# briangodwinlim/SIR-GCN

Measured on AMD Instinct MI355X. Metric: edges/sec SIRConv fwd+bwd, d_hidden=256, 1/2/4/8 MI355X, higher is better.
Workload: dtype f32; 1 GPU; cfg4 S2: Chung-Lu power-law V=2000000 E=40000000 alpha=0.8; 1 SIRConv layer d_in=H=d_out=256, agg=sum, LeakyReLU(0.2), f32, feat_dropout=0.0; fwd+bwd incl. projections; graph=S2, V=2000000, E=40000000, hidden=256, agg=sum, parallelism=single GPU

## Files before the change

include/sirconv.h:

```cpp
#ifndef SIRCONV_H
#define SIRCONV_H

#include <stdint.h>

#ifdef __cplusplus
extern "C" {
#endif

#define SIR_ABI_VERSION 17

enum { SIR_AGG_SUM = 0, SIR_AGG_MEAN = 1, SIR_AGG_SYM = 2, SIR_AGG_ACCUMULATE = 16 };
enum { SIR_ACT_IDENTITY = 0, SIR_ACT_RELU = 1, SIR_ACT_LEAKY_RELU = 2, SIR_ACT_GELU = 3, SIR_ACT_GELU_TANH = 4 };
enum { SIR_DTYPE_F32 = 0, SIR_DTYPE_BF16 = 1, SIR_DTYPE_F16 = 2 };
enum { SIR_OK = 0, SIR_EINVAL = 1, SIR_EUNSUPPORTED = 2, SIR_ELAUNCH = 3 };

int sir_abi_version(void);
const char* sir_source_hash(void);
const char* sir_last_error(void);

typedef struct {
    uint64_t seed;
    double p;
    const uint64_t* seed_ptr;
} sir_dropout_t;

int sir_dropout_apply(void* X, int64_t ldx, int64_t M, int64_t N, int dtype, int64_t col0,
                      const sir_dropout_t* drop, void* stream);

int64_t sir_mask_words(int64_t H, int act);

int sir_degree_norms(const int32_t* rowptr_dst, float* in_norm,
                     const int32_t* rowptr_src, float* out_norm, int64_t n, void* stream);

#define SIR_COLSUM_BLOCKS 1024
int sir_col_sum(const float* X, int64_t ld, int64_t n_rows, int64_t n_cols, float* out,
                float* workspace, void* stream);

int sir_edge_agg_fwd(const int32_t* rowptr, const int32_t* col,
                     const int32_t* items, int64_t n_items,
                     const int32_t* splits, int64_t n_splits,
                     int64_t H, int dtype,
                     const void* Q, int64_t ldq, const void* K, int64_t ldk,
                     const float* norm_row, const float* norm_col,
                     int agg, int act, float slope,
                     void* S, int64_t lds, uint64_t* mask_out, float* partial, void* stream);

int sir_edge_agg_bwd_dst(const int32_t* rowptr, const int32_t* col,
                         const int32_t* items, int64_t n_items,
                         const int32_t* splits, int64_t n_splits,
                         int64_t H, int dtype,
                         const void* Q, int64_t ldq, const void* K, int64_t ldk,
                         const uint64_t* mask,
                         const void* G, int64_t ldg,
                         const float* norm_row, const float* norm_col,
                         int agg, int act, float slope,
                         void* dQ, int64_t lddq, void* Gm, int64_t ldgm,
                         float* partial, const sir_dropout_t* drop, void* stream);

int sir_edge_agg_bwd_src(const int32_t* rowptr_s, const int32_t* col_s, const int32_t* perm_s,
                         const int32_t* items, int64_t n_items,
                         const int32_t* splits, int64_t n_splits,
                         int64_t H, int dtype,
                         const void* K, int64_t ldk, const void* Q, int64_t ldq,
                         const uint64_t* mask,
                         const void* Gd, int64_t ldg,
                         const float* norm_row, const float* norm_col,
                         int agg, int act, float slope,
                         void* dK, int64_t lddk, float* partial, const sir_dropout_t* drop, void* stream);

int sir_edge_agg_bwd(const int32_t* rowptr, const int32_t* col, const int32_t* items, int64_t n_items,
                     const int32_t* splits, int64_t n_splits,
                     const int32_t* rowptr_s, const int32_t* col_s, const int32_t* perm_s,
                     const int32_t* items_s, int64_t n_items_s, const int32_t* splits_s, int64_t n_splits_s,
                     int64_t H, int dtype, const uint64_t* mask, const void* G, int64_t ldg,
                     const float* in_norm, const float* out_norm, int agg, int act, float slope,
                     void* dQ, int64_t lddq, void* dK, int64_t lddk, float* partial, float* partial_s,
                     const sir_dropout_t* drop, void* stream);

int sir_edge_e_agg_fwd(const int32_t* rowptr, const int32_t* col, const int32_t* items, int64_t n_items,
                       const int32_t* splits, int64_t n_splits, int64_t H, int dtype,
                       const void* Q, int64_t ldq, const void* K, int64_t ldk,
                       const void* Eh, int64_t lde, int64_t n_erows, const int32_t* eidx,
                       const float* norm_row, const float* norm_col, int agg, int act, float slope,
                       void* S, int64_t lds, uint64_t* mask_out, float* partial, void* stream);

int sir_edge_e_bwd(const int32_t* rowptr, const int32_t* col, const int32_t* items, int64_t n_items,
                   int64_t H, int dtype, const uint64_t* mask, const void* G, int64_t ldg,
                   const float* norm_row, const float* norm_col, int agg, int act, float slope,
                   const int32_t* eidx, int64_t n_erows, void* dE, int64_t ldde, void* stream);


int sir_edge_gather_add(const int32_t* rowptr, const int32_t* col, const int32_t* items, int64_t n_items,
                        int64_t F, const float* Q, int64_t ldq, const float* K, int64_t ldk,
                        float* Z, int64_t ldz, void* stream);

int sir_edge_gather_act(const int32_t* rowptr, const int32_t* col, const int32_t* items, int64_t n_items,
                        int64_t F, const float* Q, int64_t ldq, const float* K, int64_t ldk, int act, float slope,
                        float* A, int64_t lda, uint64_t* sign_mask, void* stream);

int sir_segment_sum(const int32_t* rowptr, const int32_t* col, const int32_t* perm,
                    const int32_t* items, int64_t n_items, const int32_t* splits, int64_t n_splits,
                    int64_t F, const float* X, int64_t ldx, const float* norm_row, const float* norm_col,
                    int mean, float* out, int64_t ldo, float* partial, void* stream);

int sir_edge_broadcast(const int32_t* rowptr, const int32_t* col, const int32_t* items, int64_t n_items,
                       int64_t F, const float* dS, int64_t lds, const float* norm_row, const float* norm_col,
                       int mean, float* dM, int64_t ldm, void* stream);

int sir_segment_max(const int32_t* items, int64_t n_items, const int32_t* splits, int64_t n_splits,
                    int64_t F, const float* M, int64_t ldm, float* Y, int64_t ldy, int32_t* arg, int64_t lda,
                    float* pval, int32_t* parg, void* stream);

int sir_segment_max_bwd(const int32_t* items, int64_t n_items, int64_t F, const int32_t* arg, int64_t lda,
                        const float* dY, int64_t ldy, float* dM, int64_t ldm, void* stream);

#define SIR_AGG_MAX 3
int64_t sir_edge_mlp_pack_bytes(int64_t H, int64_t F);
int sir_edge_mlp_pack(const float* W, int64_t H, int64_t F, void* packed, void* stream);
int sir_edge_mlp_fwd(const int32_t* rowptr, const int32_t* col, const int32_t* items, int64_t n_items,
                     const int32_t* splits, int64_t n_splits, int64_t H, int64_t F,
                     const float* Q, int64_t ldq, const float* K, int64_t ldk,
                     const float* norm_row, const float* norm_col, int agg, int act1, float slope, int act2,
                     const void* packed, const float* bias, float* out, int64_t ldo, int32_t* arg, int64_t lda,
                     float* pval, int32_t* parg, void* stream);

int64_t sir_edge_mlp_stream_work_bytes(int64_t F);
int sir_edge_mlp_fwd_stream(const int32_t* rowptr, const int32_t* col, const int32_t* erow, int64_t n_rows,
                            int64_t n_edges, int64_t H, int64_t F, const float* Q, int64_t ldq, const float* K,
                            int64_t ldk, const float* norm_row, const float* norm_col, int agg, int act1, float slope,
                            int act2, const void* packed, const float* bias, float* out, int64_t ldo, int32_t* arg,
                            int64_t lda, void* work, void* stream);

int sir_edge_mlp_pack_st(const float* W, int64_t H, int64_t F, int dtype, void* packed, void* stream);
int sir_edge_mlp_fwd_st(const int32_t* rowptr, const int32_t* col, const int32_t* items, int64_t n_items,
                        const int32_t* splits, int64_t n_splits, int64_t H, int64_t F, const void* Q, int64_t ldq,
                        const void* K, int64_t ldk, int dtype, int agg, int act1, float slope, int act2,
                        const void* packed, const float* bias, float* out, int64_t ldo, int32_t* arg, int64_t lda,
                        float* pval, int32_t* parg, void* stream);
int sir_edge_mlp_fwd_stream_st(const int32_t* rowptr, const int32_t* col, const int32_t* erow, int64_t n_rows,
                               int64_t n_edges, int64_t H, int64_t F, const void* Q, int64_t ldq, const void* K,
                               int64_t ldk, int dtype, int agg, int act1, float slope, int act2, const void* packed,
                               const float* bias, float* out, int64_t ldo, int32_t* arg, int64_t lda, void* work,
                               void* stream);

int64_t sir_edge_mlp_bwd_parts(int64_t n_items, int64_t H, int64_t F);
int sir_edge_mlp_bwd_dst(const int32_t* rowptr, const int32_t* col, const int32_t* items, int64_t n_items,
                         const int32_t* splits, int64_t n_splits, int64_t H, int64_t F,
                         const float* Q, int64_t ldq, const float* K, int64_t ldk, const float* G, int64_t ldg,
                         const float* norm_row, const float* norm_col, int agg, int act1, float slope, int act2,
                         const void* packed, const float* W, const float* bias, float* dQ, int64_t lddq,
                         float* Gm, float* partial, float* wpart, void* stream);
int sir_edge_mlp_bwd_src(const int32_t* rowptr_s, const int32_t* col_s, const int32_t* items, int64_t n_items,
                         const int32_t* splits, int64_t n_splits, int64_t H, int64_t F,
                         const float* K, int64_t ldk, const float* Q, int64_t ldq, const float* Gd, int64_t ldg,
                         const float* norm_row, const float* norm_col, int agg, int act1, float slope, int act2,
                         const void* packed, const float* W, const float* bias, float* dK, int64_t lddk,
                         float* partial, void* stream);

int sir_edge_max_bwd_dst(const int32_t* rowptr, const int32_t* col, const int32_t* items, int64_t n_items,
                         const int32_t* splits, int64_t n_splits, int64_t H, int64_t O,
                         const float* Q, int64_t ldq, const float* K, int64_t ldk, const float* dY, int64_t ldy,
                         const int32_t* arg, int64_t lda, int act1, float slope, const float* W,
                         float* dQ, int64_t lddq, float* partial, float* wpart, void* stream);
int sir_edge_max_bwd_src(const int32_t* rowptr_s, const int32_t* col_s, const int32_t* perm_s,
// ... 125 lines not shown
```

sir-gcn_amd/csrc/sirconv_abi.cpp:

```cpp
#include <hip/hip_runtime.h>

#include <climits>
#include <string>

#include "sirconv.h"
#include "sirconv_internal.h"
#include "sirconv_eedge.h"

namespace {

thread_local std::string g_last_error;

int fail(int code, const char* fn, const char* msg) {
    g_last_error = std::string(fn) + ": " + msg;
    return code;
}

int check_common(const char* fn, const int32_t* rowptr, const int32_t* col, const int32_t* items,
                 int64_t n_items, const int32_t* splits, int64_t n_splits, int64_t H, int dtype,
                 int agg, int act, const float* norm_row, const float* norm_col, const void* out,
                 const float* partial) {
    if (dtype != SIR_DTYPE_F32 && dtype != SIR_DTYPE_BF16 && dtype != SIR_DTYPE_F16)
        return fail(SIR_EINVAL, fn, "dtype must be SIR_DTYPE_F32, _BF16 or _F16");
    if (agg < SIR_AGG_SUM || agg > SIR_AGG_SYM) return fail(SIR_EINVAL, fn, "agg must be SUM, MEAN or SYM");
    if (act < SIR_ACT_IDENTITY || act > SIR_ACT_GELU_TANH) return fail(SIR_EINVAL, fn, "unknown activation");
    if (H <= 0 || H > 1024) return fail(SIR_EINVAL, fn, "H must be in [1, 1024]");
    if (n_items < 0 || n_splits < 0) return fail(SIR_EINVAL, fn, "negative item/split count");
    if (n_items > 0 && (rowptr == nullptr || items == nullptr || out == nullptr))
        return fail(SIR_EINVAL, fn, "rowptr/items/output must be non-NULL");
    (void)col;
    if (n_splits > 0 && (splits == nullptr || partial == nullptr))
        return fail(SIR_EINVAL, fn, "split rows need `splits` and a `partial` workspace");
    if (agg == SIR_AGG_SYM && n_items > 0 && (norm_row == nullptr || norm_col == nullptr))
        return fail(SIR_EINVAL, fn, "SYM needs norm_row and norm_col");
    return SIR_OK;
}

int check_mask(const char* fn, int64_t H, int act) {
    if (sir_mask_words(H, act) == 0)
        return fail(SIR_EUNSUPPORTED, fn, "sign mask needs act RELU/LEAKY_RELU, H % 4 == 0 and H <= 1024");
    return SIR_OK;
}

sir::Drop to_drop(const sir_dropout_t* d, int64_t col0) {
    if (d == nullptr || !(d->p > 0.0)) return sir::Drop();
    return sir::make_drop(d->p, d->seed, (int)col0, d->seed_ptr);
}

int finish(const char* fn, hipError_t err, const char* why) {
    if (err == hipSuccess) return SIR_OK;
    if (err == hipErrorInvalidValue && why) return fail(SIR_EUNSUPPORTED, fn, why);
    if (err == hipErrorInvalidValue)
        return fail(SIR_EUNSUPPORTED, fn, "sign-mask mode needs 16-B aligned full-wave rows");
    return fail(SIR_ELAUNCH, fn, hipGetErrorString(err));
}

}

extern "C" {

int sir_abi_version(void) { return SIR_ABI_VERSION; }

#ifndef SIR_SRC_HASH
#define SIR_SRC_HASH "unknown"
#endif
const char* sir_source_hash(void) { return SIR_SRC_HASH; }

const char* sir_last_error(void) { return g_last_error.c_str(); }

int64_t sir_mask_words(int64_t H, int act) {
    if (act != SIR_ACT_RELU && act != SIR_ACT_LEAKY_RELU) return 0;
    if (H % 4 != 0 || H <= 0 || H > 1024) return 0;
    if (H > 128) return 4 * ((H + 255) / 256);
    const int64_t hc = H / 4;
    const int64_t lpr = hc <= 4 ? 4 : (hc <= 8 ? 8 : (hc <= 16 ? 16 : 32));
    return lpr >= 16 ? lpr / 16 : 1;
}

int sir_degree_norms(const int32_t* rowptr_dst, float* in_norm,
                     const int32_t* rowptr_src, float* out_norm, int64_t n, void* stream) {
    const char* fn = "sir_degree_norms";
    if (n < 0) return fail(SIR_EINVAL, fn, "negative node count");
    if (n > 0 && (rowptr_dst == nullptr || in_norm == nullptr)) return fail(SIR_EINVAL, fn, "NULL rowptr/norm");
    if ((rowptr_src == nullptr) != (out_norm == nullptr)) return fail(SIR_EINVAL, fn, "rowptr_src/out_norm pairing");
    hipError_t err = sir::run_degree_norms(rowptr_dst, in_norm, rowptr_src, out_norm, n,
                                           static_cast<hipStream_t>(stream));
    return finish(fn, err, nullptr);
}

int sir_col_sum(const float* X, int64_t ld, int64_t n_rows, int64_t n_cols, float* out,
                float* workspace, void* stream) {
    const char* fn = "sir_col_sum";
    if (n_rows < 0 || n_cols < 0 || n_cols > (1 << 20)) return fail(SIR_EINVAL, fn, "bad shape");
    if (n_cols % 4 != 0 || ld % 4 != 0 || ld < n_cols) return fail(SIR_EINVAL, fn, "n_cols and ld must be multiples of 4, ld >= n_cols");
    if (n_cols > 0 && (out == nullptr || workspace == nullptr || (n_rows > 0 && X == nullptr)))
        return fail(SIR_EINVAL, fn, "NULL buffer");
    if ((reinterpret_cast<uintptr_t>(X) & 15u) != 0) return fail(SIR_EINVAL, fn, "X must be 16-B aligned");
    hipError_t err = sir::run_colsum(X, ld, n_rows, (int)n_cols, out, workspace, SIR_COLSUM_BLOCKS,
                                     static_cast<hipStream_t>(stream));
    return finish(fn, err, nullptr);
}

int sir_edge_agg_fwd(const int32_t* rowptr, const int32_t* col,
                     const int32_t* items, int64_t n_items,
                     const int32_t* splits, int64_t n_splits,
                     int64_t H, int dtype,
                     const void* Q, int64_t ldq, const void* K, int64_t ldk,
                     const float* norm_row, const float* norm_col,
                     int agg, int act, float slope,
                     void* S, int64_t lds, uint64_t* mask_out, float* partial, void* stream) {
    const char* fn = "sir_edge_agg_fwd";
    const int accumulate = (agg & SIR_AGG_ACCUMULATE) != 0;
    agg &= ~SIR_AGG_ACCUMULATE;
    if (accumulate && agg == SIR_AGG_MEAN)
        return fail(SIR_EUNSUPPORTED, fn, "SIR_AGG_ACCUMULATE: segment sums of SUM / SYM only (divide afterwards for MEAN)");
    int rc = check_common(fn, rowptr, col, items, n_items, splits, n_splits, H, dtype, agg, act,
                          norm_row, norm_col, S, partial);
    if (rc) return rc;
    if (ldq < H || ldk < H || lds < H) return fail(SIR_EINVAL, fn, "leading dimensions must be >= H");
    if (n_items > 0 && (Q == nullptr || K == nullptr)) return fail(SIR_EINVAL, fn, "Q/K must be non-NULL");
    if (mask_out != nullptr && (rc = check_mask(fn, H, act))) return rc;
    sir::EdgeArgs a{};
    a.rowptr = rowptr; a.col = col; a.items = items; a.n_items = n_items;
    a.R = Q; a.ldr = ldq;
    a.C = K; a.ldc = ldk;
    a.G = nullptr; a.ldg = H;
    a.norm_row = norm_row; a.norm_col = norm_col; a.slope = slope; a.H = (int)H;
    a.out = S; a.ldo = lds; a.partial = partial; a.Gm = nullptr; a.ldgm = H;
    a.mask_out = mask_out;
    a.accumulate = accumulate;
    const char* why = nullptr;
    hipError_t err = sir::run_edge(sir::MODE_FWD, dtype, a, agg, act, splits, n_splits, S, lds,
                                   agg == SIR_AGG_MEAN, static_cast<hipStream_t>(stream), &why);
    return finish(fn, err, why);
}

int sir_edge_agg_bwd_dst(const int32_t* rowptr, const int32_t* col,
                         const int32_t* items, int64_t n_items,
                         const int32_t* splits, int64_t n_splits,
                         int64_t H, int dtype,
                         const void* Q, int64_t ldq, const void* K, int64_t ldk,
                         const uint64_t* mask,
                         const void* G, int64_t ldg,
                         const float* norm_row, const float* norm_col,
                         int agg, int act, float slope,
                         void* dQ, int64_t lddq, void* Gm, int64_t ldgm,
                         float* partial, const sir_dropout_t* drop, void* stream) {
    const char* fn = "sir_edge_agg_bwd_dst";
    int rc = check_common(fn, rowptr, col, items, n_items, splits, n_splits, H, dtype, agg, act,
                          norm_row, norm_col, dQ, partial);
    if (rc) return rc;
    if (ldg < H || lddq < H) return fail(SIR_EINVAL, fn, "leading dimensions must be >= H");
    if (Gm != nullptr && ldgm < H) return fail(SIR_EINVAL, fn, "ldgm must be >= H");
    if (n_items > 0 && G == nullptr) return fail(SIR_EINVAL, fn, "G must be non-NULL");
    if (mask != nullptr) {
        if ((rc = check_mask(fn, H, act))) return rc;
    } else {
        if (ldq < H || ldk < H) return fail(SIR_EINVAL, fn, "leading dimensions must be >= H");
        if (n_items > 0 && (Q == nullptr || K == nullptr)) return fail(SIR_EINVAL, fn, "Q/K must be non-NULL");
    }
    sir::EdgeArgs a{};
    a.rowptr = rowptr; a.col = col; a.items = items; a.n_items = n_items;
    a.R = Q; a.ldr = mask ? H : ldq;
    a.C = K; a.ldc = mask ? H : ldk;
    a.G = G; a.ldg = ldg;
    a.norm_row = norm_row; a.norm_col = norm_col; a.slope = slope; a.H = (int)H;
    a.out = dQ; a.ldo = lddq; a.partial = partial;
    a.Gm = (agg == SIR_AGG_MEAN) ? Gm : nullptr; a.ldgm = Gm ? ldgm : H;
    a.mask_in = mask;
    a.drop = to_drop(drop, 0);
    const char* why = nullptr;
    hipError_t err = sir::run_edge(sir::MODE_BWD_DST, dtype, a, agg, act, splits, n_splits, dQ, lddq, false,
                                   static_cast<hipStream_t>(stream), &why);
    return finish(fn, err, why);
}

int sir_edge_agg_bwd_src(const int32_t* rowptr_s, const int32_t* col_s, const int32_t* perm_s,
                         const int32_t* items, int64_t n_items,
                         const int32_t* splits, int64_t n_splits,
                         int64_t H, int dtype,
                         const void* K, int64_t ldk, const void* Q, int64_t ldq,
                         const uint64_t* mask,
                         const void* Gd, int64_t ldg,
                         const float* norm_row, const float* norm_col,
                         int agg, int act, float slope,
                         void* dK, int64_t lddk, float* partial, const sir_dropout_t* drop, void* stream) {
    const char* fn = "sir_edge_agg_bwd_src";
    int rc = check_common(fn, rowptr_s, col_s, items, n_items, splits, n_splits, H, dtype, agg, act,
                          norm_row, norm_col, dK, partial);
    if (rc) return rc;
    if (ldg < H || lddk < H) return fail(SIR_EINVAL, fn, "leading dimensions must be >= H");
    if (n_items > 0 && Gd == nullptr) return fail(SIR_EINVAL, fn, "Gd must be non-NULL");
    if (mask != nullptr) {
        if ((rc = check_mask(fn, H, act))) return rc;
        if (n_items > 0 && col_s != nullptr && perm_s == nullptr) return fail(SIR_EINVAL, fn, "sign-mask mode needs perm_s");
    } else {
        if (ldq < H || ldk < H) return fail(SIR_EINVAL, fn, "leading dimensions must be >= H");
        if (n_items > 0 && (Q == nullptr || K == nullptr)) return fail(SIR_EINVAL, fn, "K/Q must be non-NULL");
    }
    sir::EdgeArgs a{};
    a.rowptr = rowptr_s; a.col = col_s; a.items = items; a.n_items = n_items;
    a.R = K; a.ldr = mask ? H : ldk;
    a.C = Q; a.ldc = mask ? H : ldq;
    a.G = Gd; a.ldg = ldg;
    a.norm_row = norm_row; a.norm_col = norm_col; a.slope = slope; a.H = (int)H;
    a.out = dK; a.ldo = lddk; a.partial = partial; a.Gm = nullptr; a.ldgm = H;
    a.mask_in = mask; a.perm = perm_s;
    a.drop = to_drop(drop, H);
    const char* why = nullptr;
    hipError_t err = sir::run_edge(sir::MODE_BWD_SRC, dtype, a, agg, act, splits, n_splits, dK, lddk, false,
                                   static_cast<hipStream_t>(stream), &why);
    return finish(fn, err, why);
}

int sir_edge_agg_bwd(const int32_t* rowptr, const int32_t* col, const int32_t* items, int64_t n_items,
                     const int32_t* splits, int64_t n_splits,
                     const int32_t* rowptr_s, const int32_t* col_s, const int32_t* perm_s,
                     const int32_t* items_s, int64_t n_items_s, const int32_t* splits_s, int64_t n_splits_s,
                     int64_t H, int dtype, const uint64_t* mask, const void* G, int64_t ldg,
                     const float* in_norm, const float* out_norm, int agg, int act, float slope,
                     void* dQ, int64_t lddq, void* dK, int64_t lddk, float* partial, float* partial_s,
                     const sir_dropout_t* drop, void* stream) {
    const char* fn = "sir_edge_agg_bwd";
    int rc = check_common(fn, rowptr, col, items, n_items, splits, n_splits, H, dtype, agg, act, in_norm, out_norm,
                          dQ, partial);
    if (rc) return rc;
    rc = check_common(fn, rowptr_s, col_s, items_s, n_items_s, splits_s, n_splits_s, H, dtype, agg, act, out_norm,
                      in_norm, dK, partial_s);
    if (rc) return rc;
    if (agg == SIR_AGG_MEAN)
        return fail(SIR_EUNSUPPORTED, fn, "MEAN: the source pass needs the destination pass's Gm (two calls)");
    if (mask == nullptr) return fail(SIR_EINVAL, fn, "the one-launch backward is the sign-mask mode: mask required");
    if ((rc = check_mask(fn, H, act))) return rc;
    if (ldg < H || lddq < H || lddk < H) return fail(SIR_EINVAL, fn, "leading dimensions must be >= H");
    if ((n_items > 0 || n_items_s > 0) && G == nullptr) return fail(SIR_EINVAL, fn, "G must be non-NULL");
    if (n_items_s > 0 && col_s != nullptr && perm_s == nullptr) return fail(SIR_EINVAL, fn, "sign-mask mode needs perm_s");
    if (n_items > INT32_MAX || n_items_s > INT32_MAX || n_items + n_items_s > (int64_t)INT32_MAX)
        return fail(SIR_EINVAL, fn, "too many work items for one launch");
    sir::EdgeArgs a{};
    a.rowptr = rowptr; a.col = col; a.items = items; a.n_items = n_items;
    a.G = G; a.ldg = ldg; a.norm_row = in_norm; a.norm_col = out_norm; a.slope = slope; a.H = (int)H;
    a.out = dQ; a.ldo = lddq; a.partial = partial; a.mask_in = mask; a.ldr = H; a.ldc = H; a.ldgm = H;
    sir::EdgeArgs b{};
    b.rowptr = rowptr_s; b.col = col_s; b.perm = perm_s; b.items = items_s; b.n_items = n_items_s;
    b.G = G; b.ldg = ldg; b.norm_row = out_norm; b.norm_col = in_norm; b.slope = slope; b.H = (int)H;
    b.out = dK; b.ldo = lddk; b.partial = partial_s; b.mask_in = mask; b.ldr = H; b.ldc = H; b.ldgm = H;
    a.drop = to_drop(drop, 0);
    b.drop = to_drop(drop, H);
    const char* why = nullptr;
    hipError_t err = sir::run_edge_dual(dtype, a, splits, n_splits, b, splits_s, n_splits_s, agg, act,
                                        static_cast<hipStream_t>(stream), &why);
    return finish(fn, err, why);
}

static int check_eedge(const char* fn, int64_t H, int dtype, int act) {
    if (dtype != SIR_DTYPE_F32) return fail(SIR_EUNSUPPORTED, fn, "the edge-term kernels take SIR_DTYPE_F32 rows only");
    if (act != SIR_ACT_RELU && act != SIR_ACT_LEAKY_RELU)
        return fail(SIR_EUNSUPPORTED, fn, "the edge-term kernels cover act RELU / LEAKY_RELU only");
    if (H % 4 != 0) return fail(SIR_EUNSUPPORTED, fn, "the edge-term kernels need H % 4 == 0");
    return SIR_OK;
}

int sir_edge_e_agg_fwd(const int32_t* rowptr, const int32_t* col, const int32_t* items, int64_t n_items,
                       const int32_t* splits, int64_t n_splits, int64_t H, int dtype,
                       const void* Q, int64_t ldq, const void* K, int64_t ldk,
                       const void* Eh, int64_t lde, int64_t n_erows, const int32_t* eidx,
                       const float* norm_row, const float* norm_col, int agg, int act, float slope,
                       void* S, int64_t lds, uint64_t* mask_out, float* partial, void* stream) {
    const char* fn = "sir_edge_e_agg_fwd";
    int rc = check_common(fn, rowptr, col, items, n_items, splits, n_splits, H, dtype, agg, act,
                          norm_row, norm_col, S, partial);
    if (rc) return rc;
    if ((rc = check_eedge(fn, H, dtype, act))) return rc;
    if (ldq < H || ldk < H || lde < H || lds < H) return fail(SIR_EINVAL, fn, "leading dimensions must be >= H");
    if (n_items > INT32_MAX || n_erows > INT32_MAX) return fail(SIR_EINVAL, fn, "too many work items / edge rows");
    if (n_items > 0 && (Q == nullptr || K == nullptr || Eh == nullptr))
        return fail(SIR_EINVAL, fn, "Q/K/Eh must be non-NULL");
    if (n_items > 0 && n_erows <= 0) return fail(SIR_EINVAL, fn, "n_erows must be positive");
    if (n_items == 0) return SIR_OK;
    sir::EEdgeArgs a{};
    a.rowptr = rowptr; a.col = col; a.items = items; a.n_items = n_items; a.splits = splits; a.n_splits = n_splits;
    a.H = (int)H;
    a.Q = static_cast<const float*>(Q); a.ldq = ldq;
    a.K = static_cast<const float*>(K); a.ldk = ldk;
    a.Eh = static_cast<const float*>(Eh); a.lde = lde; a.n_erows = n_erows; a.eidx = eidx;
    a.norm_row = norm_row; a.norm_col = norm_col; a.slope = slope;
    a.S = static_cast<float*>(S); a.lds = lds; a.mask_out = mask_out; a.partial = partial;
    const char* why = nullptr;
    hipError_t err = sir::run_eedge_fwd(a, agg, act, static_cast<hipStream_t>(stream), &why);
    return finish(fn, err, why);
}

int sir_edge_e_bwd(const int32_t* rowptr, const int32_t* col, const int32_t* items, int64_t n_items,
                   int64_t H, int dtype, const uint64_t* mask, const void* G, int64_t ldg,
                   const float* norm_row, const float* norm_col, int agg, int act, float slope,
                   const int32_t* eidx, int64_t n_erows, void* dE, int64_t ldde, void* stream) {
    const char* fn = "sir_edge_e_bwd";
    int rc = check_common(fn, rowptr, col, items, n_items, nullptr, 0, H, dtype, agg, act,
                          norm_row, norm_col, dE, nullptr);
    if (rc) return rc;
    if (agg == SIR_AGG_MEAN)
        return fail(SIR_EUNSUPPORTED, fn, "MEAN: call with SUM on g = G / deg (as the one-launch backward)");
    if ((rc = check_eedge(fn, H, dtype, act))) return rc;
    if (ldg < H || ldde < H) return fail(SIR_EINVAL, fn, "leading dimensions must be >= H");
    if (n_items > INT32_MAX || n_erows > INT32_MAX) return fail(SIR_EINVAL, fn, "too many work items / edge rows");
    if (n_items > 0 && (mask == nullptr || G == nullptr)) return fail(SIR_EINVAL, fn, "mask/G must be non-NULL");
    if (n_items > 0 && n_erows <= 0) return fail(SIR_EINVAL, fn, "n_erows must be positive");
    if (n_items == 0) return SIR_OK;
    sir::EEdgeArgs a{};
    a.rowptr = rowptr; a.col = col; a.items = items; a.n_items = n_items;
    a.H = (int)H; a.mask_in = mask;
    a.G = static_cast<const float*>(G); a.ldg = ldg;
    a.norm_row = norm_row; a.norm_col = norm_col; a.slope = slope;
    a.eidx = eidx; a.n_erows = n_erows; a.dE = static_cast<float*>(dE); a.ldde = ldde;
    const char* why = nullptr;
    hipError_t err = sir::run_eedge_bwd_e(a, agg, act, static_cast<hipStream_t>(stream), &why);
    return finish(fn, err, why);
}

static int check_generic(const char* fn, int64_t n_items, int64_t F, const int32_t* items) {
    if (F <= 0 || F > 1024) return fail(SIR_EINVAL, fn, "F must be in [1, 1024]");
    if (n_items < 0) return fail(SIR_EINVAL, fn, "negative item count");
    if (n_items > 0 && items == nullptr) return fail(SIR_EINVAL, fn, "NULL items");
    return SIR_OK;
}

int sir_edge_gather_add(const int32_t* rowptr, const int32_t* col, const int32_t* items, int64_t n_items,
                        int64_t F, const float* Q, int64_t ldq, const float* K, int64_t ldk,
                        float* Z, int64_t ldz, void* stream) {
    const char* fn = "sir_edge_gather_add";
    int rc = check_generic(fn, n_items, F, items);
    if (rc) return rc;
    if (ldq < F || ldk < F || ldz < F) return fail(SIR_EINVAL, fn, "leading dimensions must be >= F");
    if (n_items > 0 && (Q == nullptr || K == nullptr)) return fail(SIR_EINVAL, fn, "NULL Q/K");
    sir::GenericArgs a{};
    a.rowptr = rowptr; a.col = col; a.items = items; a.n_items = n_items; a.F = (int)F;
    a.X = Q; a.ldx = ldq; a.X2 = K; a.ldx2 = ldk; a.out = Z; a.ldo = ldz;
    return finish(fn, sir::run_gather_add(a, static_cast<hipStream_t>(stream)), "unsupported F / alignment");
}

int sir_edge_gather_act(const int32_t* rowptr, const int32_t* col, const int32_t* items, int64_t n_items,
                        int64_t F, const float* Q, int64_t ldq, const float* K, int64_t ldk, int act, float slope,
                        float* A, int64_t lda, uint64_t* sign_mask, void* stream) {
    const char* fn = "sir_edge_gather_act";
    int rc = check_generic(fn, n_items, F, items);
    if (rc) return rc;
    if (act != SIR_ACT_IDENTITY && act != SIR_ACT_RELU && act != SIR_ACT_LEAKY_RELU)
        return fail(SIR_EINVAL, fn, "act must be identity, ReLU or LeakyReLU");
    if (ldq < F || ldk < F || lda < F) return fail(SIR_EINVAL, fn, "leading dimensions must be >= F");
    if (n_items > 0 && (Q == nullptr || K == nullptr)) return fail(SIR_EINVAL, fn, "NULL Q/K");
    sir::GenericArgs a{};
    a.rowptr = rowptr; a.col = col; a.items = items; a.n_items = n_items; a.F = (int)F;
    a.X = Q; a.ldx = ldq; a.X2 = K; a.ldx2 = ldk; a.out = A; a.ldo = lda;
    if (sign_mask != nullptr && F != 256) return fail(SIR_EUNSUPPORTED, fn, "sign_mask needs F = 256");
    return finish(fn, sir::run_gather_add(a, static_cast<hipStream_t>(stream), act, slope, sign_mask),
                  "unsupported F / alignment");
}

int sir_segment_sum(const int32_t* rowptr, const int32_t* col, const int32_t* perm,
                    const int32_t* items, int64_t n_items, const int32_t* splits, int64_t n_splits,
                    int64_t F, const float* X, int64_t ldx, const float* norm_row, const float* norm_col,
                    int mean, float* out, int64_t ldo, float* partial, void* stream) {
    const char* fn = "sir_segment_sum";
    int rc = check_generic(fn, n_items, F, items);
    if (rc) return rc;
    if (ldx < F || ldo < F) return fail(SIR_EINVAL, fn, "leading dimensions must be >= F");
    if ((norm_row == nullptr) != (norm_col == nullptr)) return fail(SIR_EINVAL, fn, "norm_row/norm_col pairing");
    if (n_splits > 0 && (splits == nullptr || partial == nullptr)) return fail(SIR_EINVAL, fn, "split rows need splits + partial");
    if (n_items > 0 && out == nullptr) return fail(SIR_EINVAL, fn, "NULL out");
    sir::GenericArgs a{};
    a.rowptr = rowptr; a.col = col; a.perm = perm; a.items = items; a.n_items = n_items;
    a.splits = splits; a.n_splits = n_splits; a.F = (int)F; a.X = X; a.ldx = ldx;
    a.norm_row = norm_row; a.norm_col = norm_col; a.mean = mean; a.out = out; a.ldo = ldo; a.partial = partial;
    return finish(fn, sir::run_seg_sum(a, static_cast<hipStream_t>(stream)), "unsupported F / alignment");
}

int sir_edge_broadcast(const int32_t* rowptr, const int32_t* col, const int32_t* items, int64_t n_items,
                       int64_t F, const float* dS, int64_t lds, const float* norm_row, const float* norm_col,
                       int mean, float* dM, int64_t ldm, void* stream) {
    const char* fn = "sir_edge_broadcast";
    int rc = check_generic(fn, n_items, F, items);
    if (rc) return rc;
    if (lds < F || ldm < F) return fail(SIR_EINVAL, fn, "leading dimensions must be >= F");
    if ((norm_row == nullptr) != (norm_col == nullptr)) return fail(SIR_EINVAL, fn, "norm_row/norm_col pairing");
    if (mean && rowptr == nullptr && n_items > 0) return fail(SIR_EINVAL, fn, "mean needs rowptr");
    sir::GenericArgs a{};
    a.rowptr = rowptr; a.col = col; a.items = items; a.n_items = n_items; a.F = (int)F;
    a.X = dS; a.ldx = lds; a.norm_row = norm_row; a.norm_col = norm_col; a.mean = mean; a.out = dM; a.ldo = ldm;
    return finish(fn, sir::run_edge_bcast(a, static_cast<hipStream_t>(stream)), "unsupported F / alignment");
}

int sir_segment_max(const int32_t* items, int64_t n_items, const int32_t* splits, int64_t n_splits,
                    int64_t F, const float* M, int64_t ldm, float* Y, int64_t ldy, int32_t* arg, int64_t lda,
                    float* pval, int32_t* parg, void* stream) {
    const char* fn = "sir_segment_max";
    int rc = check_generic(fn, n_items, F, items);
    if (rc) return rc;
    if (ldm < F || ldy < F || lda < F) return fail(SIR_EINVAL, fn, "leading dimensions must be >= F");
    if (n_splits > 0 && (splits == nullptr || pval == nullptr || parg == nullptr))
        return fail(SIR_EINVAL, fn, "split rows need splits + pval + parg");
    sir::GenericArgs a{};
// ... 849 lines not shown
```

sir-gcn_amd/csrc/sirconv_dispatch.hip:

```cpp
#include "sirconv_edge_impl.h"

namespace sir {

__global__ void __launch_bounds__(256)
k_degree_norms(const int* __restrict__ rowptr_a, float* __restrict__ norm_a,
               const int* __restrict__ rowptr_b, float* __restrict__ norm_b, int64_t n) {
    const int64_t i = (int64_t)blockIdx.x * blockDim.x + threadIdx.x;
    if (i >= n) return;
    const int da = rowptr_a[i + 1] - rowptr_a[i];
    norm_a[i] = 1.0f / sqrtf((float)(da > 1 ? da : 1));
    if (rowptr_b != nullptr) {
        const int db = rowptr_b[i + 1] - rowptr_b[i];
        norm_b[i] = 1.0f / sqrtf((float)(db > 1 ? db : 1));
    }
}

__global__ void __launch_bounds__(256)
k_colsum_partial(const float* __restrict__ X, int64_t ld, int64_t n_rows, int n_cols,
                 int64_t rows_per_block, float* __restrict__ part) {
    const int c4 = n_cols / 4;
    const int64_t r0 = (int64_t)blockIdx.x * rows_per_block;
    const int64_t r1 = (r0 + rows_per_block < n_rows) ? r0 + rows_per_block : n_rows;
    for (int cb = 0; cb < c4; cb += 64) {
        const int c = cb + (threadIdx.x & 63);
        const int slice = threadIdx.x >> 6;
        float4 acc = make_float4(0.f, 0.f, 0.f, 0.f);
        if (c < c4) {
            int64_t r = r0 + slice;
            for (; r + 12 < r1; r += 16) {
                float4 v[4];
#pragma unroll
                for (int i = 0; i < 4; ++i) v[i] = *reinterpret_cast<const float4*>(X + (r + 4 * i) * ld + 4 * c);
#pragma unroll
                for (int i = 0; i < 4; ++i) { acc.x += v[i].x; acc.y += v[i].y; acc.z += v[i].z; acc.w += v[i].w; }
            }
            for (; r < r1; r += 4) {
                const float4 v = *reinterpret_cast<const float4*>(X + r * ld + 4 * c);
                acc.x += v.x; acc.y += v.y; acc.z += v.z; acc.w += v.w;
            }
        }
        __shared__ float4 red[256];
        red[threadIdx.x] = acc;
        __syncthreads();
        if (threadIdx.x < 64 && c < c4) {
            float4 t = red[threadIdx.x];
#pragma unroll
            for (int k = 1; k < 4; ++k) {
                const float4 u = red[threadIdx.x + 64 * k];
                t.x += u.x; t.y += u.y; t.z += u.z; t.w += u.w;
            }
            *reinterpret_cast<float4*>(part + (int64_t)blockIdx.x * n_cols + 4 * c) = t;
        }
        __syncthreads();
    }
}

__global__ void __launch_bounds__(1024)
k_colsum_final(const float* __restrict__ part, int nb, int n_cols, float* __restrict__ out) {
    __shared__ float red[1024];
    const int c = blockIdx.x * 64 + (threadIdx.x & 63);
    const int slice = threadIdx.x >> 6;
    float acc = 0.f;
    if (c < n_cols) {
        int b = slice;
        for (; b + 7 * 16 < nb; b += 8 * 16) {
            float v[8];
#pragma unroll
            for (int i = 0; i < 8; ++i) v[i] = part[(int64_t)(b + 16 * i) * n_cols + c];
#pragma unroll
            for (int i = 0; i < 8; ++i) acc += v[i];
        }
        for (; b < nb; b += 16) acc += part[(int64_t)b * n_cols + c];
    }
    red[threadIdx.x] = acc;
    __syncthreads();
    if (threadIdx.x < 64 && c < n_cols) {
        float t = red[threadIdx.x];
        for (int k = 1; k < 16; ++k) t += red[threadIdx.x + 64 * k];
        out[c] = t;
    }
}

hipError_t run_colsum(const float* X, int64_t ld, int64_t n_rows, int n_cols, float* out,
                      float* workspace, int nb, hipStream_t st) {
    if (n_cols <= 0) return hipSuccess;
    const int64_t rpb = (n_rows + nb - 1) / nb;
    if (n_rows > 0)
        hipLaunchKernelGGL(k_colsum_partial, dim3((unsigned)nb), dim3(256), 0, st, X, ld, n_rows, n_cols, rpb, workspace);
    else
        return hipMemsetAsync(out, 0, sizeof(float) * n_cols, st);
    hipLaunchKernelGGL(k_colsum_final, dim3((unsigned)((n_cols + 63) / 64)), dim3(1024), 0, st,
                       workspace, nb, n_cols, out);
    return hipGetLastError();
}

template <int ST, bool MEAN_DIV>
static hipError_t launch_combine(const int32_t* splits, int64_t n, const float* partial, int H,
                                 void* out, int64_t ldo, int vw, hipStream_t st, const Drop& drop, int accumulate = 0) {
    if (n == 0) return hipSuccess;
    TP<ST>* o = static_cast<TP<ST>*>(out);
    if (vw == 4)
        hipLaunchKernelGGL((k_combine<ST, MEAN_DIV, 4>), dim3((unsigned)n), dim3(1024), 0, st,
                           reinterpret_cast<const int4*>(splits), partial, H, o, ldo, drop, accumulate);
    else
        hipLaunchKernelGGL((k_combine<ST, MEAN_DIV, 1>), dim3((unsigned)n), dim3(1024), 0, st,
                           reinterpret_cast<const int4*>(splits), partial, H, o, ldo, drop, accumulate);
    return hipGetLastError();
}

template <int ST>
static hipError_t run_edge_t(int mode, const EdgeArgs& a, int agg, int act, Shape s,
                             const int32_t* splits, int64_t n_splits, void* out_final, int64_t ld_final,
                             bool mean_div, hipStream_t st) {
    hipError_t err;
    switch (mode) {
        case MODE_FWD: err = launch_edge_pass<ST, MODE_FWD>(a, agg, act, s, st); break;
        case MODE_BWD_DST: err = launch_edge_pass<ST, MODE_BWD_DST>(a, agg, act, s, st); break;
        default: err = launch_edge_pass<ST, MODE_BWD_SRC>(a, agg, act, s, st); break;
    }
    if (err != hipSuccess || n_splits == 0) return err;
    return mean_div ? launch_combine<ST, true>(splits, n_splits, a.partial, a.H, out_final, ld_final, s.vw, st, a.drop)
                    : launch_combine<ST, false>(splits, n_splits, a.partial, a.H, out_final, ld_final, s.vw, st, a.drop,
                                                a.accumulate);
}

hipError_t run_degree_norms(const int* rowptr_a, float* norm_a, const int* rowptr_b, float* norm_b,
                            int64_t n, hipStream_t st) {
    if (n == 0) return hipSuccess;
    hipLaunchKernelGGL(k_degree_norms, dim3((unsigned)((n + 255) / 256)), dim3(256), 0, st,
                       rowptr_a, norm_a, rowptr_b, norm_b, n);
    return hipGetLastError();
}

static bool aligned_to(const void* p, uintptr_t b) { return p == nullptr || (reinterpret_cast<uintptr_t>(p) & (b - 1)) == 0; }

bool pick_shape(int H, bool vec4_ok, Shape* s) {
    if (H <= 0) return false;
    if (vec4_ok && (H % 4) == 0) {
        const int hc = H / 4;
        s->vw = 4;
        if (hc <= 4) { s->lpr = 4; s->nv = 1; return true; }
        if (hc <= 8) { s->lpr = 8; s->nv = 1; return true; }
        if (hc <= 16) { s->lpr = 16; s->nv = 1; return true; }
        if (hc <= 32) { s->lpr = 32; s->nv = 1; return true; }
        s->lpr = 64;
        s->nv = (hc + 63) / 64;
        return s->nv <= 4;
    }
    s->vw = 1;
    s->lpr = 64;
    s->nv = (H + 63) / 64;
    if (s->nv == 3) s->nv = 4;
    return s->nv <= 4;
}

hipError_t run_edge(int mode, int dtype, const EdgeArgs& a, int agg, int act,
                    const int32_t* splits, int64_t n_splits, void* out_final, int64_t ld_final,
                    bool mean_div, hipStream_t st, const char** why) {
    const uintptr_t vb = (dtype == ST_F32) ? 16 : 8;
    const bool v4 = aligned_to(a.R, vb) && aligned_to(a.C, vb) && aligned_to(a.G, vb) && aligned_to(a.out, vb) &&
                    aligned_to(a.partial, 16) && aligned_to(a.Gm, vb) &&
                    (a.ldr % 4 == 0) && (a.ldc % 4 == 0) && (a.ldg % 4 == 0) && (a.ldo % 4 == 0) &&
                    (a.ldgm % 4 == 0);
    Shape s;
    if (!pick_shape(a.H, v4, &s)) {
        *why = "unsupported hidden size (H must be <= 1024 with H%4==0 and 16-B aligned rows, else <= 256)";
        return hipErrorInvalidValue;
    }
    if (dtype != ST_F32 && s.vw != 4) {
        *why = "bf16/fp16 storage needs H % 4 == 0 and 8-B aligned rows (leading dimensions multiples of 4)";
        return hipErrorInvalidValue;
    }
    switch (dtype) {
        case ST_BF16: return run_edge_t<ST_BF16>(mode, a, agg, act, s, splits, n_splits, out_final, ld_final, mean_div, st);
        case ST_F16: return run_edge_t<ST_F16>(mode, a, agg, act, s, splits, n_splits, out_final, ld_final, mean_div, st);
        default: return run_edge_t<ST_F32>(mode, a, agg, act, s, splits, n_splits, out_final, ld_final, mean_div, st);
    }
}

hipError_t run_edge_dual(int dtype, const EdgeArgs& a, const int32_t* splits, int64_t n_splits,
                         const EdgeArgs& b, const int32_t* splits_s, int64_t n_splits_s,
                         int agg, int act, hipStream_t st, const char** why) {
    const uintptr_t vb = (dtype == ST_F32) ? 16 : 8;
    const bool v4 = aligned_to(a.G, vb) && aligned_to(a.out, vb) && aligned_to(b.out, vb) &&
                    aligned_to(a.partial, 16) && aligned_to(b.partial, 16) &&
                    (a.ldg % 4 == 0) && (a.ldo % 4 == 0) && (b.ldo % 4 == 0);
    Shape s;
    if (!pick_shape(a.H, v4, &s) || s.vw != 4) {
        *why = "the sign-mask backward needs H % 4 == 0, H <= 1024 and aligned rows";
        return hipErrorInvalidValue;
    }
    hipError_t err;
    switch (dtype) {
        case ST_BF16: err = launch_edge_dual<ST_BF16>(a, b, agg, act, s, st); break;
        case ST_F16: err = launch_edge_dual<ST_F16>(a, b, agg, act, s, st); break;
        default: err = launch_edge_dual<ST_F32>(a, b, agg, act, s, st); break;
    }
    if (err != hipSuccess) {
        if (err == hipErrorInvalidValue) *why = "the one-launch backward covers SUM/SYM with ReLU/LeakyReLU only";
        return err;
    }
    auto combine = [&](const int32_t* sp, int64_t n, const EdgeArgs& x) -> hipError_t {
        if (n == 0) return hipSuccess;
        switch (dtype) {
            case ST_BF16: return launch_combine<ST_BF16, false>(sp, n, x.partial, x.H, x.out, x.ldo, 4, st, x.drop);
            case ST_F16: return launch_combine<ST_F16, false>(sp, n, x.partial, x.H, x.out, x.ldo, 4, st, x.drop);
            default: return launch_combine<ST_F32, false>(sp, n, x.partial, x.H, x.out, x.ldo, 4, st, x.drop);
        }
    };
    if ((err = combine(splits, n_splits, a)) != hipSuccess) return err;
    return combine(splits_s, n_splits_s, b);
}

}
```

sir-gcn_amd/csrc/sirconv_edge_impl.h:

```cpp
#include <hip/hip_runtime.h>
#include <stdint.h>

#pragma once
#include "sirconv_internal.h"
#include "sirconv_gemm_util.h"

namespace sir {

template <int ACT>
__device__ __forceinline__ float sig(float z, float slope) {
    if constexpr (ACT == ACT_IDENTITY) {
        return z;
    } else if constexpr (ACT == ACT_RELU) {
        return z > 0.f ? z : 0.f;
    } else if constexpr (ACT == ACT_LEAKY) {
        return z > 0.f ? z : z * slope;
    } else if constexpr (ACT == ACT_GELU) {
        const float kAlpha = 0.70710678118654752440f;
        return z * 0.5f * (1.0f + erff(z * kAlpha));
    } else {
        const float kBeta = 0.79788456080286535588f;
        const float kKappa = 0.044715f;
        const float inner = kBeta * (z + kKappa * z * z * z);
        return 0.5f * z * (1.0f + tanhf(inner));
    }
}

template <int ACT>
__device__ __forceinline__ float dsig(float z, float t, float slope) {
    if constexpr (ACT == ACT_IDENTITY) {
        return t;
    } else if constexpr (ACT == ACT_RELU) {
        return z > 0.f ? t : 0.f;
    } else if constexpr (ACT == ACT_LEAKY) {
        return z > 0.f ? t : t * slope;
    } else if constexpr (ACT == ACT_GELU) {
        const float kAlpha = 0.70710678118654752440f;
        const float kBeta = 0.39894228040143267794f;
        const float cdf = 0.5f * (1.0f + erff(z * kAlpha));
        const float pdf = kBeta * expf(z * z * -0.5f);
        return t * (cdf + z * pdf);
    } else {
        const float kBeta = 0.79788456080286535588f;
        const float kKappa = 0.044715f;
        const float x_sq = z * z;
        const float x_cube = x_sq * z;
        const float inner = kBeta * (z + kKappa * x_cube);
        const float tanh_inner = tanhf(inner);
        const float left = 0.5f * z;
        const float right = 1.0f + tanh_inner;
        const float left_derivative = 0.5f * right;
        const float tanh_derivative = 1.0f - tanh_inner * tanh_inner;
        const float inner_derivative = kBeta * (1.0f + 3.0f * kKappa * x_sq);
        const float right_derivative = left * tanh_derivative * inner_derivative;
        return t * (left_derivative + right_derivative);
    }
}

template <int ST> struct Stor { typedef float T; };
template <> struct Stor<ST_BF16> { typedef __bf16 T; };
template <> struct Stor<ST_F16> { typedef _Float16 T; };

typedef unsigned int sir_u2 __attribute__((ext_vector_type(2)));
typedef unsigned int sir_u4 __attribute__((ext_vector_type(4)));

template <int ST>
__device__ __forceinline__ float h2f(uint32_t bits16) {
    if constexpr (ST == ST_BF16) return __uint_as_float(bits16 << 16);
    else return (float)__builtin_bit_cast(_Float16, (uint16_t)bits16);
}
template <int ST>
__device__ __forceinline__ uint32_t f2h(float x) {
    if constexpr (ST == ST_BF16) return (uint32_t)__builtin_bit_cast(uint16_t, (__bf16)x);
    else return (uint32_t)__builtin_bit_cast(uint16_t, (_Float16)x);
}
template <int ST>
__device__ __forceinline__ float round_st(float x) {
    if constexpr (ST == ST_F32) return x;
    else return h2f<ST>(f2h<ST>(x));
}

template <int ST, int VW>
__device__ __forceinline__ void drop_vec(const Drop& d, int64_t row, int c0, float (&v)[VW]) {
    const uint32_t rh = drop_row_hash(d, row);
#pragma unroll
    for (int w = 0; w < VW; ++w) v[w] = drop_keep(d, rh, d.col0 + c0 + w) ? round_st<ST>(v[w]) * d.scale : 0.f;
}

template <int VW>
__device__ __forceinline__ void vload(float (&d)[VW], const float* __restrict__ p) {
    if constexpr (VW == 4) {
        const float4 t = *reinterpret_cast<const float4*>(p);
        d[0] = t.x; d[1] = t.y; d[2] = t.z; d[3] = t.w;
    } else {
#pragma unroll
        for (int w = 0; w < VW; ++w) d[w] = p[w];
    }
}

template <int VW>
__device__ __forceinline__ void vstore(float* __restrict__ p, const float (&s)[VW]) {
    if constexpr (VW == 4) {
        *reinterpret_cast<float4*>(p) = make_float4(s[0], s[1], s[2], s[3]);
    } else {
#pragma unroll
        for (int w = 0; w < VW; ++w) p[w] = s[w];
    }
}

template <int ST, int VW>
__device__ __forceinline__ void tload_p(float (&d)[VW], const typename Stor<ST>::T* __restrict__ p) {
    if constexpr (ST == ST_F32) {
        vload<VW>(d, p);
    } else if constexpr (VW == 4) {
        const sir_u2* q = reinterpret_cast<const sir_u2*>(p);
        const sir_u2 t = *q;
        d[0] = h2f<ST>(t.x & 0xffffu); d[1] = h2f<ST>(t.x >> 16);
        d[2] = h2f<ST>(t.y & 0xffffu); d[3] = h2f<ST>(t.y >> 16);
    } else {
        const uint16_t* q = reinterpret_cast<const uint16_t*>(p);
#pragma unroll
        for (int w = 0; w < VW; ++w) d[w] = h2f<ST>(q[w]);
    }
}

template <int ST, int VW>
__device__ __forceinline__ void tstore_p(typename Stor<ST>::T* __restrict__ p, const float (&s)[VW]) {
    if constexpr (ST == ST_F32) {
        vstore<VW>(p, s);
    } else if constexpr (VW == 4) {
        sir_u2 t;
        t.x = f2h<ST>(s[0]) | (f2h<ST>(s[1]) << 16);
        t.y = f2h<ST>(s[2]) | (f2h<ST>(s[3]) << 16);
        *reinterpret_cast<sir_u2*>(p) = t;
    } else {
        uint16_t* q = reinterpret_cast<uint16_t*>(p);
#pragma unroll
        for (int w = 0; w < VW; ++w) q[w] = (uint16_t)f2h<ST>(s[w]);
    }
}

template <int ST, int VW>
__device__ __forceinline__ void vload_row(float (&d)[VW], const typename Stor<ST>::T* __restrict__ p) { tload_p<ST, VW>(d, p); }
template <int ST, int VW>
__device__ __forceinline__ void vstore_row(typename Stor<ST>::T* __restrict__ p, const float (&s)[VW]) { tstore_p<ST, VW>(p, s); }
template <int ST, int VW>
__device__ __forceinline__ void vload_gather(float (&d)[VW], const typename Stor<ST>::T* __restrict__ p) { tload_p<ST, VW>(d, p); }

__device__ __forceinline__ void writelane(uint32_t& v, uint32_t x, int k) {
    asm("v_writelane_b32 %0, %1, %2" : "+v"(v) : "s"(x), "i"(k));
}

template <int LPR, int VW> constexpr int sub_mask_words() { return LPR * VW >= 64 ? LPR * VW / 32 : 2; }

template <int ST, int MODE, int ACT, int AGG, int LPR, int NV, int VW, int UU, int MK>
__device__ __forceinline__ void edge_batch(int e, const int* __restrict__ col,
                                           const typename Stor<ST>::T* __restrict__ C, int64_t ldc,
                                           const typename Stor<ST>::T* __restrict__ G, int64_t ldg,
                                           const float* __restrict__ norm_col, float nr, float slope,
                                           int li, int HC,
                                           const float (&rv)[NV][VW], const float (&gv)[NV][VW],
                                           float (&acc)[NV][VW], uint64_t* __restrict__ mask, int lane,
                                           const int* __restrict__ upre = nullptr,
                                           const int* __restrict__ perm = nullptr) {
    constexpr bool MASKW = MK == 1, MASKR = MK == 2;
    static_assert(!MASKR || (LPR < 64 && NV == 1 && VW == 4 && MODE != MODE_FWD), "mask-read rows are sub-wave float4 rows");
    int u[UU];
#pragma unroll
    for (int i = 0; i < UU; ++i) u[i] = (upre != nullptr) ? upre[i] : col[e + i];
    constexpr bool kBufGather = MODE == MODE_FWD && ST == ST_F32 && VW == 4 && LPR == 64 && MASKW;
    constexpr int MWS = sub_mask_words<LPR, VW>();
    uint32_t mr[MASKR ? UU : 1][MWS];
    if constexpr (MASKR) {
#pragma unroll
        for (int i = 0; i < UU; ++i) {
            const int p = (MODE == MODE_BWD_SRC) ? perm[e + i] : e + i;
            const uint32_t* rp = reinterpret_cast<const uint32_t*>(mask) + (int64_t)p * MWS;
            if constexpr (MWS == 8) {
                const sir_u4 t = reinterpret_cast<const sir_u4*>(rp)[0];
                const sir_u4 t2 = reinterpret_cast<const sir_u4*>(rp)[1];
                mr[i][0] = t.x; mr[i][1] = t.y; mr[i][2] = t.z; mr[i][3] = t.w;
                mr[i][4] = t2.x; mr[i][5] = t2.y; mr[i][6] = t2.z; mr[i][7] = t2.w;
            } else if constexpr (MWS == 4) {
                const sir_u4 t = *reinterpret_cast<const sir_u4*>(rp);
                mr[i][0] = t.x; mr[i][1] = t.y; mr[i][2] = t.z; mr[i][3] = t.w;
            } else {
                const sir_u2 t = *reinterpret_cast<const sir_u2*>(rp);
                mr[i][0] = t.x; mr[i][1] = t.y;
            }
        }
    }
    float cv[MASKR ? 1 : UU][NV][VW];
    float gc[(MODE == MODE_BWD_SRC) ? UU : 1][NV][VW];
#pragma unroll
    for (int i = 0; i < UU; ++i) {
      if constexpr (!MASKR) {
        const auto* cp = C + (int64_t)u[i] * ldc;
        if constexpr (kBufGather) {
            const gemm::rsrc_t rs = gemm::mk_rsrc(cp, (uint32_t)(HC * 16));
#pragma unroll
            for (int j = 0; j < NV; ++j) {
                const sir_u4 t = __builtin_amdgcn_raw_buffer_load_b128(rs, (li + LPR * j) * 16, 0, 0);
                cv[i][j][0] = __uint_as_float(t.x); cv[i][j][1] = __uint_as_float(t.y);
                cv[i][j][2] = __uint_as_float(t.z); cv[i][j][3] = __uint_as_float(t.w);
            }
        } else {
#pragma unroll
            for (int j = 0; j < NV; ++j) {
                const int c = li + LPR * j;
                vload_gather<ST, VW>(cv[i][j], cp + (c < HC ? c : 0) * VW);
            }
        }
      }
        if constexpr (MODE == MODE_BWD_SRC) {
            const auto* gp = G + (int64_t)u[i] * ldg;
#pragma unroll
            for (int j = 0; j < NV; ++j) {
                const int c = li + LPR * j;
                vload_gather<ST, VW>(gc[i][j], gp + (c < HC ? c : 0) * VW);
            }
        }
    }
    float cf[UU];
    if constexpr (AGG == AGG_SYM) {
#pragma unroll
        for (int i = 0; i < UU; ++i) cf[i] = norm_col[u[i]] * nr;
    }
    if constexpr (MASKW && LPR < 64) {
        static_assert(VW == 4 && NV == 1, "sub-wave mask rows are float4 rows");
        constexpr uint32_t FM = (LPR == 32) ? 0xffffffffu : ((1u << LPR) - 1u);
        const int sh = lane - li;
        uint32_t wd[UU][MWS];
#pragma unroll
        for (int i = 0; i < UU; ++i) {
#pragma unroll
            for (int k = 0; k < MWS; ++k) wd[i][k] = 0u;
#pragma unroll
            for (int w = 0; w < VW; ++w) {
                const uint64_t b = __builtin_amdgcn_ballot_w64(li < HC && (rv[0][w] + cv[i][0][w]) > 0.f);
                wd[i][(w * LPR) / 32] |= ((uint32_t)(b >> sh) & FM) << ((w * LPR) % 32);
            }
        }
        uint32_t* mrec = reinterpret_cast<uint32_t*>(mask) + (int64_t)e * MWS;
        constexpr int NWB = UU * MWS;
#pragma unroll
        for (int r = 0; r < (NWB + LPR - 1) / LPR; ++r) {
            uint32_t mine = 0u;
#pragma unroll
            for (int i = 0; i < UU; ++i)
#pragma unroll
                for (int k = 0; k < MWS; ++k)
                    if ((i * MWS + k) / LPR == r) mine = (li == (i * MWS + k) % LPR) ? wd[i][k] : mine;
            const int q = r * LPR + li;
            if (q < NWB) mrec[q] = mine;
        }
    } else if constexpr (MASKW) {
        static_assert(LPR == 64 && VW == 4, "mask layout needs full-wave rows of float4");
        constexpr int NW = NV * VW;
        static_assert(UU * NW <= 64, "one mask store per batch");
        uint32_t mlo = 0, mhi = 0;
#pragma unroll
        for (int j = 0; j < NV; ++j) {
            const uint64_t okm = __builtin_amdgcn_ballot_w64((li + LPR * j) < HC);
#pragma unroll
            for (int i = 0; i < UU; ++i) {
#pragma unroll
                for (int w = 0; w < VW; ++w) {
                    const uint64_t b = __builtin_amdgcn_ballot_w64((rv[j][w] + cv[i][j][w]) > 0.f) & okm;
                    writelane(mlo, (uint32_t)b, i * NW + j * VW + w);
                    writelane(mhi, (uint32_t)(b >> 32), i * NW + j * VW + w);
                }
            }
        }
        const uint64_t mine = ((uint64_t)mhi << 32) | mlo;
        if (lane < UU * NW) {
            mask[(int64_t)e * NW + lane] = mine;
        }
    }
#pragma unroll
    for (int i = 0; i < UU; ++i) {
#pragma unroll
        for (int j = 0; j < NV; ++j) {
            const int c = li + LPR * j;
            if (c < HC) {
#pragma unroll
                for (int w = 0; w < VW; ++w) {
                    if constexpr (MODE == MODE_FWD) {
                        const float z = rv[j][w] + cv[i][j][w];
                        float m = sig<ACT>(z, slope);
                        if constexpr (AGG == AGG_SYM) m = cf[i] * m;
                        acc[j][w] += m;
                    } else if constexpr (MASKR) {
                        float t = (MODE == MODE_BWD_SRC) ? gc[i][j][w] : gv[j][w];
                        if constexpr (AGG == AGG_SYM) t = t * cf[i];
                        const int wi = (w * LPR) / 32;
                        const bool pos = (mr[i][wi] >> (((w * LPR) % 32) + li)) & 1u;
                        acc[j][w] += pos ? t : (ACT == ACT_RELU ? 0.f : t * slope);
                    } else if constexpr (MODE == MODE_BWD_DST) {
                        const float z = rv[j][w] + cv[i][j][w];
                        float t = gv[j][w];
                        if constexpr (AGG == AGG_SYM) t = t * cf[i];
                        acc[j][w] += dsig<ACT>(z, t, slope);
                    } else {
                        const float z = cv[i][j][w] + rv[j][w];
                        float t = gc[i][j][w];
                        if constexpr (AGG == AGG_SYM) t = t * cf[i];
                        acc[j][w] += dsig<ACT>(z, t, slope);
                    }
                }
            }
        }
    }
}

template <int ST, int MODE, int ACT, int AGG, int LPR, int NV, int VW, int U, int MK>
__device__ __forceinline__ void
edge_wave(int64_t wave, const int* __restrict__ rowptr, const int* __restrict__ col, const int* __restrict__ perm,
          const int4* __restrict__ items, int64_t n_items,
          const typename Stor<ST>::T* __restrict__ R, int64_t ldr,
          const typename Stor<ST>::T* __restrict__ C, int64_t ldc,
          const typename Stor<ST>::T* __restrict__ G, int64_t ldg,
          const float* __restrict__ norm_row, const float* __restrict__ norm_col,
          float slope, int H,
          typename Stor<ST>::T* __restrict__ out, int64_t ldo, float* __restrict__ partial,
          typename Stor<ST>::T* __restrict__ Gm, int64_t ldgm, uint64_t* __restrict__ mask, const Drop& drop,
          int accumulate = 0) {
    constexpr int MKB = MK & 3;
    constexpr bool ACC = (MK & 4) != 0;
    constexpr int RPW = 64 / LPR;
    const int lane = threadIdx.x & 63;
    const int sub = lane / LPR;
    const int li = lane - sub * LPR;
    const int64_t idx = wave * RPW + sub;
    if (idx >= n_items) return;
    int4 it = items[idx];
    if constexpr (LPR == 64) {
        it.x = __builtin_amdgcn_readfirstlane(it.x);
        it.y = __builtin_amdgcn_readfirstlane(it.y);
        it.z = __builtin_amdgcn_readfirstlane(it.z);
        it.w = __builtin_amdgcn_readfirstlane(it.w);
    }
    const int row = it.x, e0 = it.y, e1 = it.z, slot = it.w;
    const int HC = H / VW;

    float rv[NV][VW];
    float gv[NV][VW];
    float acc[NV][VW];
    const auto* rp = R + (int64_t)row * ldr;
#pragma unroll
    for (int j = 0; j < NV; ++j) {
        const int c = li + LPR * j;
#pragma unroll
        for (int w = 0; w < VW; ++w) { acc[j][w] = 0.f; rv[j][w] = 0.f; gv[j][w] = 0.f; }
        if (MKB != 2 && c < HC) vload_row<ST, VW>(rv[j], rp + c * VW);
    }
    if constexpr (MODE == MODE_BWD_DST) {
        const auto* gp = G + (int64_t)row * ldg;
        float degf = 1.f;
        bool first = true;
        if constexpr (AGG == AGG_MEAN) {
            const int rs = rowptr[row];
            const int d = rowptr[row + 1] - rs;
            degf = (float)(d > 1 ? d : 1);
            first = (e0 == rs);
        }
#pragma unroll
        for (int j = 0; j < NV; ++j) {
            const int c = li + LPR * j;
            if (c < HC) {
                vload_row<ST, VW>(gv[j], gp + c * VW);
                if constexpr (AGG == AGG_MEAN) {
#pragma unroll
                    for (int w = 0; w < VW; ++w) gv[j][w] = round_st<ST>(gv[j][w] / degf);
                    if (Gm != nullptr && first) vstore_row<ST, VW>(Gm + (int64_t)row * ldgm + c * VW, gv[j]);
                }
            }
        }
    }
    float nr = 1.f;
    if constexpr (AGG == AGG_SYM) nr = norm_row[row];

    int e = e0;
    if constexpr (LPR == 64 && ST == ST_F32) {
        if (e + U <= e1) {
            auto load_col = [&](int eb) {
                const int q0 = eb + (lane < U ? lane : 0);
                return col[q0 < e1 ? q0 : e1 - 1];
            };
            int vc = load_col(e);
            for (; e + U <= e1; e += U) {
                int uc[U];
#pragma unroll
                for (int i = 0; i < U; ++i) uc[i] = __builtin_amdgcn_readlane(vc, i);
                vc = load_col(e + U);
                edge_batch<ST, MODE, ACT, AGG, LPR, NV, VW, U, MKB>(e, col, C, ldc, G, ldg, norm_col, nr, slope, li, HC,
                                                                  rv, gv, acc, mask, lane, uc, perm);
            }
        }
    } else {
        for (; e + U <= e1; e += U)
            edge_batch<ST, MODE, ACT, AGG, LPR, NV, VW, U, MKB>(e, col, C, ldc, G, ldg, norm_col, nr, slope, li, HC, rv, gv,
                                                              acc, mask, lane, nullptr, perm);
    }
    if constexpr (U > 8) {
        if (e + 8 <= e1) {
            edge_batch<ST, MODE, ACT, AGG, LPR, NV, VW, 8, MKB>(e, col, C, ldc, G, ldg, norm_col, nr, slope, li, HC, rv, gv, acc, mask, lane, nullptr, perm);
            e += 8;
        }
    }
    if constexpr (U > 4) {
        if (e + 4 <= e1) {
            edge_batch<ST, MODE, ACT, AGG, LPR, NV, VW, 4, MKB>(e, col, C, ldc, G, ldg, norm_col, nr, slope, li, HC, rv, gv, acc, mask, lane, nullptr, perm);
            e += 4;
        }
    }
    if constexpr (U > 2) {
        if (e + 2 <= e1) {
            edge_batch<ST, MODE, ACT, AGG, LPR, NV, VW, 2, MKB>(e, col, C, ldc, G, ldg, norm_col, nr, slope, li, HC, rv, gv, acc, mask, lane, nullptr, perm);
            e += 2;
        }
    }
    if (e < e1)
        edge_batch<ST, MODE, ACT, AGG, LPR, NV, VW, 1, MKB>(e, col, C, ldc, G, ldg, norm_col, nr, slope, li, HC, rv, gv, acc, mask, lane, nullptr, perm);

    if (slot < 0) {
        if constexpr (MODE == MODE_FWD && AGG == AGG_MEAN) {
            const int d = e1 - e0;
            const float degf = (float)(d > 1 ? d : 1);
#pragma unroll
            for (int j = 0; j < NV; ++j)
#pragma unroll
                for (int w = 0; w < VW; ++w) acc[j][w] = acc[j][w] / degf;
        }
        auto* op = out + (int64_t)row * ldo;
        if constexpr (MODE != MODE_FWD) {
            if (drop.on()) {
#pragma unroll
                for (int j = 0; j < NV; ++j) drop_vec<ST, VW>(drop, row, (li + LPR * j) * VW, acc[j]);
            }
        } else {
            if constexpr (ACC) {
#pragma unroll
                for (int j = 0; j < NV; ++j) {
                    const int c = li + LPR * j;
                    if (c < HC) {
                        float prev[VW];
                        vload_row<ST, VW>(prev, op + c * VW);
#pragma unroll
                        for (int w = 0; w < VW; ++w) acc[j][w] = prev[w] + acc[j][w];
                    }
                }
            }
        }
#pragma unroll
        for (int j = 0; j < NV; ++j) {
            const int c = li + LPR * j;
            if (c < HC) vstore_row<ST, VW>(op + c * VW, acc[j]);
        }
    } else {
        float* pp = partial + (int64_t)slot * H;
#pragma unroll
        for (int j = 0; j < NV; ++j) {
            const int c = li + LPR * j;
            if (c < HC) vstore<VW>(pp + c * VW, acc[j]);
        }
    }
}

template <int ST, int MODE, int ACT, int AGG, int LPR, int NV, int VW, int U, int MK>
__global__ void __launch_bounds__(256)
k_edge(const int* __restrict__ rowptr, const int* __restrict__ col, const int* __restrict__ perm,
       const int4* __restrict__ items, int64_t n_items,
       const typename Stor<ST>::T* __restrict__ R, int64_t ldr,
       const typename Stor<ST>::T* __restrict__ C, int64_t ldc,
       const typename Stor<ST>::T* __restrict__ G, int64_t ldg,
       const float* __restrict__ norm_row, const float* __restrict__ norm_col,
       float slope, int H,
       typename Stor<ST>::T* __restrict__ out, int64_t ldo, float* __restrict__ partial,
       typename Stor<ST>::T* __restrict__ Gm, int64_t ldgm, uint64_t* __restrict__ mask, Drop drop, int accumulate) {
    drop = drop_resolve(drop);
    int64_t wave = (int64_t)blockIdx.x * (blockDim.x >> 6) + (threadIdx.x >> 6);
    if constexpr (LPR == 64) wave = __builtin_amdgcn_readfirstlane((int)wave);
    edge_wave<ST, MODE, ACT, AGG, LPR, NV, VW, U, MK>(wave, rowptr, col, perm, items, n_items, R, ldr, C, ldc, G, ldg,
                                                     norm_row, norm_col, slope, H, out, ldo, partial, Gm, ldgm, mask,
                                                     drop, accumulate);
}

__device__ __forceinline__ uint64_t uniform64(uint64_t x) {
    const uint32_t lo = __builtin_amdgcn_readfirstlane((uint32_t)x);
    const uint32_t hi = __builtin_amdgcn_readfirstlane((uint32_t)(x >> 32));
    return ((uint64_t)hi << 32) | lo;
}

__device__ __forceinline__ float lane_select(uint64_t m, float if0, float if1) {
    float r;
    asm("v_cndmask_b32_e64 %0, %1, %2, %3" : "=v"(r) : "v"(if0), "v"(if1), "s"(m));
    return r;
}

template <int ACT>
__device__ __forceinline__ float sel_mask(uint64_t m, float t, float slope) {
    if constexpr (ACT == ACT_RELU) return lane_select(m, 0.f, t);
    else return lane_select(m, t * slope, t);
}


template <int UU> struct EdgeIdx { int v[UU]; int p[UU]; };

template <int ST, int MODE, int ACT, int AGG, int NV, int UU, bool PRE = false, bool PIDX = false>
__device__ __forceinline__ void mask_batch(int e, const int* __restrict__ col, const int* __restrict__ perm,
                                           const typename Stor<ST>::T* __restrict__ G, int64_t ldg,
                                           const uint64_t* __restrict__ mask,
                                           const float* __restrict__ norm_col, float nr, float slope,
                                           int lane, int HC, const float (&gv)[NV][4], float (&acc)[NV][4],
                                           uint64_t pre = 0, int pre_lane = 0, float cfw = 0.f, int cf_lane = 0,
                                           const EdgeIdx<UU>* idx = nullptr) {
    constexpr int NW = NV * 4;
    int p[UU];
    int v[UU];
#pragma unroll
    for (int i = 0; i < UU; ++i) {
        if constexpr (MODE == MODE_BWD_SRC && PIDX) {
            v[i] = idx->v[i];
            p[i] = idx->p[i];
        } else if constexpr (MODE == MODE_BWD_SRC) {
            v[i] = __builtin_amdgcn_readfirstlane(col[e + i]);
            p[i] = __builtin_amdgcn_readfirstlane(perm[e + i]);
        } else {
            p[i] = e + i;
            if constexpr (AGG == AGG_SYM && !PRE) v[i] = __builtin_amdgcn_readfirstlane(col[e + i]);
        }
    }
    uint64_t wd[UU][NW];
    if constexpr (PRE) {
        const int mlo = (int)(uint32_t)pre, mhi = (int)(uint32_t)(pre >> 32);
#pragma unroll
        for (int i = 0; i < UU; ++i)
#pragma unroll
            for (int k = 0; k < NW; ++k) {
                const uint32_t lo = (uint32_t)__builtin_amdgcn_readlane(mlo, pre_lane + i * NW + k);
                const uint32_t hi = (uint32_t)__builtin_amdgcn_readlane(mhi, pre_lane + i * NW + k);
                wd[i][k] = ((uint64_t)hi << 32) | lo;
            }
    } else if constexpr (MODE == MODE_BWD_DST && UU * NW <= 64) {
        const uint64_t mv = (lane < UU * NW) ? mask[(int64_t)e * NW + lane] : 0ull;
        const int mlo = (int)(uint32_t)mv, mhi = (int)(uint32_t)(mv >> 32);
#pragma unroll
        for (int i = 0; i < UU; ++i)
#pragma unroll
            for (int k = 0; k < NW; ++k) {
                const uint32_t lo = (uint32_t)__builtin_amdgcn_readlane(mlo, i * NW + k);
                const uint32_t hi = (uint32_t)__builtin_amdgcn_readlane(mhi, i * NW + k);
                wd[i][k] = ((uint64_t)hi << 32) | lo;
            }
    } else {
#pragma unroll
    for (int i = 0; i < UU; ++i)
#pragma unroll
        for (int k = 0; k < NW; ++k) wd[i][k] = uniform64(mask[(int64_t)p[i] * NW + k]);
    }
    float cf[UU];
    if constexpr (AGG == AGG_SYM && PRE) {
#pragma unroll
        for (int i = 0; i < UU; ++i)
            cf[i] = __builtin_bit_cast(float, __builtin_amdgcn_readlane(__builtin_bit_cast(int, cfw), cf_lane + i)) * nr;
    } else if constexpr (AGG == AGG_SYM) {
#pragma unroll
        for (int i = 0; i < UU; ++i) cf[i] = norm_col[v[i]] * nr;
    }
    float gc[(MODE == MODE_BWD_SRC) ? UU : 1][NV][4];
    if constexpr (MODE == MODE_BWD_SRC) {
#pragma unroll
        for (int i = 0; i < UU; ++i) {
            const auto* gp = G + (int64_t)v[i] * ldg;
#pragma unroll
            for (int j = 0; j < NV; ++j) {
                const int c = lane + 64 * j;
                vload_gather<ST, 4>(gc[i][j], gp + (c < HC ? c : 0) * 4);
            }
        }
    }
#pragma unroll
    for (int i = 0; i < UU; ++i) {
#pragma unroll
        for (int j = 0; j < NV; ++j) {
            const int c = lane + 64 * j;
            if (c < HC) {
#pragma unroll
                for (int w = 0; w < 4; ++w) {
                    float t;
                    if constexpr (MODE == MODE_BWD_SRC) t = gc[i][j][w];
                    else t = gv[j][w];
                    if constexpr (AGG == AGG_SYM) t = t * cf[i];
                    acc[j][w] += sel_mask<ACT>(wd[i][j * 4 + w], t, slope);
                }
            }
        }
    }
}

template <int ST, int MODE, int ACT, int AGG, int NV, int U>
__device__ __forceinline__ void mask_item(int e0, int e1, const int* __restrict__ col, const int* __restrict__ perm,
                                          const typename Stor<ST>::T* __restrict__ G, int64_t ldg,
                                          const uint64_t* __restrict__ mask,
                                          const float* __restrict__ norm_col, float nr, float slope,
                                          int lane, int HC, const float (&gv)[NV][4], float (&acc)[NV][4]) {
    int e = e0;
    if constexpr (MODE == MODE_BWD_SRC) {
        if (e + U <= e1) {
            auto load_idx = [&](int eb, int& vc, int& pc) {
                const int q0 = eb + (lane < U ? lane : 0);
                const int q = q0 < e1 ? q0 : e1 - 1;
                vc = col[q];
                pc = perm[q];
            };
            int vc, pc;
            load_idx(e, vc, pc);
            for (; e + U <= e1; e += U) {
                EdgeIdx<U> cur;
#pragma unroll
                for (int i = 0; i < U; ++i) {
                    cur.v[i] = __builtin_amdgcn_readlane(vc, i);
                    cur.p[i] = __builtin_amdgcn_readlane(pc, i);
                }
                load_idx(e + U, vc, pc);
                mask_batch<ST, MODE, ACT, AGG, NV, U, false, true>(e, col, perm, G, ldg, mask, norm_col, nr, slope, lane,
                                                                   HC, gv, acc, 0, 0, 0.f, 0, &cur);
            }
        }
    } else {
        for (; e + U <= e1; e += U)
            mask_batch<ST, MODE, ACT, AGG, NV, U>(e, col, perm, G, ldg, mask, norm_col, nr, slope, lane, HC, gv, acc);
    }
    if constexpr (U > 8) {
        if (e + 8 <= e1) {
            mask_batch<ST, MODE, ACT, AGG, NV, 8>(e, col, perm, G, ldg, mask, norm_col, nr, slope, lane, HC, gv, acc);
            e += 8;
        }
    }
    if constexpr (U > 4) {
        if (e + 4 <= e1) {
            mask_batch<ST, MODE, ACT, AGG, NV, 4>(e, col, perm, G, ldg, mask, norm_col, nr, slope, lane, HC, gv, acc);
            e += 4;
        }
    }
    if constexpr (U > 2) {
        if (e + 2 <= e1) {
            mask_batch<ST, MODE, ACT, AGG, NV, 2>(e, col, perm, G, ldg, mask, norm_col, nr, slope, lane, HC, gv, acc);
            e += 2;
        }
    }
    if (e < e1)
        mask_batch<ST, MODE, ACT, AGG, NV, 1>(e, col, perm, G, ldg, mask, norm_col, nr, slope, lane, HC, gv, acc);
}


template <int ST, int ACT, int AGG, int NV>
__device__ __forceinline__ void mask_item_dst_wide(int e0, int e1, const int* __restrict__ col,
                                                   const uint64_t* __restrict__ mask,
                                                   const float* __restrict__ norm_col, float nr, float slope, int lane,
                                                   int HC, const float (&gv)[NV][4], float (&acc)[NV][4]) {
    constexpr int NW = NV * 4, CH = 64 / NW, SB = (NV == 1) ? 4 : (NV == 2 ? 2 : 1);
    static_assert(CH % SB == 0, "sub-batches tile a chunk");
    constexpr bool kSym = (AGG == AGG_SYM);
    if (e0 >= e1) return;
    auto load_chunk = [&](int eb) -> uint64_t {
        const int n = e1 - eb;
        const int lim = (n >= CH ? CH : n) * NW;
        return mask[(lane < lim) ? (int64_t)eb * NW + lane : (int64_t)e0 * NW];
    };
    auto load_col = [&](int eb) -> int {
        const int n = e1 - eb;
        return col[(lane < (n >= CH ? CH : n)) ? eb + lane : e0];
    };
    auto gather_norm = [&](int c) -> float { return norm_col[c]; };
    auto full = [&](uint64_t c, int eb, float f) {
#pragma unroll
        for (int s = 0; s < CH / SB; ++s)
            mask_batch<ST, MODE_BWD_DST, ACT, AGG, NV, SB, true>(eb + s * SB, nullptr, nullptr, nullptr, 0, mask,
                                                                 nullptr, nr, slope, lane, HC, gv, acc, c, s * SB * NW,
                                                                 f, s * SB);
    };
    auto tail = [&](uint64_t c, int eb, float f) {
        const int r = e1 - eb;
#pragma unroll
        for (int i = 0; i < CH - 1; ++i)
            if (i < r)
                mask_batch<ST, MODE_BWD_DST, ACT, AGG, NV, 1, true>(eb + i, nullptr, nullptr, nullptr, 0, mask, nullptr,
                                                                nr, slope, lane, HC, gv, acc, c, i * NW, f, i);
    };
    const int nfull = (e1 - e0) / CH;
    uint64_t ca = load_chunk(e0);
    int ka = 0, kb = 0;
    if constexpr (kSym) ka = load_col(e0);
    uint64_t cb = load_chunk(e0 + CH);
    if constexpr (kSym) kb = load_col(e0 + CH);
    float fa = 0.f, fb = 0.f;
    if constexpr (kSym) fa = gather_norm(ka);
    int e = e0;
    for (int k = 2; k <= nfull; k += 2) {
        full(ca, e, fa);
        if constexpr (kSym) fb = gather_norm(kb);
        ca = load_chunk(e + 2 * CH);
        if constexpr (kSym) ka = load_col(e + 2 * CH);
        full(cb, e + CH, fb);
        if constexpr (kSym) fa = gather_norm(ka);
        cb = load_chunk(e + 3 * CH);
        if constexpr (kSym) kb = load_col(e + 3 * CH);
        e += 2 * CH;
    }
    if (nfull & 1) {
        full(ca, e, fa);
        if constexpr (kSym) fb = gather_norm(kb);
        tail(cb, e + CH, fb);
    } else {
        tail(ca, e, fa);
    }
}


__device__ __forceinline__ int4 uniform_item(const int4* __restrict__ items, int64_t i) {
    int4 it = items[i];
    it.x = __builtin_amdgcn_readfirstlane(it.x);
    it.y = __builtin_amdgcn_readfirstlane(it.y);
    it.z = __builtin_amdgcn_readfirstlane(it.z);
    it.w = __builtin_amdgcn_readfirstlane(it.w);
    return it;
}

template <int ST, int MODE, int ACT, int AGG, int NV, int U>
__device__ __forceinline__ void
mask_pass_item(int64_t wave, const int* __restrict__ rowptr, const int* __restrict__ col, const int* __restrict__ perm,
               const int4* __restrict__ items,
               const typename Stor<ST>::T* __restrict__ G, int64_t ldg, const uint64_t* __restrict__ mask,
               const float* __restrict__ norm_row, const float* __restrict__ norm_col,
               float slope, int H, typename Stor<ST>::T* __restrict__ out, int64_t ldo, float* __restrict__ partial,
               typename Stor<ST>::T* __restrict__ Gm, int64_t ldgm, const Drop& drop) {
    const int lane = threadIdx.x & 63;
    const int4 it = uniform_item(items, wave);
    const int row = it.x, e0 = it.y, e1 = it.z, slot = it.w;
    const int HC = H / 4;
    float gv[NV][4];
    float acc[NV][4];
#pragma unroll
    for (int j = 0; j < NV; ++j)
#pragma unroll
        for (int w = 0; w < 4; ++w) { acc[j][w] = 0.f; gv[j][w] = 0.f; }
    if constexpr (MODE == MODE_BWD_DST) {
        const auto* gp = G + (int64_t)row * ldg;
        float degf = 1.f;
        bool first = true;
        if constexpr (AGG == AGG_MEAN) {
            const int rs = rowptr[row];
            const int d = rowptr[row + 1] - rs;
            degf = (float)(d > 1 ? d : 1);
            first = (e0 == rs);
        }
#pragma unroll
        for (int j = 0; j < NV; ++j) {
            const int c = lane + 64 * j;
            if (c < HC) {
                vload_row<ST, 4>(gv[j], gp + c * 4);
                if constexpr (AGG == AGG_MEAN) {
#pragma unroll
                    for (int w = 0; w < 4; ++w) gv[j][w] = round_st<ST>(gv[j][w] / degf);
                    if (Gm != nullptr && first) vstore_row<ST, 4>(Gm + (int64_t)row * ldgm + c * 4, gv[j]);
                }
            }
        }
    }
    float nr = 1.f;
    if constexpr (AGG == AGG_SYM) nr = norm_row[row];
    if constexpr (MODE == MODE_BWD_DST)
        mask_item_dst_wide<ST, ACT, AGG, NV>(e0, e1, col, mask, norm_col, nr, slope, lane, HC, gv, acc);
    else
        mask_item<ST, MODE, ACT, AGG, NV, U>(e0, e1, col, perm, G, ldg, mask, norm_col, nr, slope, lane, HC, gv, acc);
    if (slot < 0) {
        auto* op = out + (int64_t)row * ldo;
        if (drop.on()) {
#pragma unroll
            for (int j = 0; j < NV; ++j) drop_vec<ST, 4>(drop, row, (lane + 64 * j) * 4, acc[j]);
        }
#pragma unroll
        for (int j = 0; j < NV; ++j) {
            const int c = lane + 64 * j;
            if (c < HC) vstore_row<ST, 4>(op + c * 4, acc[j]);
        }
    } else {
        float* op = partial + (int64_t)slot * H;
#pragma unroll
        for (int j = 0; j < NV; ++j) {
            const int c = lane + 64 * j;
            if (c < HC) vstore<4>(op + c * 4, acc[j]);
        }
    }
}

template <int ST, int MODE, int ACT, int AGG, int NV, int U>
__global__ void __launch_bounds__(256)
k_edge_mask(const int* __restrict__ rowptr, const int* __restrict__ col, const int* __restrict__ perm,
            const int4* __restrict__ items, int64_t n_items,
            const typename Stor<ST>::T* __restrict__ G, int64_t ldg, const uint64_t* __restrict__ mask,
            const float* __restrict__ norm_row, const float* __restrict__ norm_col,
            float slope, int H, typename Stor<ST>::T* __restrict__ out, int64_t ldo, float* __restrict__ partial,
            typename Stor<ST>::T* __restrict__ Gm, int64_t ldgm, Drop drop) {
    drop = drop_resolve(drop);
    const int64_t wave = __builtin_amdgcn_readfirstlane((int)((int64_t)blockIdx.x * (blockDim.x >> 6) + (threadIdx.x >> 6)));
    if (wave >= n_items) return;
    mask_pass_item<ST, MODE, ACT, AGG, NV, U>(wave, rowptr, col, perm, items, G, ldg, mask, norm_row, norm_col, slope, H,
                                              out, ldo, partial, Gm, ldgm, drop);
}

template <int ST, int ACT, int AGG, int NV, int UD, int US, bool DR>
__global__ void __launch_bounds__(256)
k_edge_mask_dual(const int* __restrict__ rowptr, const int* __restrict__ col, const int4* __restrict__ items,
                 int64_t n_items, float* __restrict__ partial, typename Stor<ST>::T* __restrict__ dQ, int64_t lddq,
                 const int* __restrict__ rowptr_s, const int* __restrict__ col_s, const int* __restrict__ perm_s,
                 const int4* __restrict__ items_s, int64_t n_items_s, float* __restrict__ partial_s,
                 typename Stor<ST>::T* __restrict__ dK, int64_t lddk,
                 const typename Stor<ST>::T* __restrict__ G, int64_t ldg, const uint64_t* __restrict__ mask,
                 const float* __restrict__ in_norm, const float* __restrict__ out_norm, float slope, int H,
                 Drop drop_q, Drop drop_k) {
    if constexpr (DR) {
        drop_q = drop_resolve(drop_q);
        drop_k = drop_resolve(drop_k);
    }
    const int64_t w = __builtin_amdgcn_readfirstlane((int)((int64_t)blockIdx.x * (blockDim.x >> 6) + (threadIdx.x >> 6)));
    const int64_t nmin = n_items < n_items_s ? n_items : n_items_s;
    bool dst;
    int64_t idx;
    if (w < 2 * nmin) {
        dst = (w & 1) == 0;
        idx = w >> 1;
    } else {
        dst = n_items > n_items_s;
        idx = nmin + (w - 2 * nmin);
        if (idx >= (dst ? n_items : n_items_s)) return;
    }
    if (dst)
        mask_pass_item<ST, MODE_BWD_DST, ACT, AGG, NV, UD>(idx, rowptr, col, nullptr, items, G, ldg, mask, in_norm,
                                                           out_norm, slope, H, dQ, lddq, partial, nullptr, H, drop_q);
    else
        mask_pass_item<ST, MODE_BWD_SRC, ACT, AGG, NV, US>(idx, rowptr_s, col_s, perm_s, items_s, G, ldg, mask,
                                                           out_norm, in_norm, slope, H, dK, lddk, partial_s, nullptr, H,
                                                           drop_k);
}

#ifndef SIR_COMBINE_PF
#define SIR_COMBINE_PF 4
#endif
template <int ST, bool MEAN_DIV, int VW>
__global__ void __launch_bounds__(1024)
k_combine(const int4* __restrict__ splits, const float* __restrict__ partial,
          int H, typename Stor<ST>::T* __restrict__ out, int64_t ldo, Drop drop, int accumulate) {
    drop = drop_resolve(drop);
    __shared__ float red[1024 * VW];
    const int4 sp = splits[blockIdx.x];
    const int HC = H / VW;
    const int cols = HC < 1024 ? HC : 1024;
    const int nslice = 1024 / cols;
    const int t = threadIdx.x;
    const int slice = t / cols;
    const float degf = (float)(sp.w > 1 ? sp.w : 1);
    for (int c0 = 0; c0 < HC; c0 += cols) {
        const int c = c0 + (t % cols);
        float acc[VW];
#pragma unroll
        for (int w = 0; w < VW; ++w) acc[w] = 0.f;
        if (slice < nslice && c < HC) {
            const float* base = partial + (int64_t)sp.y * H + c * VW;
            int s = slice;
            for (; s + (SIR_COMBINE_PF - 1) * nslice < sp.z; s += SIR_COMBINE_PF * nslice) {
                float v[SIR_COMBINE_PF][VW];
#pragma unroll
                for (int i = 0; i < SIR_COMBINE_PF; ++i) vload<VW>(v[i], base + (int64_t)(s + i * nslice) * H);
#pragma unroll
                for (int i = 0; i < SIR_COMBINE_PF; ++i)
#pragma unroll
                    for (int w = 0; w < VW; ++w) acc[w] += v[i][w];
            }
            for (; s < sp.z; s += nslice) {
                float v[VW];
                vload<VW>(v, base + (int64_t)s * H);
#pragma unroll
                for (int w = 0; w < VW; ++w) acc[w] += v[w];
            }
        }
#pragma unroll
        for (int w = 0; w < VW; ++w) red[t * VW + w] = acc[w];
        __syncthreads();
        if (t < cols && c < HC) {
            float r[VW];
#pragma unroll
            for (int w = 0; w < VW; ++w) r[w] = red[t * VW + w];
            for (int k = 1; k < nslice; ++k)
#pragma unroll
                for (int w = 0; w < VW; ++w) r[w] += red[(k * cols + t) * VW + w];
            if constexpr (MEAN_DIV) {
#pragma unroll
                for (int w = 0; w < VW; ++w) r[w] = r[w] / degf;
            }
            if (drop.on()) drop_vec<ST, VW>(drop, sp.x, c * VW, r);
            if (accumulate) {
                float prev[VW];
                tload_p<ST, VW>(prev, out + (int64_t)sp.x * ldo + c * VW);
#pragma unroll
                for (int w = 0; w < VW; ++w) r[w] = prev[w] + r[w];
            }
            tstore_p<ST, VW>(out + (int64_t)sp.x * ldo + c * VW, r);
        }
        __syncthreads();
    }
}

#ifndef SIR_UNROLL_FWD
#define SIR_UNROLL_FWD 6
#endif
#ifndef SIR_UNROLL_DST
#define SIR_UNROLL_DST 6
#endif
#ifndef SIR_UNROLL_SRC
#define SIR_UNROLL_SRC 8
#endif
#ifndef SIR_UNROLL_FWD_H
#define SIR_UNROLL_FWD_H 4
#endif
#ifndef SIR_UNROLL_DST_H
#define SIR_UNROLL_DST_H 6
#endif
#ifndef SIR_UNROLL_SRC_H
#define SIR_UNROLL_SRC_H 4
#endif
#if SIR_UNROLL_FWD > 16 || SIR_UNROLL_DST > 16 || SIR_UNROLL_SRC > 16 || SIR_UNROLL_FWD_H > 16 || \
    SIR_UNROLL_DST_H > 16 || SIR_UNROLL_SRC_H > 16
#error "unroll must be <= 16 (the tail covers < 16 edges)"
#endif
template <int MODE, int ST>
constexpr int unroll_of() {
    if constexpr (ST == ST_F32)
        return MODE == MODE_FWD ? SIR_UNROLL_FWD : (MODE == MODE_BWD_DST ? SIR_UNROLL_DST : SIR_UNROLL_SRC);
    else
        return MODE == MODE_FWD ? SIR_UNROLL_FWD_H : (MODE == MODE_BWD_DST ? SIR_UNROLL_DST_H : SIR_UNROLL_SRC_H);
}

template <int ST> using TP = typename Stor<ST>::T;
template <int ST> __host__ inline const TP<ST>* cp_(const void* p) { return static_cast<const TP<ST>*>(p); }
template <int ST> __host__ inline TP<ST>* mp_(void* p) { return static_cast<TP<ST>*>(p); }

template <int ST, int MODE, int ACT, int AGG, int LPR, int NV, int VW>
static hipError_t launch_edge_t(const EdgeArgs& a, hipStream_t st) {
    constexpr int U = (NV == 1) ? unroll_of<MODE, ST>() : 4;
    constexpr int RPW = 64 / LPR;
    const int64_t waves = (a.n_items + RPW - 1) / RPW;
    const int64_t blocks = (waves + 3) / 4;
    if (blocks == 0) return hipSuccess;
    constexpr bool kReluFamily = (ACT == ACT_RELU || ACT == ACT_LEAKY) && VW == 4 && (LPR == 64 || NV == 1);
    constexpr bool kMaskable = (MODE == MODE_FWD) && kReluFamily;
    if constexpr (kMaskable) {
        if (a.mask_out != nullptr) {
#define SIR_EDGE_FWD_MASK(MKV)                                                                                       \
            hipLaunchKernelGGL((k_edge<ST, MODE, ACT, AGG, LPR, NV, VW, U, MKV>), dim3((unsigned)blocks), dim3(256), 0,   \
                               st, a.rowptr, a.col, nullptr, reinterpret_cast<const int4*>(a.items), a.n_items,        \
                               cp_<ST>(a.R), a.ldr, cp_<ST>(a.C), a.ldc, cp_<ST>(a.G), a.ldg, a.norm_row, a.norm_col,  \
                               a.slope, a.H, mp_<ST>(a.out), a.ldo, a.partial, mp_<ST>(a.Gm), a.ldgm, a.mask_out,      \
                               a.drop, a.accumulate)
            if (a.accumulate) SIR_EDGE_FWD_MASK(1 | 4);
            else SIR_EDGE_FWD_MASK(1);
#undef SIR_EDGE_FWD_MASK
            return hipGetLastError();
        }
    } else {
        if (a.mask_out != nullptr) return hipErrorInvalidValue;
    }
    if constexpr (MODE != MODE_FWD && kReluFamily && LPR < 64) {
        if (a.mask_in != nullptr) {
            hipLaunchKernelGGL((k_edge<ST, MODE, ACT, AGG, LPR, NV, VW, U, 2>), dim3((unsigned)blocks), dim3(256), 0, st,
                               a.rowptr, a.col, a.perm, reinterpret_cast<const int4*>(a.items), a.n_items,
                               cp_<ST>(a.R), a.ldr, cp_<ST>(a.C), a.ldc, cp_<ST>(a.G), a.ldg, a.norm_row, a.norm_col,
                               a.slope, a.H, mp_<ST>(a.out), a.ldo, a.partial, mp_<ST>(a.Gm), a.ldgm,
                               const_cast<uint64_t*>(a.mask_in), a.drop, 0);
            return hipGetLastError();
        }
    }
    if (a.mask_in != nullptr) return hipErrorInvalidValue;
#define SIR_EDGE_PLAIN(MKV)                                                                                           \
    hipLaunchKernelGGL((k_edge<ST, MODE, ACT, AGG, LPR, NV, VW, U, MKV>), dim3((unsigned)blocks), dim3(256), 0, st,   \
                       a.rowptr, a.col, nullptr, reinterpret_cast<const int4*>(a.items), a.n_items,                   \
                       cp_<ST>(a.R), a.ldr, cp_<ST>(a.C), a.ldc, cp_<ST>(a.G), a.ldg, a.norm_row, a.norm_col,         \
                       a.slope, a.H, mp_<ST>(a.out), a.ldo, a.partial, mp_<ST>(a.Gm), a.ldgm, nullptr, a.drop,        \
                       a.accumulate)
    if constexpr (MODE == MODE_FWD) {
        if (a.accumulate) SIR_EDGE_PLAIN(4);
        else SIR_EDGE_PLAIN(0);
    } else {
        SIR_EDGE_PLAIN(0);
    }
#undef SIR_EDGE_PLAIN
    return hipGetLastError();
}

template <int ST, int MODE, int ACT, int AGG, int NV>
static hipError_t launch_mask_t(const EdgeArgs& a, hipStream_t st) {
    constexpr int U = (NV == 1) ? unroll_of<MODE, ST>() : (NV == 2 ? 4 : 2);
    const int64_t blocks = (a.n_items + 3) / 4;
    if (blocks == 0) return hipSuccess;
    hipLaunchKernelGGL((k_edge_mask<ST, MODE, ACT, AGG, NV, U>), dim3((unsigned)blocks), dim3(256), 0, st,
                       a.rowptr, a.col, a.perm, reinterpret_cast<const int4*>(a.items), a.n_items,
                       cp_<ST>(a.G), a.ldg, a.mask_in, a.norm_row, a.norm_col, a.slope, a.H,
                       mp_<ST>(a.out), a.ldo, a.partial, mp_<ST>(a.Gm), a.ldgm, a.drop);
    return hipGetLastError();
}

template <int ST, int ACT, int AGG, int NV>
static hipError_t launch_dual_t(const EdgeArgs& a, const EdgeArgs& b, hipStream_t st) {
    constexpr int UD = (NV == 1) ? unroll_of<MODE_BWD_DST, ST>() : (NV == 2 ? 4 : 2);
    constexpr int US = (NV == 1) ? unroll_of<MODE_BWD_SRC, ST>() : (NV == 2 ? 4 : 2);
    const int64_t blocks = (a.n_items + b.n_items + 3) / 4;
    if (blocks == 0) return hipSuccess;
#define SIR_DUAL(DRV)                                                                                               \
    hipLaunchKernelGGL((k_edge_mask_dual<ST, ACT, AGG, NV, UD, US, DRV>), dim3((unsigned)blocks), dim3(256), 0, st,  \
                       a.rowptr, a.col, reinterpret_cast<const int4*>(a.items), a.n_items, a.partial,              \
                       mp_<ST>(a.out), a.ldo,                                                                      \
                       b.rowptr, b.col, b.perm, reinterpret_cast<const int4*>(b.items), b.n_items, b.partial,      \
                       mp_<ST>(b.out), b.ldo, cp_<ST>(a.G), a.ldg, a.mask_in, a.norm_row, a.norm_col, a.slope, a.H, \
                       a.drop, b.drop)
    if (a.drop.sptr != nullptr || b.drop.sptr != nullptr) SIR_DUAL(true);
    else SIR_DUAL(false);
#undef SIR_DUAL
    return hipGetLastError();
}

template <int ST, int ACT, int AGG>
static hipError_t launch_dual_shape(const EdgeArgs& a, const EdgeArgs& b, Shape s, hipStream_t st) {
    switch (s.nv) {
        case 1: return launch_dual_t<ST, ACT, AGG, 1>(a, b, st);
        case 2: return launch_dual_t<ST, ACT, AGG, 2>(a, b, st);
        case 3: return launch_dual_t<ST, ACT, AGG, 3>(a, b, st);
        default: return launch_dual_t<ST, ACT, AGG, 4>(a, b, st);
    }
}

template <int ST>
static hipError_t launch_edge_dual_st(const EdgeArgs& a, const EdgeArgs& b, int agg, int act, Shape s, hipStream_t st) {
    if (s.vw != 4 || (agg != AGG_SUM && agg != AGG_SYM) || (act != ACT_RELU && act != ACT_LEAKY))
        return hipErrorInvalidValue;
    if (s.lpr < 64) {
        hipError_t e2 = launch_edge_pass<ST, MODE_BWD_DST>(a, agg, act, s, st);
        if (e2 != hipSuccess) return e2;
        return launch_edge_pass<ST, MODE_BWD_SRC>(b, agg, act, s, st);
    }
    if (act == ACT_RELU)
        return agg == AGG_SUM ? launch_dual_shape<ST, ACT_RELU, AGG_SUM>(a, b, s, st)
                              : launch_dual_shape<ST, ACT_RELU, AGG_SYM>(a, b, s, st);
    return agg == AGG_SUM ? launch_dual_shape<ST, ACT_LEAKY, AGG_SUM>(a, b, s, st)
                          : launch_dual_shape<ST, ACT_LEAKY, AGG_SYM>(a, b, s, st);
}

template <int ST, int MODE, int ACT, int AGG>
static hipError_t launch_mask_shape(const EdgeArgs& a, Shape s, hipStream_t st) {
    switch (s.nv) {
        case 1: return launch_mask_t<ST, MODE, ACT, AGG, 1>(a, st);
        case 2: return launch_mask_t<ST, MODE, ACT, AGG, 2>(a, st);
        case 3: return launch_mask_t<ST, MODE, ACT, AGG, 3>(a, st);
        default: return launch_mask_t<ST, MODE, ACT, AGG, 4>(a, st);
    }
}

template <int ST, int MODE, int ACT, int AGG>
static hipError_t launch_edge_shape(const EdgeArgs& a, Shape s, hipStream_t st) {
    if constexpr (MODE != MODE_FWD && (ACT == ACT_RELU || ACT == ACT_LEAKY)) {
        if (a.mask_in != nullptr) {
            if (s.vw != 4) return hipErrorInvalidValue;
            if (s.lpr == 64) return launch_mask_shape<ST, MODE, ACT, AGG>(a, s, st);
        }
    } else if constexpr (MODE != MODE_FWD) {
        if (a.mask_in != nullptr) return hipErrorInvalidValue;
    }
    if (s.vw == 4) {
        if (s.lpr == 4) return launch_edge_t<ST, MODE, ACT, AGG, 4, 1, 4>(a, st);
        if (s.lpr == 8) return launch_edge_t<ST, MODE, ACT, AGG, 8, 1, 4>(a, st);
        if (s.lpr == 16) return launch_edge_t<ST, MODE, ACT, AGG, 16, 1, 4>(a, st);
        if (s.lpr == 32) return launch_edge_t<ST, MODE, ACT, AGG, 32, 1, 4>(a, st);
        switch (s.nv) {
            case 1: return launch_edge_t<ST, MODE, ACT, AGG, 64, 1, 4>(a, st);
            case 2: return launch_edge_t<ST, MODE, ACT, AGG, 64, 2, 4>(a, st);
            case 3: return launch_edge_t<ST, MODE, ACT, AGG, 64, 3, 4>(a, st);
            default: return launch_edge_t<ST, MODE, ACT, AGG, 64, 4, 4>(a, st);
        }
    }
    if constexpr (ST != ST_F32) {
        return hipErrorInvalidValue;
    } else {
        switch (s.nv) {
            case 1: return launch_edge_t<ST, MODE, ACT, AGG, 64, 1, 1>(a, st);
            case 2: return launch_edge_t<ST, MODE, ACT, AGG, 64, 2, 1>(a, st);
            default: return launch_edge_t<ST, MODE, ACT, AGG, 64, 4, 1>(a, st);
        }
    }
}

template <int ST, int MODE, int ACT>
static hipError_t launch_edge_agg(const EdgeArgs& a, int agg, Shape s, hipStream_t st) {
    switch (agg) {
        case AGG_SUM: return launch_edge_shape<ST, MODE, ACT, AGG_SUM>(a, s, st);
        case AGG_MEAN: return launch_edge_shape<ST, MODE, ACT, AGG_MEAN>(a, s, st);
        default: return launch_edge_shape<ST, MODE, ACT, AGG_SYM>(a, s, st);
    }
}

template <int ST, int MODE>
static hipError_t launch_edge_mode(const EdgeArgs& a, int agg, int act, Shape s, hipStream_t st) {
    switch (act) {
        case ACT_IDENTITY: return launch_edge_agg<ST, MODE, ACT_IDENTITY>(a, agg, s, st);
        case ACT_RELU: return launch_edge_agg<ST, MODE, ACT_RELU>(a, agg, s, st);
        case ACT_LEAKY: return launch_edge_agg<ST, MODE, ACT_LEAKY>(a, agg, s, st);
        case ACT_GELU: return launch_edge_agg<ST, MODE, ACT_GELU>(a, agg, s, st);
        default: return launch_edge_agg<ST, MODE, ACT_GELU_TANH>(a, agg, s, st);
    }
}

}
```

sir-gcn_amd/csrc/sirconv_internal.h:

```cpp
#pragma once
#include <hip/hip_runtime.h>
#include <stdint.h>

#include "sirconv_dropout.h"

namespace sir {

enum { AGG_SUM = 0, AGG_MEAN = 1, AGG_SYM = 2 };
enum { ACT_IDENTITY = 0, ACT_RELU = 1, ACT_LEAKY = 2, ACT_GELU = 3, ACT_GELU_TANH = 4 };
enum { MODE_FWD = 0, MODE_BWD_DST = 1, MODE_BWD_SRC = 2 };
enum { ST_F32 = 0, ST_BF16 = 1, ST_F16 = 2 };

struct EdgeArgs {
    const int* rowptr;
    const int* col;
    const int32_t* items;
    int64_t n_items;
    const void* R;  int64_t ldr;
    const void* C;  int64_t ldc;
    const void* G;  int64_t ldg;
    const float* norm_row;
    const float* norm_col;
    float slope;
    int H;
    void* out;  int64_t ldo;
    float* partial;
    void* Gm;  int64_t ldgm;
    uint64_t* mask_out;
    const uint64_t* mask_in;
    const int* perm;
    Drop drop;
    int accumulate;
};

struct Shape {
    int lpr, nv, vw;
};

template <int ST, int MODE>
hipError_t launch_edge_pass(const EdgeArgs& a, int agg, int act, Shape s, hipStream_t st);
#define SIR_DECL_PASS(ST_, MODE_) \
    template <> hipError_t launch_edge_pass<ST_, MODE_>(const EdgeArgs&, int, int, Shape, hipStream_t);
SIR_DECL_PASS(ST_F32, MODE_FWD) SIR_DECL_PASS(ST_F32, MODE_BWD_DST) SIR_DECL_PASS(ST_F32, MODE_BWD_SRC)
SIR_DECL_PASS(ST_BF16, MODE_FWD) SIR_DECL_PASS(ST_BF16, MODE_BWD_DST) SIR_DECL_PASS(ST_BF16, MODE_BWD_SRC)
SIR_DECL_PASS(ST_F16, MODE_FWD) SIR_DECL_PASS(ST_F16, MODE_BWD_DST) SIR_DECL_PASS(ST_F16, MODE_BWD_SRC)
#undef SIR_DECL_PASS
template <int ST>
hipError_t launch_edge_dual(const EdgeArgs& a, const EdgeArgs& b, int agg, int act, Shape s, hipStream_t st);
template <> hipError_t launch_edge_dual<ST_F32>(const EdgeArgs&, const EdgeArgs&, int, int, Shape, hipStream_t);
template <> hipError_t launch_edge_dual<ST_BF16>(const EdgeArgs&, const EdgeArgs&, int, int, Shape, hipStream_t);
template <> hipError_t launch_edge_dual<ST_F16>(const EdgeArgs&, const EdgeArgs&, int, int, Shape, hipStream_t);
hipError_t run_edge_dual(int dtype, const EdgeArgs& a, const int32_t* splits, int64_t n_splits,
                         const EdgeArgs& b, const int32_t* splits_s, int64_t n_splits_s,
                         int agg, int act, hipStream_t st, const char** why);

struct GenericArgs {
    const int* rowptr;
    const int* col;
    const int* perm;
    const int32_t* items;
    int64_t n_items;
    const int32_t* splits;
    int64_t n_splits;
    int F;
    const float* X;  int64_t ldx;
    const float* X2; int64_t ldx2;
    const float* norm_row;
    const float* norm_col;
    int mean;
    float* out;  int64_t ldo;
    float* partial;
    int* arg;  int64_t lda;
    int* parg;
};

hipError_t run_gather_add(const GenericArgs& a, hipStream_t st, int act = ACT_IDENTITY, float slope = 0.f,
                          uint64_t* smask = nullptr);
hipError_t run_seg_sum(const GenericArgs& a, hipStream_t st);
hipError_t run_edge_bcast(const GenericArgs& a, hipStream_t st);
hipError_t run_seg_max(const GenericArgs& a, hipStream_t st);
hipError_t run_seg_max_bwd(const GenericArgs& a, hipStream_t st);

hipError_t run_resid_act_fwd(const void* Y, int64_t ldy, int dtype, const float* R, int64_t ldr, float* O, int64_t ldo,
                             int64_t M, int N, int act, float slope, int order, hipStream_t st);
hipError_t run_resid_act_bwd(const float* D, int64_t ldd, const float* D2, int64_t ldd2, const void* Y, int64_t ldy,
                             int dtype, const float* R, int64_t ldr, void* DY, int64_t lddy, float* DR, int64_t lddr,
                             int64_t M, int N, int act, float slope, int order, hipStream_t st);
hipError_t run_graph_norm_fwd(const int64_t* off, int64_t B, int F, const float* X, int64_t ldx,
                              const float* w, const float* bias, const float* ms, float eps, int act, float slope,
                              const float* R, int64_t ldr, float* Y, int64_t ldy, float* mean, float* sd,
                              hipStream_t st);
hipError_t run_graph_norm_bwd(const int64_t* off, int64_t B, int F, const float* X, int64_t ldx,
                              const float* dY, int64_t ldg, const float* w, const float* bias, const float* ms,
                              const float* mean, const float* sd, int act, float slope, float* dX, int64_t lddx,
                              float* dw_part, float* dms_part, float* db_part, hipStream_t st);

int64_t batch_norm_slabs(int64_t M);
int64_t batch_norm_work_floats(int64_t M, int64_t N);
hipError_t run_batch_norm_stats(const float* X, int64_t ldx, int64_t M, int N, float eps, float momentum,
                                float* run_mean, float* run_var, double* mean, double* invstd, float* work,
                                hipStream_t st);
hipError_t run_batch_norm_act_fwd(const float* X, int64_t ldx, int64_t M, int N, const double* mean,
                                  const double* invstd, const float* gamma, const float* beta, int act, float slope,
                                  const float* R, int64_t ldr, float* Y, int64_t ldy, hipStream_t st);
hipError_t run_batch_norm_act_bwd(const float* X, int64_t ldx, const float* D, int64_t ldg, int64_t M, int N,
                                  const double* mean, const double* invstd, const float* gamma, const float* beta,
                                  int act, float slope, int training, float* dX, int64_t lddx, float* dgamma,
                                  float* dbeta, float* work, hipStream_t st);
int64_t layer_norm_parts(int64_t M);
hipError_t run_layer_norm_act_fwd(const float* X, int64_t ldx, int64_t M, int N, const float* gamma,
                                  const float* beta, float eps, int act, float slope, const float* R, int64_t ldr,
                                  float* Y, int64_t ldy, float* mean, float* rstd, hipStream_t st);
hipError_t run_layer_norm_act_bwd(const float* X, int64_t ldx, const float* D, int64_t ldg, int64_t M, int N,
                                  const float* gamma, const float* beta, const float* mean, const float* rstd,
                                  int act, float slope, float* dX, int64_t lddx, float* dw_part, float* db_part,
                                  int64_t ldp, hipStream_t st);

int64_t graph_pool_slots(int64_t V, int64_t B);
int64_t graph_pool_work_floats(int64_t V, int64_t B, int64_t F, int op);
hipError_t run_graph_pool_fwd(const int64_t* off, int64_t B, int64_t V, int F, int op, int dtype, const void* X,
                              int64_t ldx, void* P, int64_t ldp, int* arg, float* work, hipStream_t st);
hipError_t run_graph_pool_bwd(const int64_t* off, int64_t B, int64_t V, int F, int op, int dtype, const void* dP,
                              int64_t ldg, const int* arg, void* dX, int64_t lddx, hipStream_t st);

hipError_t run_degree_norms(const int* rowptr_a, float* norm_a, const int* rowptr_b, float* norm_b,
                            int64_t n, hipStream_t st);

hipError_t run_colsum(const float* X, int64_t ld, int64_t n_rows, int n_cols, float* out,
                      float* workspace, int nb, hipStream_t st);

hipError_t run_edge(int mode, int dtype, const EdgeArgs& a, int agg, int act,
                    const int32_t* splits, int64_t n_splits, void* out_final, int64_t ld_final,
                    bool mean_div, hipStream_t st, const char** why);

int64_t csr_build_workspace(int64_t n_rows, int64_t E);
hipError_t run_csr_build(const int64_t* rows, const int64_t* cols, int64_t E, int64_t n_rows, int64_t n_cols,
                         int chunk, int* rowptr, int* col, int64_t* eid, int32_t* items, int32_t* splits,
                         int64_t* counts, void* ws, int64_t ws_bytes, hipStream_t st);
hipError_t run_csr_perm(const int64_t* eid_a, const int64_t* eid_b, int64_t E, int* pos_ws, int* perm,
                        hipStream_t st);

struct EdgeMlpArgs {
    const int* rowptr;
    const int* col;
    const int32_t* items;
    int64_t n_items;
    const int32_t* splits;
    int64_t n_splits;
    const float* Q;  int64_t ldq;
    const float* K;  int64_t ldk;
    const float* G;  int64_t ldg;
    const float* norm_row;
    const float* norm_col;
    float slope;
    int H, HP, F;
    const void* Wp;
    const float* W;
    const float* bias;
    float* out;  int64_t ldo;
    int* arg;  int64_t lda;
    const int* perm;
    float* pval;
    int* parg;
    float* Gm;
    float* wpart;
    const int* erow;
    int64_t n_rows, n_edges;
    void* work;
    int st = 0;
};
int64_t mlp_stream_work_bytes(int F);
hipError_t run_mlp_fwd_stream(const EdgeMlpArgs& a, int red, int act1, int act2, hipStream_t st);
int64_t mlp_pack_floats(int H, int F);
hipError_t run_mlp_pack(const float* W, int H, int F, void* packed, hipStream_t st);
hipError_t run_mlp_pack_st(const float* W, int H, int F, int dtype, void* packed, hipStream_t st);
hipError_t run_mlp_fwd(const EdgeMlpArgs& a, int red, int act1, int act2, hipStream_t st);
int mlp_bwd_blocks(int64_t n_items, int H, int F);
hipError_t run_mlp_bwd(const EdgeMlpArgs& a, bool dst, int red, int act1, int act2, hipStream_t st);

struct MaxBwdArgs {
    const int* rowptr_d; const int* col_d; const int32_t* items_d; int64_t n_items_d;
    const int32_t* splits_d; int64_t n_splits_d;
    const int* col_s; const int32_t* items_s; int64_t n_items_s; const int32_t* splits_s; int64_t n_splits_s;
    const int* pinv;
    int H, O; int64_t V;
// ... 57 lines not shown
```

sir-gcn_amd/sirgcn/_native.py:

```python
import ctypes
import os
import threading

import torch

LIB_PATH = os.environ.get("SIRGCN_LIB") or os.path.join(os.path.dirname(os.path.dirname(os.path.abspath(__file__))),
                                                        "lib", "libsirconv.so")

AGG = {"sum": 0, "mean": 1, "sym": 2}
ACT_IDENTITY, ACT_RELU, ACT_LEAKY, ACT_GELU, ACT_GELU_TANH = range(5)
DTYPE_F32, DTYPE_BF16, DTYPE_F16 = 0, 1, 2
ABI_VERSION = 17
STORAGE = {torch.float32: DTYPE_F32, torch.bfloat16: DTYPE_BF16, torch.float16: DTYPE_F16}

_P, _I64, _I, _F = ctypes.c_void_p, ctypes.c_int64, ctypes.c_int, ctypes.c_float
SIGNATURES = {
    "sir_abi_version": (ctypes.c_int, []),
    "sir_source_hash": (ctypes.c_char_p, []),
    "sir_last_error": (ctypes.c_char_p, []),
    "sir_mask_words": (ctypes.c_int64, [_I64, _I]),
    "sir_degree_norms": (ctypes.c_int, [_P, _P, _P, _P, _I64, _P]),
    "sir_col_sum": (ctypes.c_int, [_P, _I64, _I64, _I64, _P, _P, _P]),
    "sir_graph_norm_fwd": (ctypes.c_int, [_P, _I64, _I64, _P, _I64, _P, _P, _P, _F, _P, _I64, _P, _P, _P]),
    "sir_graph_norm_bwd": (ctypes.c_int, [_P, _I64, _I64, _P, _I64, _P, _I64, _P, _P, _P, _P, _P, _I64,
# ... 100 lines not shown
        return ctypes.byref(Dropout(0, float(p), seed.data_ptr()))
    return ctypes.byref(Dropout(int(seed) & (2 ** 64 - 1), float(p), None))


_lib = None
_lock = threading.Lock()

_timing = None


def enable_timing(on=True):
    global _timing
    _timing = {} if on else None
    return _timing


class _Timed:
    __slots__ = ("name", "dev", "ev", "work")

    def __init__(self, name, dev, work=0):
        self.name, self.dev, self.ev, self.work = name, dev, None, work

    def __enter__(self):
        if _timing is not None:
            s = torch.cuda.current_stream(self.dev)
            self.ev = (torch.cuda.Event(enable_timing=True), torch.cuda.Event(enable_timing=True))
            self.ev[0].record(s)

    def __exit__(self, *exc):
        if self.ev is not None:
            self.ev[1].record(torch.cuda.current_stream(self.dev))
            _timing.setdefault(self.name, []).append((self.ev[0], self.ev[1], self.work))


CSRC = os.path.join(os.path.dirname(os.path.dirname(os.path.abspath(__file__))), "csrc")
INCLUDE = os.path.join(os.path.dirname(os.path.dirname(os.path.dirname(os.path.abspath(__file__)))), "include")


def source_hash():
    import glob
    import hashlib
    files = sorted(glob.glob(os.path.join(CSRC, "*.hip")) + glob.glob(os.path.join(CSRC, "*.h"))
                   + glob.glob(os.path.join(CSRC, "*.cpp")) + glob.glob(os.path.join(INCLUDE, "*.h")))
    if not files:
        return None
    h = hashlib.sha256()
    for f in files:
        with open(f, "rb") as fh:
            h.update(fh.read())
    return h.hexdigest()[:16]


EDGE_SOURCES = ("sirconv_edge_impl.h", "sirconv_dropout.h", "sirconv_internal.h", "sirconv_dispatch.hip",
                "sirconv_fwd_f32.hip", "sirconv_fwd_bf16.hip", "sirconv_fwd_f16.hip",
                "sirconv_bwd_dual_f32.hip", "sirconv_bwd_dual_bf16.hip", "sirconv_bwd_dual_f16.hip")


def edge_source_hash():
    import hashlib
    h = hashlib.sha256()
    for name in EDGE_SOURCES:
        p = os.path.join(CSRC, name)
        if not os.path.exists(p):
            return None
        with open(p, "rb") as fh:
            h.update(fh.read())
    return h.hexdigest()[:16]


def build_id():
    return {"source_hash": source_hash(), "edge_source_hash": edge_source_hash()}


def load():
    global _lib
    if _lib is not None:
        return _lib
    with _lock:
        if _lib is None:
            if not os.path.exists(LIB_PATH):
                raise RuntimeError(f"sirgcn: native library not found at {LIB_PATH}; "
                                   "build it with `make -C sir-gcn_amd/csrc` (no CPU fallback exists)")
            lib = ctypes.CDLL(LIB_PATH)
            for name, (res, args) in SIGNATURES.items():
                fn = getattr(lib, name)
                fn.restype = res
                fn.argtypes = args
            if lib.sir_abi_version() != ABI_VERSION:
                raise RuntimeError(f"sirgcn: ABI mismatch (library {lib.sir_abi_version()}, host {ABI_VERSION})")
            want = source_hash()
            got = lib.sir_source_hash().decode()
            if want is not None and got != want:
                raise RuntimeError(f"sirgcn: {LIB_PATH} was built from other sources (library {got}, tree {want}); "
                                   "rebuild it with `make -C sir-gcn_amd/csrc`")
            _lib = lib
    return _lib


def _ptr(t):
    return None if t is None else ctypes.c_void_p(t.data_ptr())


def _check(rc, lib):
    if rc != 0:
        raise RuntimeError(f"sirgcn native error {rc}: {lib.sir_last_error().decode()}")


def _stream(device):
    return ctypes.c_void_p(torch.cuda.current_stream(device).cuda_stream)


def _ld(t, H):
    assert t.dim() == 2 and t.stride(1) == 1 and t.shape[1] >= H, "rows must be unit-stride"
    return t.stride(0)


def mask_words(H, act):
    return int(load().sir_mask_words(H, act))


def degree_norms(rowptr_dst, rowptr_src, in_norm, out_norm):
    lib = load()
    n = in_norm.numel()
    rc = lib.sir_degree_norms(_ptr(rowptr_dst), _ptr(in_norm), _ptr(rowptr_src), _ptr(out_norm), n,
                              _stream(in_norm.device))
    _check(rc, lib)


COLSUM_BLOCKS = 1024


def col_sum(X):
    lib = load()
    n, m = X.shape
    out = torch.empty(m, device=X.device, dtype=torch.float32)
    ws = torch.empty(COLSUM_BLOCKS * m, device=X.device, dtype=torch.float32)
    rc = lib.sir_col_sum(_ptr(X), X.stride(0), n, m, _ptr(out), _ptr(ws), _stream(X.device))
    _check(rc, lib)
    return out


def _ldx(t, H):
    return H if t is None else _ld(t, H)


def _storage(*ts):
    dts = {t.dtype for t in ts if t is not None}
    if len(dts) != 1 or next(iter(dts)) not in STORAGE:
        raise RuntimeError(f"edge pass: feature tensors must share one of fp32/bf16/fp16, got {dts}")
    return STORAGE[dts.pop()]


AGG_ACCUMULATE = 16


def edge_agg_fwd(csr, Q, K, norm_row, norm_col, agg, act, slope, S, partial, mask_out=None, accumulate=False):
    lib = load()
    H = S.shape[1]
    with _Timed("sir_edge_agg_fwd", S.device):
        rc = lib.sir_edge_agg_fwd(
            _ptr(csr.rowptr), _ptr(csr.col), _ptr(csr.items), csr.n_items, _ptr(csr.splits), csr.n_splits,
            H, _storage(Q, K, S), _ptr(Q), _ld(Q, H), _ptr(K), _ld(K, H), _ptr(norm_row), _ptr(norm_col),
            AGG[agg] | (AGG_ACCUMULATE if accumulate else 0), act, float(slope), _ptr(S), _ld(S, H),
            _ptr(mask_out), _ptr(partial), _stream(S.device))
    _check(rc, lib)


def edge_agg_bwd_dst(csr, Q, K, G, norm_row, norm_col, agg, act, slope, dQ, Gm, partial, mask=None, drop=None):
    lib = load()
    H = dQ.shape[1]
    with _Timed("sir_edge_agg_bwd_dst", dQ.device):
        rc = lib.sir_edge_agg_bwd_dst(
            _ptr(csr.rowptr), _ptr(csr.col), _ptr(csr.items), csr.n_items, _ptr(csr.splits), csr.n_splits,
            H, _storage(Q, K, G, dQ, Gm), _ptr(Q), _ldx(Q, H), _ptr(K), _ldx(K, H), _ptr(mask), _ptr(G), _ld(G, H),
            _ptr(norm_row), _ptr(norm_col), AGG[agg], act, float(slope),
            _ptr(dQ), _ld(dQ, H), _ptr(Gm), _ldx(Gm, H), _ptr(partial), _drop(drop), _stream(dQ.device))
    _check(rc, lib)


def edge_agg_bwd_src(csr_s, K, Q, Gd, norm_row, norm_col, agg, act, slope, dK, partial, mask=None, drop=None):
    lib = load()
    H = dK.shape[1]
    with _Timed("sir_edge_agg_bwd_src", dK.device):
        rc = lib.sir_edge_agg_bwd_src(
            _ptr(csr_s.rowptr), _ptr(csr_s.col), _ptr(csr_s.perm if mask is not None else None),
            _ptr(csr_s.items), csr_s.n_items, _ptr(csr_s.splits), csr_s.n_splits, H, _storage(K, Q, Gd, dK),
            _ptr(K), _ldx(K, H), _ptr(Q), _ldx(Q, H), _ptr(mask), _ptr(Gd), _ld(Gd, H),
            _ptr(norm_row), _ptr(norm_col), AGG[agg], act, float(slope),
            _ptr(dK), _ld(dK, H), _ptr(partial), _drop(drop), _stream(dK.device))
    _check(rc, lib)


def edge_agg_bwd(csr, csr_s, G, mask, in_norm, out_norm, agg, act, slope, dQ, dK, partial, partial_s, drop=None):
    lib = load()
    H = dQ.shape[1]
    with _Timed("sir_edge_agg_bwd", dQ.device):
        rc = lib.sir_edge_agg_bwd(
            _ptr(csr.rowptr), _ptr(csr.col), _ptr(csr.items), csr.n_items, _ptr(csr.splits), csr.n_splits,
            _ptr(csr_s.rowptr), _ptr(csr_s.col), _ptr(csr_s.perm), _ptr(csr_s.items), csr_s.n_items,
            _ptr(csr_s.splits), csr_s.n_splits, H, _storage(G, dQ, dK), _ptr(mask), _ptr(G), _ld(G, H),
            _ptr(in_norm), _ptr(out_norm), AGG[agg], act, float(slope), _ptr(dQ), _ld(dQ, H), _ptr(dK), _ld(dK, H),
            _ptr(partial), _ptr(partial_s), _drop(drop), _stream(dQ.device))
    _check(rc, lib)


def edge_e_agg_fwd(csr, Q, K, Eh, eidx, norm_row, norm_col, agg, act, slope, S, partial, mask_out=None):
    lib = load()
    H = S.shape[1]
    if eidx is not None and not (eidx.dtype == torch.int32 and eidx.is_contiguous() and eidx.numel() == csr.col.numel()):
        raise ValueError("eidx must be a contiguous int32 tensor with one entry per edge")
    with _Timed("sir_edge_e_agg_fwd", S.device):
        rc = lib.sir_edge_e_agg_fwd(
            _ptr(csr.rowptr), _ptr(csr.col), _ptr(csr.items), csr.n_items, _ptr(csr.splits), csr.n_splits,
            H, _storage(Q, K, Eh, S), _ptr(Q), _ld(Q, H), _ptr(K), _ld(K, H), _ptr(Eh), _ld(Eh, H), Eh.shape[0],
            _ptr(eidx), _ptr(norm_row), _ptr(norm_col), AGG[agg], act, float(slope), _ptr(S), _ld(S, H),
            _ptr(mask_out), _ptr(partial), _stream(S.device))
    _check(rc, lib)


def edge_e_bwd(csr, mask, G, norm_row, norm_col, agg, act, slope, eidx, dE):
    lib = load()
    H = dE.shape[1]
    if eidx is not None and not (eidx.dtype == torch.int32 and eidx.is_contiguous() and eidx.numel() == csr.col.numel()):
        raise ValueError("eidx must be a contiguous int32 tensor with one entry per edge")
    with _Timed("sir_edge_e_bwd", dE.device):
        rc = lib.sir_edge_e_bwd(
            _ptr(csr.rowptr), _ptr(csr.col), _ptr(csr.items), csr.n_items, H, _storage(G, dE), _ptr(mask),
            _ptr(G), _ld(G, H), _ptr(norm_row), _ptr(norm_col), AGG[agg], act, float(slope), _ptr(eidx),
            dE.shape[0], _ptr(dE), _ld(dE, H), _stream(dE.device))
    _check(rc, lib)


def edge_gather_add(csr, Q, K, Z):
    lib = load()
    F = Z.shape[1]
    with _Timed("sir_edge_gather_add", Z.device):
        rc = lib.sir_edge_gather_add(_ptr(csr.rowptr), _ptr(csr.col), _ptr(csr.items), csr.n_items, F,
                                     _ptr(Q), _ld(Q, F), _ptr(K), _ld(K, F), _ptr(Z), _ld(Z, F), _stream(Z.device))
    _check(rc, lib)


def edge_gather_act(csr, Q, K, act, slope, A, sign_mask=None):
    lib = load()
    F = A.shape[1]
    with _Timed("sir_edge_gather_act", A.device):
        rc = lib.sir_edge_gather_act(_ptr(csr.rowptr), _ptr(csr.col), _ptr(csr.items), csr.n_items, F,
                                     _ptr(Q), _ld(Q, F), _ptr(K), _ld(K, F), int(act), float(slope), _ptr(A),
                                     _ld(A, F), _ptr(sign_mask), _stream(A.device))
    _check(rc, lib)


def segment_sum(csr, X, out, norm_row=None, norm_col=None, mean=False, perm=None, partial=None):
    lib = load()
    F = out.shape[1]
    with _Timed("sir_segment_sum", out.device):
        rc = lib.sir_segment_sum(_ptr(csr.rowptr), _ptr(csr.col), _ptr(perm), _ptr(csr.items), csr.n_items,
                                 _ptr(csr.splits), csr.n_splits, F, _ptr(X), _ld(X, F), _ptr(norm_row),
                                 _ptr(norm_col), int(bool(mean)), _ptr(out), _ld(out, F), _ptr(partial),
                                 _stream(out.device))
    _check(rc, lib)


def edge_broadcast(csr, dS, dM, norm_row=None, norm_col=None, mean=False):
    lib = load()
    F = dM.shape[1]
    with _Timed("sir_edge_broadcast", dM.device):
        rc = lib.sir_edge_broadcast(_ptr(csr.rowptr), _ptr(csr.col), _ptr(csr.items), csr.n_items, F,
                                    _ptr(dS), _ld(dS, F), _ptr(norm_row), _ptr(norm_col), int(bool(mean)),
                                    _ptr(dM), _ld(dM, F), _stream(dM.device))
    _check(rc, lib)


def segment_max(csr, M, Y, arg, pval=None, parg=None):
    lib = load()
    F = Y.shape[1]
    with _Timed("sir_segment_max", Y.device):
        rc = lib.sir_segment_max(_ptr(csr.items), csr.n_items, _ptr(csr.splits), csr.n_splits, F,
                                 _ptr(M), _ld(M, F), _ptr(Y), _ld(Y, F), _ptr(arg), _ld(arg, F),
                                 _ptr(pval), _ptr(parg), _stream(Y.device))
    _check(rc, lib)


def segment_max_bwd(csr, arg, dY, dM):
    lib = load()
    F = dM.shape[1]
    with _Timed("sir_segment_max_bwd", dM.device):
        rc = lib.sir_segment_max_bwd(_ptr(csr.items), csr.n_items, F, _ptr(arg), _ld(arg, F),
                                     _ptr(dY), _ld(dY, F), _ptr(dM), _ld(dM, F), _stream(dM.device))
    _check(rc, lib)


def csr_build(rows, cols, n_rows, n_cols, chunk):
    lib = load()
    dev = rows.device
    E = rows.numel()
    rows = rows.to(torch.int64).contiguous()
    cols = cols.to(torch.int64).contiguous()
    ws_bytes = lib.sir_csr_build_workspace(n_rows, E)
    if ws_bytes < 0:
        raise RuntimeError("sir_csr_build_workspace failed (sizes out of range or no device)")
    ws = torch.empty((ws_bytes,), dtype=torch.uint8, device=dev)
    rowptr = torch.empty((n_rows + 1,), dtype=torch.int32, device=dev)
    col = torch.empty((E,), dtype=torch.int32, device=dev)
    eid = torch.empty((E,), dtype=torch.int64, device=dev)
    items = torch.empty((n_rows + E // chunk + 1, 4), dtype=torch.int32, device=dev)
    splits = torch.empty((min(n_rows, E // (chunk + 1)) + 1, 4), dtype=torch.int32, device=dev)
    counts = torch.empty((5,), dtype=torch.int64, device=dev)
    with _Timed("sir_csr_build", dev):
        rc = lib.sir_csr_build(_ptr(rows), _ptr(cols), E, n_rows, n_cols, chunk, _ptr(rowptr), _ptr(col),
                               _ptr(eid), _ptr(items), _ptr(splits), _ptr(counts), _ptr(ws), ws_bytes,
                               _stream(dev))
    _check(rc, lib)
    return rowptr, col, eid, items, splits, counts


def csr_perm(eid_a, eid_b):
    lib = load()
    E = eid_a.numel()
    pos = torch.empty((E,), dtype=torch.int32, device=eid_a.device)
    perm = torch.empty((E,), dtype=torch.int32, device=eid_a.device)
    rc = lib.sir_csr_perm(_ptr(eid_a), _ptr(eid_b), E, _ptr(pos), _ptr(perm), _stream(eid_a.device))
    _check(rc, lib)
    return perm


def graph_norm_fwd(off, X, weight, bias, mean_scale, eps, Y, mean, std):
    lib = load()
    B, F = mean.shape
    with _Timed("sir_graph_norm_fwd", Y.device):
        rc = lib.sir_graph_norm_fwd(_ptr(off), B, F, _ptr(X), _ld(X, F), _ptr(weight), _ptr(bias),
                                    _ptr(mean_scale), float(eps), _ptr(Y), _ld(Y, F), _ptr(mean), _ptr(std),
                                    _stream(Y.device))
    _check(rc, lib)


_DT_CODE = {torch.float32: 0, torch.bfloat16: 1, torch.float16: 2}


def resid_act_fwd(Y, R, act, slope, order, out):
    lib = load()
    M, N = Y.shape
    with _Timed("sir_resid_act_fwd", out.device):
        rc = lib.sir_resid_act_fwd(_ptr(Y), Y.stride(0), _DT_CODE[Y.dtype], _ptr(R), R.stride(0), _ptr(out),
                                   out.stride(0), M, N, int(act), float(slope), int(order), _stream(out.device))
    _check(rc, lib)


def resid_act_bwd(D, Y, R, act, slope, order, dY, dR=None, D2=None):
    lib = load()
    M, N = Y.shape
    with _Timed("sir_resid_act_bwd", dY.device):
        rc = lib.sir_resid_act_bwd(_ptr(D), D.stride(0), _ptr(D2), D2.stride(0) if D2 is not None else 0,
                                   _ptr(Y), Y.stride(0), _DT_CODE[Y.dtype], _ptr(R),
                                   R.stride(0) if R is not None else 0, _ptr(dY), dY.stride(0), _ptr(dR),
# ... 358 lines not shown
```

sir-gcn_amd/sirgcn/conv.py:

```python
import torch
from torch import nn
import torch.nn.functional as F

from . import _native, linalg
from .graph import DEFAULT_CHUNK, get_plan


QK_TRACE = None


def _trace_qk(QK):
    if QK_TRACE is not None:
        QK_TRACE.append(QK.detach().clone())


def activation_code(act):
    if isinstance(act, nn.LeakyReLU):
        return _native.ACT_LEAKY, float(act.negative_slope)
    if isinstance(act, nn.ReLU) or act in (torch.relu, F.relu):
        return _native.ACT_RELU, 0.0
    if isinstance(act, nn.GELU):
        return (_native.ACT_GELU_TANH if act.approximate == "tanh" else _native.ACT_GELU), 0.0
    if act is F.gelu:
        return _native.ACT_GELU, 0.0
    if isinstance(act, nn.Identity) or act is None:
        return _native.ACT_IDENTITY, 0.0
    if act is F.leaky_relu:
        return _native.ACT_LEAKY, 0.01
    raise NotImplementedError(
        f"SIRConv: activation {act!r} has no native kernel (supported: ReLU, LeakyReLU, GELU, Identity)")


def _storage_dtype(dtype, H):
    if dtype in (torch.bfloat16, torch.float16) and H % 4 == 0:
        return dtype
    return torch.float32


class EdgeAggregate(torch.autograd.Function):

    use_mask = True
    dual = True

    @staticmethod
    def forward(ctx, QK, plan, H, agg, act, slope, grad_on=True):
        if QK.device.type != "cuda":
            raise RuntimeError("SIRConv native path needs a ROCm GPU tensor (no CPU fallback)")
        ctx.in_dtype = QK.dtype
        st = _storage_dtype(QK.dtype, H)
        QK = QK.contiguous().to(st)
        V = QK.shape[0]
        Q, K = QK[:, :H], QK[:, H:]
        in_norm, out_norm = plan.norms(agg)
        S = torch.empty((V, H), device=QK.device, dtype=st)
        partial = _partial(plan, H, QK.device)
        nw = _native.mask_words(H, act) if EdgeAggregate.use_mask else 0
        mask = None
        if nw and grad_on and QK.requires_grad:
            mask = torch.empty((max(plan.dst.col.numel(), 1) * nw,), device=QK.device, dtype=torch.int64)
        _native.edge_agg_fwd(plan.dst, Q, K, in_norm, out_norm, agg, act, slope, S, partial, mask)
        if mask is not None:
            ctx.save_for_backward(mask)
        else:
            ctx.save_for_backward(QK)
        ctx.masked = mask is not None
        ctx.plan, ctx.H, ctx.agg, ctx.act, ctx.slope, ctx.V, ctx.st = plan, H, agg, act, slope, V, st
        return S

    @staticmethod
    def backward(ctx, dS):
        (saved,) = ctx.saved_tensors
        plan, H, agg, act, slope, V, st = ctx.plan, ctx.H, ctx.agg, ctx.act, ctx.slope, ctx.V, ctx.st
        G = dS.contiguous().to(st)
        dQK = torch.empty((V, 2 * H), device=G.device, dtype=st)
        if ctx.masked:
            Q = K = None
            mask = saved
        else:
            Q, K = saved[:, :H], saved[:, H:]
            mask = None
        edge_backward(plan, H, agg, act, slope, G, Q, K, mask, dQK)
        return dQK.to(ctx.in_dtype), None, None, None, None, None, None


def _partial(plan, H, device):
    n = max(plan.dst.n_slots, plan.src.n_slots)
    return torch.empty((max(n, 1) * H,), device=device, dtype=torch.float32) if n else None


def _slots(csr, H, device):
    return torch.empty((csr.n_slots * H,), device=device, dtype=torch.float32) if csr.n_slots else None


def edge_backward(plan, H, agg, act, slope, G, Q, K, mask, dQK, drop=None):
    in_norm, out_norm = plan.norms(agg)
    if mask is not None and EdgeAggregate.dual:
        if agg == "mean":
            deg = plan.in_degree_f()
            G = torch.div(G, deg, out=torch.empty_like(G))
            agg = "sum"
        _native.edge_agg_bwd(plan.dst, plan.src, G, mask, in_norm, out_norm, agg, act, slope, dQK[:, :H],
                             dQK[:, H:], _slots(plan.dst, H, G.device), _slots(plan.src, H, G.device), drop=drop)
        return
    partial = _partial(plan, H, G.device)
    Gm = torch.empty((G.shape[0], H), device=G.device, dtype=G.dtype) if agg == "mean" else None
    _native.edge_agg_bwd_dst(plan.dst, Q, K, G, in_norm, out_norm, agg, act, slope, dQK[:, :H], Gm, partial, mask,
                             drop=drop)
    _native.edge_agg_bwd_src(plan.src, K, Q, Gm if Gm is not None else G, out_norm, in_norm,
                             agg, act, slope, dQK[:, H:], partial, mask, drop=drop)


_tn = linalg.mm_tn


def _bias_grad(G):
    if (G.is_cuda and G.shape[1] % 4 == 0 and G.stride(1) == 1 and G.stride(0) % 4 == 0
            and G.data_ptr() % 16 == 0):
        return _native.col_sum(G)
    return G.sum(0)


def _weight_and_bias_grad(G, X, need_w, need_b):
    if need_w and need_b:
        return _tn(G, X, colsum=True)
    if need_w:
        return _tn(G, X), None
    return None, (_bias_grad(G) if need_b else None)


def _weight_and_bias_grad16(G, X, need_w, need_b):
    if need_w:
        return linalg.mm_tn16(G, X, colsum=True) if need_b else (linalg.mm_tn16(G, X), None)
    return None, (_bias_grad(G.float()) if need_b else None)


class SIRConvFunction(torch.autograd.Function):

    @staticmethod
    def forward(ctx, X, W_Q, b_Q, W_K, W_R, b_R, plan, agg, act, slope, grad_on=True, drop=None):
        H = W_Q.shape[0]
        X = X.contiguous()
        QK = linalg.mm_wt_pair(X, W_Q, W_K, b_Q, drop=drop)
        _trace_qk(QK)
        V = QK.shape[0]
        in_norm, out_norm = plan.norms(agg)
        S = torch.empty((V, H), device=X.device, dtype=torch.float32)
        partial = _partial(plan, H, X.device)
        training = grad_on and any(ctx.needs_input_grad[:6])
        nw = _native.mask_words(H, act) if (EdgeAggregate.use_mask and training) else 0
        mask = torch.empty((max(plan.dst.col.numel(), 1) * nw,), device=X.device, dtype=torch.int64) if nw else None
        _native.edge_agg_fwd(plan.dst, QK[:, :H], QK[:, H:], in_norm, out_norm, agg, act, slope, S, partial, mask)
        Y = linalg.mm_wt(S, W_R, b_R)
        ctx.save_for_backward(X, W_Q, W_K, W_R, S, mask if mask is not None else QK)
        ctx.masked = mask is not None
        ctx.plan, ctx.agg, ctx.act, ctx.slope, ctx.drop = plan, agg, act, slope, drop
        ctx.has_bq, ctx.has_br = b_Q is not None, b_R is not None
        return Y

    @staticmethod
    def backward(ctx, dY):
        X, W_Q, W_K, W_R, S, saved = ctx.saved_tensors
        plan, agg, act, slope = ctx.plan, ctx.agg, ctx.act, ctx.slope
        H = W_R.shape[1]
        V = X.shape[0]
        dY = dY.contiguous()
        G = linalg.mm_w(dY, W_R)
        dW_R, db_R = _weight_and_bias_grad(dY, S, ctx.needs_input_grad[4], ctx.has_br and ctx.needs_input_grad[5])
        if ctx.masked:
            Q = K = None
            mask = saved
        else:
            Q, K = saved[:, :H], saved[:, H:]
            mask = None
        dQK = torch.empty((V, 2 * H), device=X.device, dtype=torch.float32)
        edge_backward(plan, H, agg, act, slope, G, Q, K, mask, dQK, ctx.drop)
        dX = linalg.mm_w_pair(dQK, W_Q, W_K) if ctx.needs_input_grad[0] else None
        dW_Q = dW_K = db_Q = None
        need_bq = ctx.has_bq and ctx.needs_input_grad[2]
        if ctx.needs_input_grad[1] or ctx.needs_input_grad[3]:
            dW, cs = _weight_and_bias_grad(dQK, X, True, need_bq)
            dW_Q, dW_K = dW[:H], dW[H:]
            db_Q = cs[:H] if need_bq else None
        elif need_bq:
            db_Q = _bias_grad(dQK[:, :H])
        return dX, dW_Q, db_Q, dW_K, dW_R, db_R, None, None, None, None, None, None


class SIRConvFunction16(torch.autograd.Function):

    @staticmethod
    def forward(ctx, X, W_Q, b_Q, W_K, W_R, b_R, plan, agg, act, slope, grad_on, dt, drop=None):
        H = W_Q.shape[0]
        W_cat = torch.cat([W_Q, W_K], 0)
        b_cat = F.pad(b_Q, (0, H)) if b_Q is not None else None
        X = X.contiguous()
        if X.dtype == dt:
            Xh = X
            QK = linalg.mm16_wt(X, W_cat, b_cat, dt, drop=drop)
        else:
            Xh = torch.empty(X.shape, dtype=dt, device=X.device)
            QK = linalg.mm16_wt(X, W_cat, b_cat, dt, acopy=Xh, drop=drop)
        _trace_qk(QK)
        V = QK.shape[0]
        in_norm, out_norm = plan.norms(agg)
        S = torch.empty((V, H), device=X.device, dtype=dt)
        partial = _partial(plan, H, X.device)
        training = grad_on and any(ctx.needs_input_grad[:6])
        nw = _native.mask_words(H, act) if (EdgeAggregate.use_mask and training) else 0
        mask = torch.empty((max(plan.dst.col.numel(), 1) * nw,), device=X.device, dtype=torch.int64) if nw else None
        _native.edge_agg_fwd(plan.dst, QK[:, :H], QK[:, H:], in_norm, out_norm, agg, act, slope, S, partial, mask)
        Y = linalg.mm16_wt(S, W_R, b_R, dt)
        ctx.save_for_backward(Xh, W_cat, W_R, S, mask if mask is not None else QK)
        ctx.masked = mask is not None
        ctx.plan, ctx.agg, ctx.act, ctx.slope, ctx.x_dtype, ctx.dt, ctx.drop = plan, agg, act, slope, X.dtype, dt, drop
        ctx.has_bq, ctx.has_br = b_Q is not None, b_R is not None
        return Y

    @staticmethod
    def backward(ctx, dY):
        Xh, W_cat, W_R, S, saved = ctx.saved_tensors
        plan, agg, act, slope, dt = ctx.plan, ctx.agg, ctx.act, ctx.slope, ctx.dt
        H = W_R.shape[1]
        V = Xh.shape[0]
        dY = dY.contiguous().to(dt)
        G = linalg.mm16_w(dY, W_R, dt)
        dW_R = db_R = None
        if ctx.needs_input_grad[4] or ctx.needs_input_grad[5]:
            dW_R, db_R = _weight_and_bias_grad16(dY, S, ctx.needs_input_grad[4],
                                                 ctx.has_br and ctx.needs_input_grad[5])
        if ctx.masked:
            Q = K = None
            mask = saved
        else:
            Q, K = saved[:, :H], saved[:, H:]
            mask = None
        dQK = torch.empty((V, 2 * H), device=Xh.device, dtype=dt)
        edge_backward(plan, H, agg, act, slope, G, Q, K, mask, dQK, ctx.drop)
        dX = linalg.mm16_w(dQK, W_cat, dt, out_dtype=ctx.x_dtype) if ctx.needs_input_grad[0] else None
        dW_Q = dW_K = db_Q = None
        need_bq = ctx.has_bq and ctx.needs_input_grad[2]
        if ctx.needs_input_grad[1] or ctx.needs_input_grad[3] or need_bq:
            dW, cs = _weight_and_bias_grad16(dQK, Xh, True, need_bq)
            dW_Q, dW_K = dW[:H], dW[H:]
            db_Q = cs[:H] if need_bq else None
        return dX, dW_Q, db_Q, dW_K, dW_R, db_R, None, None, None, None, None, None, None


class SIRConv(nn.Module):

    use_fused = True
    fuse_edge_mlp = True
    native_linear = True

    def __init__(self, input_dim, hidden_dim, output_dim, activation, dropout=0, inner_bias=True,
                 outer_bias=True, agg_type='sum'):
        super().__init__()
        if agg_type not in ("sum", "mean", "sym", "max"):
            raise AttributeError(f"module 'dgl.function' has no attribute '{agg_type}'")
        self.activation = activation
        self.dropout = nn.Dropout(dropout)
        self.linear_query = nn.Linear(input_dim, hidden_dim, bias=inner_bias)
        self.linear_key = nn.Linear(input_dim, hidden_dim, bias=False)
        self.linear_relation = nn.Linear(hidden_dim, output_dim, bias=outer_bias)
        self._agg_type = agg_type
        self.chunk = DEFAULT_CHUNK
        self.step_seed = None

    def _drop(self, device):
        if not (self.training and self.dropout.p > 0):
            self.step_seed = None
            return None
        seed, self.step_seed = self.step_seed, None
        if seed is None or seed.device != torch.device(device):
            seed = torch.randint(0, 2 ** 62, (1,), device=device, dtype=torch.int64)
        return seed, float(self.dropout.p)

    def _linear(self, x, W, b):
        if self.native_linear:
            return linalg.linear(x, W, b)
        return F.linear(x, W, b)

    def _relation(self, S):
        lin = self.linear_relation
        if type(lin) is nn.Linear:
            return self._linear(S, lin.weight, lin.bias)
        return lin(S)

    def _project(self, feat_key, feat_query):
        H = self.linear_query.out_features
        if feat_key is feat_query:
            W = torch.cat([self.linear_query.weight, self.linear_key.weight], 0)
            b = None
            if self.linear_query.bias is not None:
                b = torch.cat([self.linear_query.bias, self.linear_query.bias.new_zeros(H)])
            QK = self._linear(feat_query, W, b)
        else:
            QK = torch.cat([self._linear(feat_query, self.linear_query.weight, self.linear_query.bias),
                            self._linear(feat_key, self.linear_key.weight, None)], 1)
        if self.training and self.dropout.p > 0:
            QK = self.dropout(QK)
        _trace_qk(QK)
        return QK

    def forward(self, graph, feat):
        try:
            return self._forward(graph, feat)
        finally:
            self.step_seed = None

    def _forward(self, graph, feat):
        if isinstance(feat, tuple):
            feat_key, feat_query = feat
        else:
            feat_key = feat_query = feat
        if feat_query.dim() != 2:
            raise ValueError("SIRConv expects 2-D node features [V, input_dim]")
        if feat_query.device.type != "cuda":
            raise RuntimeError("SIRConv native path needs a ROCm GPU tensor (no CPU fallback)")
        plan = get_plan(graph, feat_query.device, self.chunk)
        if plan.num_nodes != feat_query.shape[0]:
            raise ValueError(f"feat has {feat_query.shape[0]} rows, graph has {plan.num_nodes} nodes")
        try:
            act, slope = activation_code(self.activation)
        except NotImplementedError:
            act = None
        H = self.linear_query.out_features
        if self.fuse_edge_mlp and feat_query.dtype != torch.float64:
            from .edgemlp import EdgeMaxLinear, EdgeMLPSum, max_supported, seq_sigma
# ... 49 lines not shown
```

sir-gcn_amd/sirgcn/graph.py:

```python
import contextlib
import weakref
from dataclasses import dataclass
from typing import Optional

import torch

DEFAULT_CHUNK = 256


class Graph:

    def __init__(self, src, dst, num_nodes=None, batch_num_nodes=None):
        src = torch.as_tensor(src, dtype=torch.int64)
        dst = torch.as_tensor(dst, dtype=torch.int64)
        if src.shape != dst.shape or src.dim() != 1:
            raise ValueError("src and dst must be 1-D and of equal length")
        if num_nodes is None:
            num_nodes = int(max(src.max().item(), dst.max().item()) + 1) if src.numel() else 0
        self._src, self._dst, self._n = src, dst.to(src.device), int(num_nodes)
        if batch_num_nodes is None:
            batch_num_nodes = [self._n]
        self._bnn = torch.as_tensor(batch_num_nodes, dtype=torch.int64)
        if int(self._bnn.sum()) != self._n:
            raise ValueError("batch_num_nodes must sum to num_nodes")
        self.ndata, self.edata = {}, {}
        self._plans = {}

    def num_nodes(self):
        return self._n

    def num_edges(self):
        return int(self._src.numel())

    number_of_nodes = num_nodes
    number_of_edges = num_edges

    @property
    def device(self):
        return self._src.device

    def edges(self):
        return self._src, self._dst

    def in_degrees(self):
        return torch.bincount(self._dst, minlength=self._n)

    def out_degrees(self):
        return torch.bincount(self._src, minlength=self._n)

    def to(self, device):
        return Graph(self._src.to(device), self._dst.to(device), self._n, self._bnn)

    def batch_num_nodes(self):
        return self._bnn

    @property
    def batch_size(self):
        return int(self._bnn.numel())

    @contextlib.contextmanager
    def local_scope(self):
        nd, ed = dict(self.ndata), dict(self.edata)
        try:
            yield
        finally:
            self.ndata, self.edata = nd, ed

    def __repr__(self):
        return f"Graph(num_nodes={self._n}, num_edges={self.num_edges()}, device={self.device})"


def batch(graphs):
    offs, src, dst, bnn = 0, [], [], []
    for g in graphs:
        s_, d_ = g.edges()
        src.append(torch.as_tensor(s_, dtype=torch.int64) + offs)
        dst.append(torch.as_tensor(d_, dtype=torch.int64) + offs)
        n = int(g.num_nodes())
        bnn.append(n)
        offs += n
    if not graphs:
        return Graph(torch.zeros(0, dtype=torch.int64), torch.zeros(0, dtype=torch.int64), 0, [])
    return Graph(torch.cat(src), torch.cat(dst), offs, bnn)


def node_offsets(graph, device):
    cache = getattr(graph, "_plans", None)
    key = ("offsets", str(device))
    if cache is not None and key in cache:
        return cache[key]
    bnn = torch.as_tensor(graph.batch_num_nodes(), dtype=torch.int64).to(device)
    off = torch.zeros(bnn.numel() + 1, dtype=torch.int64, device=device)
    torch.cumsum(bnn, 0, out=off[1:])
    if cache is not None:
        cache[key] = off
    return off


@dataclass
class RowCSR:
    n_rows: int
    rowptr: torch.Tensor
    col: torch.Tensor
    eid: torch.Tensor
    items: torch.Tensor
    splits: Optional[torch.Tensor]
    n_items: int
    n_splits: int
    n_slots: int
    max_degree: int
    perm: Optional[torch.Tensor] = None


def build_row_csr(rows, cols, n_rows, chunk=DEFAULT_CHUNK):
    rows = rows.to(torch.int64)
    E = rows.numel()
    if E >= 2 ** 31 - 1:
        raise ValueError("int32 edge indices: E must be < 2^31")
    dev = rows.device
    if E:
        _, eid = torch.sort(rows, stable=True)
    else:
        eid = torch.zeros(0, dtype=torch.int64, device=dev)
    col = cols.to(torch.int64)[eid].to(torch.int32)
    deg = torch.bincount(rows, minlength=n_rows) if E else torch.zeros(n_rows, dtype=torch.int64, device=dev)
    rowptr = torch.zeros(n_rows + 1, dtype=torch.int64, device=dev)
    torch.cumsum(deg, 0, out=rowptr[1:])
    return plan_from_rowptr(rowptr, col, eid, n_rows, chunk)


def plan_from_rowptr(rowptr, col, eid, n_rows, chunk=DEFAULT_CHUNK):
    dev = rowptr.device
    rowptr = rowptr.to(torch.int64)
    deg = rowptr[1:] - rowptr[:-1]
    nch = torch.clamp((deg + chunk - 1) // chunk, min=1)
    n_items = int(nch.sum().item()) if n_rows else 0
    row_of = torch.repeat_interleave(torch.arange(n_rows, device=dev), nch)
    first = torch.cumsum(nch, 0) - nch
    k = torch.arange(n_items, device=dev) - first[row_of]
    eb = rowptr[row_of] + k * chunk
    ee = torch.minimum(eb + chunk, rowptr[row_of + 1])
    split_row = nch > 1
    split_item = split_row[row_of]
    slot = torch.full((n_items,), -1, dtype=torch.int64, device=dev)
    n_slots = int(split_item.sum().item()) if n_items else 0
    if n_slots:
        slot[split_item] = torch.arange(n_slots, device=dev)
    items = torch.stack([row_of, eb, ee, slot], 1).to(torch.int32).contiguous()
    srows = torch.nonzero(split_row).flatten()
    n_splits = int(srows.numel())
    splits = None
    if n_splits:
        s_n = nch[srows]
        s_begin = torch.cumsum(s_n, 0) - s_n
        splits = torch.stack([srows, s_begin, s_n, deg[srows]], 1).to(torch.int32).contiguous()
    return RowCSR(n_rows=n_rows, rowptr=rowptr.to(torch.int32).contiguous(), col=col.contiguous(),
                  eid=eid, items=items, splits=splits, n_items=n_items, n_splits=n_splits,
                  n_slots=n_slots, max_degree=int(deg.max().item()) if n_rows else 0)


def build_plans_native(src, dst, n_dst_rows, n_src_rows, chunk=DEFAULT_CHUNK):
    from . import _native
    E = src.numel()
    if E >= 2 ** 31 - 1:
        raise ValueError("int32 edge indices: E must be < 2^31")
    d = _native.csr_build(dst, src, n_dst_rows, n_src_rows, chunk)
    s = _native.csr_build(src, dst, n_src_rows, n_dst_rows, chunk)
    perm = _native.csr_perm(d[2], s[2])
    counts = torch.stack([d[5], s[5]]).cpu().tolist()
    if counts[0][4] or counts[1][4]:
        raise ValueError(f"edge endpoint out of range: {counts[0][4]} bad edges "
                         f"(dst must be in [0, {n_dst_rows}), src in [0, {n_src_rows}))")
    csrs = []
    for (rowptr, col, eid, items, splits, _), cnt, n in ((d, counts[0], n_dst_rows), (s, counts[1], n_src_rows)):
        n_items, n_splits, n_slots, max_deg = cnt[:4]
        csrs.append(RowCSR(n_rows=n, rowptr=rowptr, col=col, eid=eid, items=items[:n_items],
                           splits=splits[:n_splits] if n_splits else None, n_items=n_items,
                           n_splits=n_splits, n_slots=n_slots, max_degree=max_deg))
    csrs[1].perm = perm
    return csrs[0], csrs[1]


class GraphPlan:

    def __init__(self, src, dst, num_nodes, device, chunk=DEFAULT_CHUNK, csc=None):
        self.num_nodes = int(num_nodes)
        self.device = torch.device(device)
        src = src.to(self.device, torch.int64)
        dst = dst.to(self.device, torch.int64)
        self.num_edges = int(src.numel())
        if self.device.type == "cuda" and csc is None:
            self.dst, self.src = build_plans_native(src, dst, self.num_nodes, self.num_nodes, chunk)
        else:
            if self.num_edges:
                lo = int(torch.minimum(src.min(), dst.min()).item())
                hi = int(torch.maximum(src.max(), dst.max()).item())
                if lo < 0 or hi >= self.num_nodes:
                    raise ValueError(f"edge endpoint out of range [0, {self.num_nodes}): min {lo}, max {hi}")
            if csc is not None:
                indptr, indices, eids = (t.to(self.device) for t in csc)
                self.dst = plan_from_rowptr(indptr, indices.to(torch.int32), eids.to(torch.int64),
                                            self.num_nodes, chunk)
            else:
                self.dst = build_row_csr(dst, src, self.num_nodes, chunk)
            self.src = build_row_csr(src, dst, self.num_nodes, chunk)
            pos_in_dst = torch.empty(self.num_edges, dtype=torch.int64, device=self.device)
            pos_in_dst[self.dst.eid] = torch.arange(self.num_edges, device=self.device)
            self.src.perm = pos_in_dst[self.src.eid].to(torch.int32).contiguous()
        self.in_deg = (self.dst.rowptr[1:] - self.dst.rowptr[:-1]).to(torch.int64)
        self.out_deg = (self.src.rowptr[1:] - self.src.rowptr[:-1]).to(torch.int64)
        self._norms = {}

    def norms(self, agg):
        if agg != "sym":
            return None, None
        if "sym" not in self._norms:
            if self.device.type == "cuda":
                from . import _native
                in_norm = torch.empty(self.num_nodes, dtype=torch.float32, device=self.device)
                out_norm = torch.empty_like(in_norm)
                _native.degree_norms(self.dst.rowptr, self.src.rowptr, in_norm, out_norm)
            else:
                in_norm = torch.pow(self.in_deg.float().clamp(min=1), -0.5).contiguous()
                out_norm = torch.pow(self.out_deg.float().clamp(min=1), -0.5).contiguous()
            self._norms["sym"] = (in_norm, out_norm)
        return self._norms["sym"]

    def in_degree_f(self):
        if "deg" not in self._norms:
            rp = self.dst.rowptr
            self._norms["deg"] = (rp[1:] - rp[:-1]).clamp(min=1).to(torch.float32)[:, None]
        return self._norms["deg"]


_weak_plans = weakref.WeakKeyDictionary()


def get_plan(graph, device, chunk=DEFAULT_CHUNK):
    device = torch.device(device)
    key = (str(device), chunk)
    cache = getattr(graph, "_plans", None)
    if cache is None:
        try:
            cache = _weak_plans.setdefault(graph, {})
        except TypeError:
            cache = {}
    plan = cache.get(key)
    if plan is not None:
        return plan
    n = int(graph.num_nodes())
    csc = None
    if hasattr(graph, "adj_tensors"):
        csc = graph.adj_tensors("csc")
    src, dst = graph.edges()
    plan = GraphPlan(torch.as_tensor(src), torch.as_tensor(dst), n, device, chunk, csc=csc)
    cache[key] = plan
    return plan
```

Before: 1.980 billion edges/s.

## Add degree-based cache policy for gathered rows and nontemporal streaming

Adds a per-graph gather policy that encodes high-degree neighbors as hot (non-negative index) and cold ones as bitwise-negated indices in a packed col array. Hot rows are gathered with normal cached buffer loads and cold rows with a streaming cache-policy flag. Self rows, outputs and sign-mask stores use nontemporal loads and stores. The aim is to keep the most reused neighbor rows resident in cache on a large power-law graph. It costs a one-time build of the packed column array per plan and adds a code path that is restricted to fp32, H=256/512, SUM/SYM and ReLU/LeakyReLU with the sign mask.

New measurement: 1.989 billion edges/s (median of 2 runs). No clear change (+0.4%).

```diff
diff --git a/include/sirconv.h b/include/sirconv.h
--- a/include/sirconv.h
+++ b/include/sirconv.h
@@ -9,7 +9,7 @@
 
 #define SIR_ABI_VERSION 17
 
-enum { SIR_AGG_SUM = 0, SIR_AGG_MEAN = 1, SIR_AGG_SYM = 2, SIR_AGG_ACCUMULATE = 16 };
+enum { SIR_AGG_SUM = 0, SIR_AGG_MEAN = 1, SIR_AGG_SYM = 2, SIR_AGG_ACCUMULATE = 16, SIR_AGG_COLPOL = 32 };
 enum { SIR_ACT_IDENTITY = 0, SIR_ACT_RELU = 1, SIR_ACT_LEAKY_RELU = 2, SIR_ACT_GELU = 3, SIR_ACT_GELU_TANH = 4 };
 enum { SIR_DTYPE_F32 = 0, SIR_DTYPE_BF16 = 1, SIR_DTYPE_F16 = 2 };
 enum { SIR_OK = 0, SIR_EINVAL = 1, SIR_EUNSUPPORTED = 2, SIR_ELAUNCH = 3 };
diff --git a/sir-gcn_amd/csrc/sirconv_abi.cpp b/sir-gcn_amd/csrc/sirconv_abi.cpp
--- a/sir-gcn_amd/csrc/sirconv_abi.cpp
+++ b/sir-gcn_amd/csrc/sirconv_abi.cpp
@@ -36,6 +36,16 @@
     return SIR_OK;
 }
 
+int check_colpol(const char* fn, int64_t H, int dtype, int agg, int act, bool masked) {
+    if (dtype != SIR_DTYPE_F32) return fail(SIR_EUNSUPPORTED, fn, "SIR_AGG_COLPOL: SIR_DTYPE_F32 rows only");
+    if (H != 256 && H != 512) return fail(SIR_EUNSUPPORTED, fn, "SIR_AGG_COLPOL: H must be 256 or 512");
+    if (agg != SIR_AGG_SUM && agg != SIR_AGG_SYM) return fail(SIR_EUNSUPPORTED, fn, "SIR_AGG_COLPOL: SUM / SYM only");
+    if (act != SIR_ACT_RELU && act != SIR_ACT_LEAKY_RELU)
+        return fail(SIR_EUNSUPPORTED, fn, "SIR_AGG_COLPOL: act RELU / LEAKY_RELU only");
+    if (!masked) return fail(SIR_EUNSUPPORTED, fn, "SIR_AGG_COLPOL: sign-mask mode only (the recompute mode takes plain col)");
+    return SIR_OK;
+}
+
 int check_mask(const char* fn, int64_t H, int act) {
     if (sir_mask_words(H, act) == 0)
         return fail(SIR_EUNSUPPORTED, fn, "sign mask needs act RELU/LEAKY_RELU, H % 4 == 0 and H <= 1024");
@@ -111,15 +121,19 @@
                      void* S, int64_t lds, uint64_t* mask_out, float* partial, void* stream) {
     const char* fn = "sir_edge_agg_fwd";
     const int accumulate = (agg & SIR_AGG_ACCUMULATE) != 0;
-    agg &= ~SIR_AGG_ACCUMULATE;
+    const int colpol = (agg & SIR_AGG_COLPOL) != 0;
+    agg &= ~(SIR_AGG_ACCUMULATE | SIR_AGG_COLPOL);
     if (accumulate && agg == SIR_AGG_MEAN)
         return fail(SIR_EUNSUPPORTED, fn, "SIR_AGG_ACCUMULATE: segment sums of SUM / SYM only (divide afterwards for MEAN)");
+    if (colpol && accumulate)
+        return fail(SIR_EUNSUPPORTED, fn, "SIR_AGG_COLPOL: not with SIR_AGG_ACCUMULATE (segmented forward)");
     int rc = check_common(fn, rowptr, col, items, n_items, splits, n_splits, H, dtype, agg, act,
                           norm_row, norm_col, S, partial);
     if (rc) return rc;
     if (ldq < H || ldk < H || lds < H) return fail(SIR_EINVAL, fn, "leading dimensions must be >= H");
     if (n_items > 0 && (Q == nullptr || K == nullptr)) return fail(SIR_EINVAL, fn, "Q/K must be non-NULL");
     if (mask_out != nullptr && (rc = check_mask(fn, H, act))) return rc;
+    if (colpol && (rc = check_colpol(fn, H, dtype, agg, act, mask_out != nullptr))) return rc;
     sir::EdgeArgs a{};
     a.rowptr = rowptr; a.col = col; a.items = items; a.n_items = n_items;
     a.R = Q; a.ldr = ldq;
@@ -129,6 +143,7 @@
     a.out = S; a.ldo = lds; a.partial = partial; a.Gm = nullptr; a.ldgm = H;
     a.mask_out = mask_out;
     a.accumulate = accumulate;
+    a.colpol = colpol;
     const char* why = nullptr;
     hipError_t err = sir::run_edge(sir::MODE_FWD, dtype, a, agg, act, splits, n_splits, S, lds,
                                    agg == SIR_AGG_MEAN, static_cast<hipStream_t>(stream), &why);
@@ -186,6 +201,8 @@
                          int agg, int act, float slope,
                          void* dK, int64_t lddk, float* partial, const sir_dropout_t* drop, void* stream) {
     const char* fn = "sir_edge_agg_bwd_src";
+    const int colpol = (agg & SIR_AGG_COLPOL) != 0;
+    agg &= ~SIR_AGG_COLPOL;
     int rc = check_common(fn, rowptr_s, col_s, items, n_items, splits, n_splits, H, dtype, agg, act,
                           norm_row, norm_col, dK, partial);
     if (rc) return rc;
@@ -198,6 +215,7 @@
         if (ldq < H || ldk < H) return fail(SIR_EINVAL, fn, "leading dimensions must be >= H");
         if (n_items > 0 && (Q == nullptr || K == nullptr)) return fail(SIR_EINVAL, fn, "K/Q must be non-NULL");
     }
+    if (colpol && (rc = check_colpol(fn, H, dtype, agg, act, mask != nullptr))) return rc;
     sir::EdgeArgs a{};
     a.rowptr = rowptr_s; a.col = col_s; a.items = items; a.n_items = n_items;
     a.R = K; a.ldr = mask ? H : ldk;
@@ -206,6 +224,7 @@
     a.norm_row = norm_row; a.norm_col = norm_col; a.slope = slope; a.H = (int)H;
     a.out = dK; a.ldo = lddk; a.partial = partial; a.Gm = nullptr; a.ldgm = H;
     a.mask_in = mask; a.perm = perm_s;
+    a.colpol = colpol;
     a.drop = to_drop(drop, H);
     const char* why = nullptr;
     hipError_t err = sir::run_edge(sir::MODE_BWD_SRC, dtype, a, agg, act, splits, n_splits, dK, lddk, false,
@@ -222,6 +241,8 @@
                      void* dQ, int64_t lddq, void* dK, int64_t lddk, float* partial, float* partial_s,
                      const sir_dropout_t* drop, void* stream) {
     const char* fn = "sir_edge_agg_bwd";
+    const int colpol = (agg & SIR_AGG_COLPOL) != 0;
+    agg &= ~SIR_AGG_COLPOL;
     int rc = check_common(fn, rowptr, col, items, n_items, splits, n_splits, H, dtype, agg, act, in_norm, out_norm,
                           dQ, partial);
     if (rc) return rc;
@@ -232,6 +253,7 @@
         return fail(SIR_EUNSUPPORTED, fn, "MEAN: the source pass needs the destination pass's Gm (two calls)");
     if (mask == nullptr) return fail(SIR_EINVAL, fn, "the one-launch backward is the sign-mask mode: mask required");
     if ((rc = check_mask(fn, H, act))) return rc;
+    if (colpol && (rc = check_colpol(fn, H, dtype, agg, act, true))) return rc;
     if (ldg < H || lddq < H || lddk < H) return fail(SIR_EINVAL, fn, "leading dimensions must be >= H");
     if ((n_items > 0 || n_items_s > 0) && G == nullptr) return fail(SIR_EINVAL, fn, "G must be non-NULL");
     if (n_items_s > 0 && col_s != nullptr && perm_s == nullptr) return fail(SIR_EINVAL, fn, "sign-mask mode needs perm_s");
@@ -247,6 +269,7 @@
     b.out = dK; b.ldo = lddk; b.partial = partial_s; b.mask_in = mask; b.ldr = H; b.ldc = H; b.ldgm = H;
     a.drop = to_drop(drop, 0);
     b.drop = to_drop(drop, H);
+    b.colpol = colpol;
     const char* why = nullptr;
     hipError_t err = sir::run_edge_dual(dtype, a, splits, n_splits, b, splits_s, n_splits_s, agg, act,
                                         static_cast<hipStream_t>(stream), &why);
diff --git a/sir-gcn_amd/csrc/sirconv_dispatch.hip b/sir-gcn_amd/csrc/sirconv_dispatch.hip
--- a/sir-gcn_amd/csrc/sirconv_dispatch.hip
+++ b/sir-gcn_amd/csrc/sirconv_dispatch.hip
@@ -154,6 +154,12 @@
     return s->nv <= 4;
 }
 
+static const char* const kColpolWhy =
+    "SIR_AGG_COLPOL: fp32 rows, H = 256 or 512, 16-B aligned rows, sign-mask mode, SUM / SYM only";
+static bool colpol_shape(int dtype, int H, const Shape& s) {
+    return dtype == ST_F32 && s.vw == 4 && s.lpr == 64 && (H == 256 || H == 512);
+}
+
 hipError_t run_edge(int mode, int dtype, const EdgeArgs& a, int agg, int act,
                     const int32_t* splits, int64_t n_splits, void* out_final, int64_t ld_final,
                     bool mean_div, hipStream_t st, const char** why) {
@@ -171,6 +177,13 @@
         *why = "bf16/fp16 storage needs H % 4 == 0 and 8-B aligned rows (leading dimensions multiples of 4)";
         return hipErrorInvalidValue;
     }
+    if (a.colpol) {
+        const bool masked = (mode == MODE_FWD) ? a.mask_out != nullptr : (mode == MODE_BWD_SRC && a.mask_in != nullptr);
+        if (!colpol_shape(dtype, a.H, s) || !masked || agg == AGG_MEAN || a.accumulate) {
+            *why = kColpolWhy;
+            return hipErrorInvalidValue;
+        }
+    }
     switch (dtype) {
         case ST_BF16: return run_edge_t<ST_BF16>(mode, a, agg, act, s, splits, n_splits, out_final, ld_final, mean_div, st);
         case ST_F16: return run_edge_t<ST_F16>(mode, a, agg, act, s, splits, n_splits, out_final, ld_final, mean_div, st);
@@ -190,6 +203,10 @@
         *why = "the sign-mask backward needs H % 4 == 0, H <= 1024 and aligned rows";
         return hipErrorInvalidValue;
     }
+    if (a.colpol || (b.colpol && !colpol_shape(dtype, a.H, s))) {
+        *why = kColpolWhy;
+        return hipErrorInvalidValue;
+    }
     hipError_t err;
     switch (dtype) {
         case ST_BF16: err = launch_edge_dual<ST_BF16>(a, b, agg, act, s, st); break;
diff --git a/sir-gcn_amd/csrc/sirconv_edge_impl.h b/sir-gcn_amd/csrc/sirconv_edge_impl.h
--- a/sir-gcn_amd/csrc/sirconv_edge_impl.h
+++ b/sir-gcn_amd/csrc/sirconv_edge_impl.h
@@ -140,20 +140,49 @@
     }
 }
 
-template <int ST, int VW>
-__device__ __forceinline__ void vload_row(float (&d)[VW], const typename Stor<ST>::T* __restrict__ p) { tload_p<ST, VW>(d, p); }
-template <int ST, int VW>
-__device__ __forceinline__ void vstore_row(typename Stor<ST>::T* __restrict__ p, const float (&s)[VW]) { tstore_p<ST, VW>(p, s); }
+typedef float sir_f4 __attribute__((ext_vector_type(4)));
+template <int ST, int VW, bool NT = false>
+__device__ __forceinline__ void vload_row(float (&d)[VW], const typename Stor<ST>::T* __restrict__ p) {
+    if constexpr (NT) {
+        static_assert(ST == ST_F32 && VW == 4, "nt streams: fp32 float4 rows");
+        const sir_f4 t = __builtin_nontemporal_load(reinterpret_cast<const sir_f4*>(p));
+        d[0] = t.x; d[1] = t.y; d[2] = t.z; d[3] = t.w;
+    } else {
+        tload_p<ST, VW>(d, p);
+    }
+}
+template <int ST, int VW, bool NT = false>
+__device__ __forceinline__ void vstore_row(typename Stor<ST>::T* __restrict__ p, const float (&s)[VW]) {
+    if constexpr (NT) {
+        static_assert(ST == ST_F32 && VW == 4, "nt streams: fp32 float4 rows");
+        sir_f4 t;
+        t.x = s[0]; t.y = s[1]; t.z = s[2]; t.w = s[3];
+        __builtin_nontemporal_store(t, reinterpret_cast<sir_f4*>(p));
+    } else {
+        tstore_p<ST, VW>(p, s);
+    }
+}
 template <int ST, int VW>
 __device__ __forceinline__ void vload_gather(float (&d)[VW], const typename Stor<ST>::T* __restrict__ p) { tload_p<ST, VW>(d, p); }
 
+__device__ __forceinline__ int pol_decode(int packed, bool& hot) {
+    hot = packed >= 0;
+    return hot ? packed : ~packed;
+}
+__device__ __forceinline__ sir_u4 pol_load(gemm::rsrc_t rs, int off, bool hot) {
+    sir_u4 t;
+    if (hot) t = __builtin_amdgcn_raw_buffer_load_b128(rs, off, 0, 0);
+    else t = __builtin_amdgcn_raw_buffer_load_b128(rs, off, 0, 2);
+    return t;
+}
+
 __device__ __forceinline__ void writelane(uint32_t& v, uint32_t x, int k) {
     asm("v_writelane_b32 %0, %1, %2" : "+v"(v) : "s"(x), "i"(k));
 }
 
 template <int LPR, int VW> constexpr int sub_mask_words() { return LPR * VW >= 64 ? LPR * VW / 32 : 2; }
 
-template <int ST, int MODE, int ACT, int AGG, int LPR, int NV, int VW, int UU, int MK>
+template <int ST, int MODE, int ACT, int AGG, int LPR, int NV, int VW, int UU, int MK, bool POL = false>
 __device__ __forceinline__ void edge_batch(int e, const int* __restrict__ col,
                                            const typename Stor<ST>::T* __restrict__ C, int64_t ldc,
                                            const typename Stor<ST>::T* __restrict__ G, int64_t ldg,
@@ -169,6 +198,12 @@
 #pragma unroll
     for (int i = 0; i < UU; ++i) u[i] = (upre != nullptr) ? upre[i] : col[e + i];
     constexpr bool kBufGather = MODE == MODE_FWD && ST == ST_F32 && VW == 4 && LPR == 64 && MASKW;
+    static_assert(!POL || kBufGather, "gather policy: the fp32 full-wave sign-mask forward");
+    bool hot[POL ? UU : 1];
+    if constexpr (POL) {
+#pragma unroll
+        for (int i = 0; i < UU; ++i) u[i] = pol_decode(__builtin_amdgcn_readfirstlane(u[i]), hot[i]);
+    }
     constexpr int MWS = sub_mask_words<LPR, VW>();
     uint32_t mr[MASKR ? UU : 1][MWS];
     if constexpr (MASKR) {
@@ -200,7 +235,9 @@
             const gemm::rsrc_t rs = gemm::mk_rsrc(cp, (uint32_t)(HC * 16));
 #pragma unroll
             for (int j = 0; j < NV; ++j) {
-                const sir_u4 t = __builtin_amdgcn_raw_buffer_load_b128(rs, (li + LPR * j) * 16, 0, 0);
+                sir_u4 t;
+                if constexpr (POL) t = pol_load(rs, (li + LPR * j) * 16, hot[i]);
+                else t = __builtin_amdgcn_raw_buffer_load_b128(rs, (li + LPR * j) * 16, 0, 0);
                 cv[i][j][0] = __uint_as_float(t.x); cv[i][j][1] = __uint_as_float(t.y);
                 cv[i][j][2] = __uint_as_float(t.z); cv[i][j][3] = __uint_as_float(t.w);
             }
@@ -274,7 +311,8 @@
         }
         const uint64_t mine = ((uint64_t)mhi << 32) | mlo;
         if (lane < UU * NW) {
-            mask[(int64_t)e * NW + lane] = mine;
+            if constexpr (POL) __builtin_nontemporal_store(mine, &mask[(int64_t)e * NW + lane]);
+            else mask[(int64_t)e * NW + lane] = mine;
         }
     }
 #pragma unroll
@@ -313,7 +351,7 @@
     }
 }
 
-template <int ST, int MODE, int ACT, int AGG, int LPR, int NV, int VW, int U, int MK>
+template <int ST, int MODE, int ACT, int AGG, int LPR, int NV, int VW, int U, int MK, bool POL = false>
 __device__ __forceinline__ void
 edge_wave(int64_t wave, const int* __restrict__ rowptr, const int* __restrict__ col, const int* __restrict__ perm,
           const int4* __restrict__ items, int64_t n_items,
@@ -352,7 +390,7 @@
         const int c = li + LPR * j;
 #pragma unroll
         for (int w = 0; w < VW; ++w) { acc[j][w] = 0.f; rv[j][w] = 0.f; gv[j][w] = 0.f; }
-        if (MKB != 2 && c < HC) vload_row<ST, VW>(rv[j], rp + c * VW);
+        if (MKB != 2 && c < HC) vload_row<ST, VW, POL>(rv[j], rp + c * VW);
     }
     if constexpr (MODE == MODE_BWD_DST) {
         const auto* gp = G + (int64_t)row * ldg;
@@ -393,35 +431,35 @@
 #pragma unroll
                 for (int i = 0; i < U; ++i) uc[i] = __builtin_amdgcn_readlane(vc, i);
                 vc = load_col(e + U);
-                edge_batch<ST, MODE, ACT, AGG, LPR, NV, VW, U, MKB>(e, col, C, ldc, G, ldg, norm_col, nr, slope, li, HC,
+                edge_batch<ST, MODE, ACT, AGG, LPR, NV, VW, U, MKB, POL>(e, col, C, ldc, G, ldg, norm_col, nr, slope, li, HC,
                                                                   rv, gv, acc, mask, lane, uc, perm);
             }
         }
     } else {
         for (; e + U <= e1; e += U)
-            edge_batch<ST, MODE, ACT, AGG, LPR, NV, VW, U, MKB>(e, col, C, ldc, G, ldg, norm_col, nr, slope, li, HC, rv, gv,
+            edge_batch<ST, MODE, ACT, AGG, LPR, NV, VW, U, MKB, POL>(e, col, C, ldc, G, ldg, norm_col, nr, slope, li, HC, rv, gv,
                                                               acc, mask, lane, nullptr, perm);
     }
     if constexpr (U > 8) {
         if (e + 8 <= e1) {
-            edge_batch<ST, MODE, ACT, AGG, LPR, NV, VW, 8, MKB>(e, col, C, ldc, G, ldg, norm_col, nr, slope, li, HC, rv, gv, acc, mask, lane, nullptr, perm);
+            edge_batch<ST, MODE, ACT, AGG, LPR, NV, VW, 8, MKB, POL>(e, col, C, ldc, G, ldg, norm_col, nr, slope, li, HC, rv, gv, acc, mask, lane, nullptr, perm);
             e += 8;
         }
     }
     if constexpr (U > 4) {
         if (e + 4 <= e1) {
-            edge_batch<ST, MODE, ACT, AGG, LPR, NV, VW, 4, MKB>(e, col, C, ldc, G, ldg, norm_col, nr, slope, li, HC, rv, gv, acc, mask, lane, nullptr, perm);
+            edge_batch<ST, MODE, ACT, AGG, LPR, NV, VW, 4, MKB, POL>(e, col, C, ldc, G, ldg, norm_col, nr, slope, li, HC, rv, gv, acc, mask, lane, nullptr, perm);
             e += 4;
         }
     }
     if constexpr (U > 2) {
         if (e + 2 <= e1) {
-            edge_batch<ST, MODE, ACT, AGG, LPR, NV, VW, 2, MKB>(e, col, C, ldc, G, ldg, norm_col, nr, slope, li, HC, rv, gv, acc, mask, lane, nullptr, perm);
+            edge_batch<ST, MODE, ACT, AGG, LPR, NV, VW, 2, MKB, POL>(e, col, C, ldc, G, ldg, norm_col, nr, slope, li, HC, rv, gv, acc, mask, lane, nullptr, perm);
             e += 2;
         }
     }
     if (e < e1)
-        edge_batch<ST, MODE, ACT, AGG, LPR, NV, VW, 1, MKB>(e, col, C, ldc, G, ldg, norm_col, nr, slope, li, HC, rv, gv, acc, mask, lane, nullptr, perm);
+        edge_batch<ST, MODE, ACT, AGG, LPR, NV, VW, 1, MKB, POL>(e, col, C, ldc, G, ldg, norm_col, nr, slope, li, HC, rv, gv, acc, mask, lane, nullptr, perm);
 
     if (slot < 0) {
         if constexpr (MODE == MODE_FWD && AGG == AGG_MEAN) {
@@ -455,7 +493,7 @@
 #pragma unroll
         for (int j = 0; j < NV; ++j) {
             const int c = li + LPR * j;
-            if (c < HC) vstore_row<ST, VW>(op + c * VW, acc[j]);
+            if (c < HC) vstore_row<ST, VW, POL>(op + c * VW, acc[j]);
         }
     } else {
         float* pp = partial + (int64_t)slot * H;
@@ -486,6 +524,20 @@
                                                      drop, accumulate);
 }
 
+template <int ACT, int AGG, int NV, int U>
+__global__ void __launch_bounds__(256)
+k_edge_pol(const int* __restrict__ rowptr, const int* __restrict__ col,
+           const int4* __restrict__ items, int64_t n_items,
+           const float* __restrict__ R, int64_t ldr, const float* __restrict__ C, int64_t ldc,
+           const float* __restrict__ norm_row, const float* __restrict__ norm_col,
+           float slope, int H, float* __restrict__ out, int64_t ldo, float* __restrict__ partial,
+           uint64_t* __restrict__ mask) {
+    const int64_t wave = __builtin_amdgcn_readfirstlane((int)((int64_t)blockIdx.x * (blockDim.x >> 6) + (threadIdx.x >> 6)));
+    edge_wave<ST_F32, MODE_FWD, ACT, AGG, 64, NV, 4, U, 1, true>(wave, rowptr, col, nullptr, items, n_items, R, ldr, C,
+                                                                ldc, nullptr, H, norm_row, norm_col, slope, H, out, ldo,
+                                                                partial, nullptr, H, mask, Drop(), 0);
+}
+
 __device__ __forceinline__ uint64_t uniform64(uint64_t x) {
     const uint32_t lo = __builtin_amdgcn_readfirstlane((uint32_t)x);
     const uint32_t hi = __builtin_amdgcn_readfirstlane((uint32_t)(x >> 32));
@@ -507,7 +559,7 @@
 
 template <int UU> struct EdgeIdx { int v[UU]; int p[UU]; };
 
-template <int ST, int MODE, int ACT, int AGG, int NV, int UU, bool PRE = false, bool PIDX = false>
+template <int ST, int MODE, int ACT, int AGG, int NV, int UU, bool PRE = false, bool PIDX = false, bool POL = false>
 __device__ __forceinline__ void mask_batch(int e, const int* __restrict__ col, const int* __restrict__ perm,
                                            const typename Stor<ST>::T* __restrict__ G, int64_t ldg,
                                            const uint64_t* __restrict__ mask,
@@ -531,6 +583,13 @@
             if constexpr (AGG == AGG_SYM && !PRE) v[i] = __builtin_amdgcn_readfirstlane(col[e + i]);
         }
     }
+    constexpr bool kPolGather = POL && MODE == MODE_BWD_SRC;
+    static_assert(!kPolGather || ST == ST_F32, "gather policy: fp32 rows");
+    bool hot[kPolGather ? UU : 1];
+    if constexpr (kPolGather) {
+#pragma unroll
+        for (int i = 0; i < UU; ++i) v[i] = pol_decode(v[i], hot[i]);
+    }
     uint64_t wd[UU][NW];
     if constexpr (PRE) {
         const int mlo = (int)(uint32_t)pre, mhi = (int)(uint32_t)(pre >> 32);
@@ -573,10 +632,20 @@
 #pragma unroll
         for (int i = 0; i < UU; ++i) {
             const auto* gp = G + (int64_t)v[i] * ldg;
-#pragma unroll
-            for (int j = 0; j < NV; ++j) {
-                const int c = lane + 64 * j;
-                vload_gather<ST, 4>(gc[i][j], gp + (c < HC ? c : 0) * 4);
+            if constexpr (kPolGather) {
+                const gemm::rsrc_t rs = gemm::mk_rsrc(gp, (uint32_t)(HC * 16));
+#pragma unroll
+                for (int j = 0; j < NV; ++j) {
+                    const sir_u4 t = pol_load(rs, (lane + 64 * j) * 16, hot[i]);
+                    gc[i][j][0] = __uint_as_float(t.x); gc[i][j][1] = __uint_as_float(t.y);
+                    gc[i][j][2] = __uint_as_float(t.z); gc[i][j][3] = __uint_as_float(t.w);
+                }
+            } else {
+#pragma unroll
+                for (int j = 0; j < NV; ++j) {
+                    const int c = lane + 64 * j;
+                    vload_gather<ST, 4>(gc[i][j], gp + (c < HC ? c : 0) * 4);
+                }
             }
         }
     }
@@ -599,7 +668,7 @@
     }
 }
 
-template <int ST, int MODE, int ACT, int AGG, int NV, int U>
+template <int ST, int MODE, int ACT, int AGG, int NV, int U, bool POL = false>
 __device__ __forceinline__ void mask_item(int e0, int e1, const int* __restrict__ col, const int* __restrict__ perm,
                                           const typename Stor<ST>::T* __restrict__ G, int64_t ldg,
                                           const uint64_t* __restrict__ mask,
@@ -624,34 +693,34 @@
                     cur.p[i] = __builtin_amdgcn_readlane(pc, i);
                 }
                 load_idx(e + U, vc, pc);
-                mask_batch<ST, MODE, ACT, AGG, NV, U, false, true>(e, col, perm, G, ldg, mask, norm_col, nr, slope, lane,
+                mask_batch<ST, MODE, ACT, AGG, NV, U, false, true, POL>(e, col, perm, G, ldg, mask, norm_col, nr, slope, lane,
                                                                    HC, gv, acc, 0, 0, 0.f, 0, &cur);
             }
         }
     } else {
         for (; e + U <= e1; e += U)
-            mask_batch<ST, MODE, ACT, AGG, NV, U>(e, col, perm, G, ldg, mask, norm_col, nr, slope, lane, HC, gv, acc);
+            mask_batch<ST, MODE, ACT, AGG, NV, U, false, false, POL>(e, col, perm, G, ldg, mask, norm_col, nr, slope, lane, HC, gv, acc);
     }
     if constexpr (U > 8) {
         if (e + 8 <= e1) {
-            mask_batch<ST, MODE, ACT, AGG, NV, 8>(e, col, perm, G, ldg, mask, norm_col, nr, slope, lane, HC, gv, acc);
+            mask_batch<ST, MODE, ACT, AGG, NV, 8, false, false, POL>(e, col, perm, G, ldg, mask, norm_col, nr, slope, lane, HC, gv, acc);
             e += 8;
         }
     }
     if constexpr (U > 4) {
         if (e + 4 <= e1) {
-            mask_batch<ST, MODE, ACT, AGG, NV, 4>(e, col, perm, G, ldg, mask, norm_col, nr, slope, lane, HC, gv, acc);
+            mask_batch<ST, MODE, ACT, AGG, NV, 4, false, false, POL>(e, col, perm, G, ldg, mask, norm_col, nr, slope, lane, HC, gv, acc);
             e += 4;
         }
     }
     if constexpr (U > 2) {
         if (e + 2 <= e1) {
-            mask_batch<ST, MODE, ACT, AGG, NV, 2>(e, col, perm, G, ldg, mask, norm_col, nr, slope, lane, HC, gv, acc);
+            mask_batch<ST, MODE, ACT, AGG, NV, 2, false, false, POL>(e, col, perm, G, ldg, mask, norm_col, nr, slope, lane, HC, gv, acc);
             e += 2;
         }
     }
     if (e < e1)
-        mask_batch<ST, MODE, ACT, AGG, NV, 1>(e, col, perm, G, ldg, mask, norm_col, nr, slope, lane, HC, gv, acc);
+        mask_batch<ST, MODE, ACT, AGG, NV, 1, false, false, POL>(e, col, perm, G, ldg, mask, norm_col, nr, slope, lane, HC, gv, acc);
 }
 
 
@@ -728,7 +797,7 @@
     return it;
 }
 
-template <int ST, int MODE, int ACT, int AGG, int NV, int U>
+template <int ST, int MODE, int ACT, int AGG, int NV, int U, bool POL = false>
 __device__ __forceinline__ void
 mask_pass_item(int64_t wave, const int* __restrict__ rowptr, const int* __restrict__ col, const int* __restrict__ perm,
                const int4* __restrict__ items,
@@ -760,7 +829,7 @@
         for (int j = 0; j < NV; ++j) {
             const int c = lane + 64 * j;
             if (c < HC) {
-                vload_row<ST, 4>(gv[j], gp + c * 4);
+                vload_row<ST, 4, POL>(gv[j], gp + c * 4);
                 if constexpr (AGG == AGG_MEAN) {
 #pragma unroll
                     for (int w = 0; w < 4; ++w) gv[j][w] = round_st<ST>(gv[j][w] / degf);
@@ -774,7 +843,7 @@
     if constexpr (MODE == MODE_BWD_DST)
         mask_item_dst_wide<ST, ACT, AGG, NV>(e0, e1, col, mask, norm_col, nr, slope, lane, HC, gv, acc);
     else
-        mask_item<ST, MODE, ACT, AGG, NV, U>(e0, e1, col, perm, G, ldg, mask, norm_col, nr, slope, lane, HC, gv, acc);
+        mask_item<ST, MODE, ACT, AGG, NV, U, POL>(e0, e1, col, perm, G, ldg, mask, norm_col, nr, slope, lane, HC, gv, acc);
     if (slot < 0) {
         auto* op = out + (int64_t)row * ldo;
         if (drop.on()) {
@@ -784,7 +853,7 @@
 #pragma unroll
         for (int j = 0; j < NV; ++j) {
             const int c = lane + 64 * j;
-            if (c < HC) vstore_row<ST, 4>(op + c * 4, acc[j]);
+            if (c < HC) vstore_row<ST, 4, POL>(op + c * 4, acc[j]);
         }
     } else {
         float* op = partial + (int64_t)slot * H;
@@ -844,6 +913,55 @@
         mask_pass_item<ST, MODE_BWD_SRC, ACT, AGG, NV, US>(idx, rowptr_s, col_s, perm_s, items_s, G, ldg, mask,
                                                            out_norm, in_norm, slope, H, dK, lddk, partial_s, nullptr, H,
                                                            drop_k);
+}
+
+template <int ACT, int AGG, int NV, int U>
+__global__ void __launch_bounds__(256)
+k_edge_mask_src_pol(const int* __restrict__ rowptr, const int* __restrict__ col, const int* __restrict__ perm,
+                    const int4* __restrict__ items, int64_t n_items, const float* __restrict__ G, int64_t ldg,
+                    const uint64_t* __restrict__ mask, const float* __restrict__ norm_row,
+                    const float* __restrict__ norm_col, float slope, int H, float* __restrict__ out, int64_t ldo,
+                    float* __restrict__ partial, Drop drop) {
+    drop = drop_resolve(drop);
+    const int64_t wave = __builtin_amdgcn_readfirstlane((int)((int64_t)blockIdx.x * (blockDim.x >> 6) + (threadIdx.x >> 6)));
+    if (wave >= n_items) return;
+    mask_pass_item<ST_F32, MODE_BWD_SRC, ACT, AGG, NV, U, true>(wave, rowptr, col, perm, items, G, ldg, mask, norm_row,
+                                                               norm_col, slope, H, out, ldo, partial, nullptr, H, drop);
+}
+
+template <int ACT, int AGG, int NV, int UD, int US, bool DR>
+__global__ void __launch_bounds__(256)
+k_edge_mask_dual_pol(const int* __restrict__ rowptr, const int* __restrict__ col, const int4* __restrict__ items,
+                     int64_t n_items, float* __restrict__ partial, float* __restrict__ dQ, int64_t lddq,
+                     const int* __restrict__ rowptr_s, const int* __restrict__ col_s, const int* __restrict__ perm_s,
+                     const int4* __restrict__ items_s, int64_t n_items_s, float* __restrict__ partial_s,
+                     float* __restrict__ dK, int64_t lddk, const float* __restrict__ G, int64_t ldg,
+                     const uint64_t* __restrict__ mask, const float* __restrict__ in_norm,
+                     const float* __restrict__ out_norm, float slope, int H, Drop drop_q, Drop drop_k) {
+    if constexpr (DR) {
+        drop_q = drop_resolve(drop_q);
+        drop_k = drop_resolve(drop_k);
+    }
+    const int64_t w = __builtin_amdgcn_readfirstlane((int)((int64_t)blockIdx.x * (blockDim.x >> 6) + (threadIdx.x >> 6)));
+    const int64_t nmin = n_items < n_items_s ? n_items : n_items_s;
+    bool dst;
+    int64_t idx;
+    if (w < 2 * nmin) {
+        dst = (w & 1) == 0;
+        idx = w >> 1;
+    } else {
+        dst = n_items > n_items_s;
+        idx = nmin + (w - 2 * nmin);
+        if (idx >= (dst ? n_items : n_items_s)) return;
+    }
+    if (dst)
+        mask_pass_item<ST_F32, MODE_BWD_DST, ACT, AGG, NV, UD, true>(idx, rowptr, col, nullptr, items, G, ldg, mask,
+                                                                    in_norm, out_norm, slope, H, dQ, lddq, partial,
+                                                                    nullptr, H, drop_q);
+    else
+        mask_pass_item<ST_F32, MODE_BWD_SRC, ACT, AGG, NV, US, true>(idx, rowptr_s, col_s, perm_s, items_s, G, ldg, mask,
+                                                                    out_norm, in_norm, slope, H, dK, lddk, partial_s,
+                                                                    nullptr, H, drop_k);
 }
 
 #ifndef SIR_COMBINE_PF
@@ -956,6 +1074,18 @@
     if (blocks == 0) return hipSuccess;
     constexpr bool kReluFamily = (ACT == ACT_RELU || ACT == ACT_LEAKY) && VW == 4 && (LPR == 64 || NV == 1);
     constexpr bool kMaskable = (MODE == MODE_FWD) && kReluFamily;
+    if (a.colpol) {
+        if constexpr (kMaskable && ST == ST_F32 && LPR == 64 && NV <= 2 && AGG != AGG_MEAN) {
+            if (a.mask_out == nullptr || a.accumulate) return hipErrorInvalidValue;
+            hipLaunchKernelGGL((k_edge_pol<ACT, AGG, NV, U>), dim3((unsigned)blocks), dim3(256), 0, st, a.rowptr, a.col,
+                               reinterpret_cast<const int4*>(a.items), a.n_items, cp_<ST>(a.R), a.ldr, cp_<ST>(a.C),
+                               a.ldc, a.norm_row, a.norm_col, a.slope, a.H, mp_<ST>(a.out), a.ldo, a.partial,
+                               a.mask_out);
+            return hipGetLastError();
+        } else {
+            return hipErrorInvalidValue;
+        }
+    }
     if constexpr (kMaskable) {
         if (a.mask_out != nullptr) {
 #define SIR_EDGE_FWD_MASK(MKV)                                                                                       \
@@ -1004,6 +1134,17 @@
     constexpr int U = (NV == 1) ? unroll_of<MODE, ST>() : (NV == 2 ? 4 : 2);
     const int64_t blocks = (a.n_items + 3) / 4;
     if (blocks == 0) return hipSuccess;
+    if (a.colpol) {
+        if constexpr (ST == ST_F32 && MODE == MODE_BWD_SRC && NV <= 2 && AGG != AGG_MEAN) {
+            hipLaunchKernelGGL((k_edge_mask_src_pol<ACT, AGG, NV, U>), dim3((unsigned)blocks), dim3(256), 0, st,
+                               a.rowptr, a.col, a.perm, reinterpret_cast<const int4*>(a.items), a.n_items, cp_<ST>(a.G),
+                               a.ldg, a.mask_in, a.norm_row, a.norm_col, a.slope, a.H, mp_<ST>(a.out), a.ldo, a.partial,
+                               a.drop);
+            return hipGetLastError();
+        } else {
+            return hipErrorInvalidValue;
+        }
+    }
     hipLaunchKernelGGL((k_edge_mask<ST, MODE, ACT, AGG, NV, U>), dim3((unsigned)blocks), dim3(256), 0, st,
                        a.rowptr, a.col, a.perm, reinterpret_cast<const int4*>(a.items), a.n_items,
                        cp_<ST>(a.G), a.ldg, a.mask_in, a.norm_row, a.norm_col, a.slope, a.H,
@@ -1024,6 +1165,23 @@
                        b.rowptr, b.col, b.perm, reinterpret_cast<const int4*>(b.items), b.n_items, b.partial,      \
                        mp_<ST>(b.out), b.ldo, cp_<ST>(a.G), a.ldg, a.mask_in, a.norm_row, a.norm_col, a.slope, a.H, \
                        a.drop, b.drop)
+    if (a.colpol) return hipErrorInvalidValue;
+    if (b.colpol) {
+        if constexpr (ST == ST_F32 && NV <= 2) {
+#define SIR_DUAL_POL(DRV)                                                                                           \
+            hipLaunchKernelGGL((k_edge_mask_dual_pol<ACT, AGG, NV, UD, US, DRV>), dim3((unsigned)blocks), dim3(256), \
+                               0, st, a.rowptr, a.col, reinterpret_cast<const int4*>(a.items), a.n_items, a.partial, \
+                               mp_<ST>(a.out), a.ldo, b.rowptr, b.col, b.perm,                                      \
+                               reinterpret_cast<const int4*>(b.items), b.n_items, b.partial, mp_<ST>(b.out), b.ldo,  \
+                               cp_<ST>(a.G), a.ldg, a.mask_in, a.norm_row, a.norm_col, a.slope, a.H, a.drop, b.drop)
+            if (a.drop.sptr != nullptr || b.drop.sptr != nullptr) SIR_DUAL_POL(true);
+            else SIR_DUAL_POL(false);
+#undef SIR_DUAL_POL
+            return hipGetLastError();
+        } else {
+            return hipErrorInvalidValue;
+        }
+    }
     if (a.drop.sptr != nullptr || b.drop.sptr != nullptr) SIR_DUAL(true);
     else SIR_DUAL(false);
 #undef SIR_DUAL
@@ -1045,6 +1203,7 @@
     if (s.vw != 4 || (agg != AGG_SUM && agg != AGG_SYM) || (act != ACT_RELU && act != ACT_LEAKY))
         return hipErrorInvalidValue;
     if (s.lpr < 64) {
+        if (a.colpol || b.colpol) return hipErrorInvalidValue;
         hipError_t e2 = launch_edge_pass<ST, MODE_BWD_DST>(a, agg, act, s, st);
         if (e2 != hipSuccess) return e2;
         return launch_edge_pass<ST, MODE_BWD_SRC>(b, agg, act, s, st);
diff --git a/sir-gcn_amd/csrc/sirconv_internal.h b/sir-gcn_amd/csrc/sirconv_internal.h
--- a/sir-gcn_amd/csrc/sirconv_internal.h
+++ b/sir-gcn_amd/csrc/sirconv_internal.h
@@ -31,6 +31,7 @@
     const int* perm;
     Drop drop;
     int accumulate;
+    int colpol;
 };
 
 struct Shape {
diff --git a/sir-gcn_amd/sirgcn/_native.py b/sir-gcn_amd/sirgcn/_native.py
--- a/sir-gcn_amd/sirgcn/_native.py
+++ b/sir-gcn_amd/sirgcn/_native.py
@@ -276,16 +276,27 @@
 
 
 AGG_ACCUMULATE = 16
-
-
-def edge_agg_fwd(csr, Q, K, norm_row, norm_col, agg, act, slope, S, partial, mask_out=None, accumulate=False):
+AGG_COLPOL = 32
+
+
+def _col(csr, policy):
+    if policy is None:
+        return csr.col, 0
+    if policy.dtype != torch.int32 or policy.shape != csr.col.shape or not policy.is_contiguous():
+        raise RuntimeError("policy: a contiguous int32 array shaped like csr.col")
+    return policy, AGG_COLPOL
+
+
+def edge_agg_fwd(csr, Q, K, norm_row, norm_col, agg, act, slope, S, partial, mask_out=None, accumulate=False,
+                 policy=None):
     lib = load()
     H = S.shape[1]
+    col, pol = _col(csr, policy)
     with _Timed("sir_edge_agg_fwd", S.device):
         rc = lib.sir_edge_agg_fwd(
-            _ptr(csr.rowptr), _ptr(csr.col), _ptr(csr.items), csr.n_items, _ptr(csr.splits), csr.n_splits,
+            _ptr(csr.rowptr), _ptr(col), _ptr(csr.items), csr.n_items, _ptr(csr.splits), csr.n_splits,
             H, _storage(Q, K, S), _ptr(Q), _ld(Q, H), _ptr(K), _ld(K, H), _ptr(norm_row), _ptr(norm_col),
-            AGG[agg] | (AGG_ACCUMULATE if accumulate else 0), act, float(slope), _ptr(S), _ld(S, H),
+            AGG[agg] | (AGG_ACCUMULATE if accumulate else 0) | pol, act, float(slope), _ptr(S), _ld(S, H),
             _ptr(mask_out), _ptr(partial), _stream(S.device))
     _check(rc, lib)
 
@@ -302,28 +313,33 @@
     _check(rc, lib)
 
 
-def edge_agg_bwd_src(csr_s, K, Q, Gd, norm_row, norm_col, agg, act, slope, dK, partial, mask=None, drop=None):
+def edge_agg_bwd_src(csr_s, K, Q, Gd, norm_row, norm_col, agg, act, slope, dK, partial, mask=None, drop=None,
+                     policy=None):
     lib = load()
     H = dK.shape[1]
+    col, pol = _col(csr_s, policy)
     with _Timed("sir_edge_agg_bwd_src", dK.device):
         rc = lib.sir_edge_agg_bwd_src(
-            _ptr(csr_s.rowptr), _ptr(csr_s.col), _ptr(csr_s.perm if mask is not None else None),
+            _ptr(csr_s.rowptr), _ptr(col), _ptr(csr_s.perm if mask is not None else None),
             _ptr(csr_s.items), csr_s.n_items, _ptr(csr_s.splits), csr_s.n_splits, H, _storage(K, Q, Gd, dK),
             _ptr(K), _ldx(K, H), _ptr(Q), _ldx(Q, H), _ptr(mask), _ptr(Gd), _ld(Gd, H),
-            _ptr(norm_row), _ptr(norm_col), AGG[agg], act, float(slope),
+            _ptr(norm_row), _ptr(norm_col), AGG[agg] | pol, act, float(slope),
             _ptr(dK), _ld(dK, H), _ptr(partial), _drop(drop), _stream(dK.device))
     _check(rc, lib)
 
 
-def edge_agg_bwd(csr, csr_s, G, mask, in_norm, out_norm, agg, act, slope, dQ, dK, partial, partial_s, drop=None):
+def edge_agg_bwd(csr, csr_s, G, mask, in_norm, out_norm, agg, act, slope, dQ, dK, partial, partial_s, drop=None,
+                 policy=None):
     lib = load()
     H = dQ.shape[1]
+    col_s, pol = _col(csr_s, policy)
     with _Timed("sir_edge_agg_bwd", dQ.device):
         rc = lib.sir_edge_agg_bwd(
             _ptr(csr.rowptr), _ptr(csr.col), _ptr(csr.items), csr.n_items, _ptr(csr.splits), csr.n_splits,
-            _ptr(csr_s.rowptr), _ptr(csr_s.col), _ptr(csr_s.perm), _ptr(csr_s.items), csr_s.n_items,
+            _ptr(csr_s.rowptr), _ptr(col_s), _ptr(csr_s.perm), _ptr(csr_s.items), csr_s.n_items,
             _ptr(csr_s.splits), csr_s.n_splits, H, _storage(G, dQ, dK), _ptr(mask), _ptr(G), _ld(G, H),
-            _ptr(in_norm), _ptr(out_norm), AGG[agg], act, float(slope), _ptr(dQ), _ld(dQ, H), _ptr(dK), _ld(dK, H),
+            _ptr(in_norm), _ptr(out_norm), AGG[agg] | pol, act, float(slope), _ptr(dQ), _ld(dQ, H), _ptr(dK),
+            _ld(dK, H),
             _ptr(partial), _ptr(partial_s), _drop(drop), _stream(dQ.device))
     _check(rc, lib)
 
diff --git a/sir-gcn_amd/sirgcn/conv.py b/sir-gcn_amd/sirgcn/conv.py
--- a/sir-gcn_amd/sirgcn/conv.py
+++ b/sir-gcn_amd/sirgcn/conv.py
@@ -41,6 +41,7 @@
 
     use_mask = True
     dual = True
+    gather_policy = True
 
     @staticmethod
     def forward(ctx, QK, plan, H, agg, act, slope, grad_on=True):
@@ -58,7 +59,8 @@
         mask = None
         if nw and grad_on and QK.requires_grad:
             mask = torch.empty((max(plan.dst.col.numel(), 1) * nw,), device=QK.device, dtype=torch.int64)
-        _native.edge_agg_fwd(plan.dst, Q, K, in_norm, out_norm, agg, act, slope, S, partial, mask)
+        _native.edge_agg_fwd(plan.dst, Q, K, in_norm, out_norm, agg, act, slope, S, partial, mask,
+                             policy=_policy_col(plan, "dst", H, agg, act, st, mask is not None))
         if mask is not None:
             ctx.save_for_backward(mask)
         else:
@@ -79,8 +81,19 @@
         else:
             Q, K = saved[:, :H], saved[:, H:]
             mask = None
-        edge_backward(plan, H, agg, act, slope, G, Q, K, mask, dQK)
+        edge_backward(plan, H, agg, act, slope, G, Q, K, mask, dQK, policy=True)
         return dQK.to(ctx.in_dtype), None, None, None, None, None, None
+
+
+def _policy_col(plan, side, H, agg, act, dtype, masked):
+    if not (EdgeAggregate.gather_policy and masked and dtype == torch.float32 and H in (256, 512)
+            and agg == "sum" and act in (_native.ACT_RELU, _native.ACT_LEAKY)):
+        return None
+    fn = getattr(plan, "policy_col", None)
+    if fn is None:
+        return None
+    pol = fn(side, H * 4)
+    return None if pol is getattr(plan, side).col else pol
 
 
 def _partial(plan, H, device):
@@ -92,22 +105,25 @@
     return torch.empty((csr.n_slots * H,), device=device, dtype=torch.float32) if csr.n_slots else None
 
 
-def edge_backward(plan, H, agg, act, slope, G, Q, K, mask, dQK, drop=None):
+def edge_backward(plan, H, agg, act, slope, G, Q, K, mask, dQK, drop=None, policy=False):
     in_norm, out_norm = plan.norms(agg)
     if mask is not None and EdgeAggregate.dual:
         if agg == "mean":
             deg = plan.in_degree_f()
             G = torch.div(G, deg, out=torch.empty_like(G))
             agg = "sum"
+        pol = _policy_col(plan, "src", H, agg, act, G.dtype, True) if policy else None
         _native.edge_agg_bwd(plan.dst, plan.src, G, mask, in_norm, out_norm, agg, act, slope, dQK[:, :H],
-                             dQK[:, H:], _slots(plan.dst, H, G.device), _slots(plan.src, H, G.device), drop=drop)
+                             dQK[:, H:], _slots(plan.dst, H, G.device), _slots(plan.src, H, G.device), drop=drop,
+                             policy=pol)
         return
     partial = _partial(plan, H, G.device)
     Gm = torch.empty((G.shape[0], H), device=G.device, dtype=G.dtype) if agg == "mean" else None
     _native.edge_agg_bwd_dst(plan.dst, Q, K, G, in_norm, out_norm, agg, act, slope, dQK[:, :H], Gm, partial, mask,
                              drop=drop)
+    pol = _policy_col(plan, "src", H, agg, act, G.dtype, mask is not None) if policy else None
     _native.edge_agg_bwd_src(plan.src, K, Q, Gm if Gm is not None else G, out_norm, in_norm,
-                             agg, act, slope, dQK[:, H:], partial, mask, drop=drop)
+                             agg, act, slope, dQK[:, H:], partial, mask, drop=drop, policy=pol)
 
 
 _tn = linalg.mm_tn
@@ -149,7 +165,8 @@
         training = grad_on and any(ctx.needs_input_grad[:6])
         nw = _native.mask_words(H, act) if (EdgeAggregate.use_mask and training) else 0
         mask = torch.empty((max(plan.dst.col.numel(), 1) * nw,), device=X.device, dtype=torch.int64) if nw else None
-        _native.edge_agg_fwd(plan.dst, QK[:, :H], QK[:, H:], in_norm, out_norm, agg, act, slope, S, partial, mask)
+        _native.edge_agg_fwd(plan.dst, QK[:, :H], QK[:, H:], in_norm, out_norm, agg, act, slope, S, partial, mask,
+                             policy=_policy_col(plan, "dst", H, agg, act, QK.dtype, mask is not None))
         Y = linalg.mm_wt(S, W_R, b_R)
         ctx.save_for_backward(X, W_Q, W_K, W_R, S, mask if mask is not None else QK)
         ctx.masked = mask is not None
@@ -173,7 +190,7 @@
             Q, K = saved[:, :H], saved[:, H:]
             mask = None
         dQK = torch.empty((V, 2 * H), device=X.device, dtype=torch.float32)
-        edge_backward(plan, H, agg, act, slope, G, Q, K, mask, dQK, ctx.drop)
+        edge_backward(plan, H, agg, act, slope, G, Q, K, mask, dQK, ctx.drop, policy=True)
         dX = linalg.mm_w_pair(dQK, W_Q, W_K) if ctx.needs_input_grad[0] else None
         dW_Q = dW_K = db_Q = None
         need_bq = ctx.has_bq and ctx.needs_input_grad[2]
diff --git a/sir-gcn_amd/sirgcn/graph.py b/sir-gcn_amd/sirgcn/graph.py
--- a/sir-gcn_amd/sirgcn/graph.py
+++ b/sir-gcn_amd/sirgcn/graph.py
@@ -159,6 +159,41 @@
                   n_slots=n_slots, max_degree=int(deg.max().item()) if n_rows else 0)
 
 
+POLICY_BUDGET_BYTES = 128 << 20
+POLICY_MIN_TABLE_BYTES = 256 << 20
+POLICY_MIN_SHARE = 0.5
+
+
+def hot_nodes(counts, row_bytes, budget_bytes):
+    counts = counts.to(torch.int64)
+    n = min(int(budget_bytes) // int(row_bytes), int((counts > 0).sum().item()))
+    hot = torch.zeros(counts.numel(), dtype=torch.bool, device=counts.device)
+    if n > 0:
+        order = torch.sort(counts, descending=True, stable=True).indices
+        hot[order[:n]] = True
+    return hot
+
+
+def pack_policy(col, hot):
+    return torch.where(hot[col.long()], col, ~col).contiguous()
+
+
+def policy_col(col, counts, row_bytes, budget_bytes=None, min_share=None, min_table_bytes=None):
+    budget_bytes = POLICY_BUDGET_BYTES if budget_bytes is None else budget_bytes
+    min_share = POLICY_MIN_SHARE if min_share is None else min_share
+    min_table_bytes = POLICY_MIN_TABLE_BYTES if min_table_bytes is None else min_table_bytes
+    table = counts.numel() * int(row_bytes)
+    if col.numel() == 0 or table <= budget_bytes or table <= min_table_bytes:
+        return col
+    total = int(counts.sum().item())
+    if total == 0:
+        return col
+    hot = hot_nodes(counts, row_bytes, budget_bytes)
+    if float(counts[hot].sum().item()) < min_share * total:
+        return col
+    return pack_policy(col, hot)
+
+
 def build_plans_native(src, dst, n_dst_rows, n_src_rows, chunk=DEFAULT_CHUNK):
     from . import _native
     E = src.numel()
@@ -210,6 +245,14 @@
         self.in_deg = (self.dst.rowptr[1:] - self.dst.rowptr[:-1]).to(torch.int64)
         self.out_deg = (self.src.rowptr[1:] - self.src.rowptr[:-1]).to(torch.int64)
         self._norms = {}
+        self._policy = {}
+
+    def policy_col(self, side, row_bytes):
+        key = (side, int(row_bytes))
+        if key not in self._policy:
+            csr, counts = (self.dst, self.out_deg) if side == "dst" else (self.src, self.in_deg)
+            self._policy[key] = policy_col(csr.col, counts, row_bytes)
+        return self._policy[key]
 
     def norms(self, agg):
         if agg != "sym":
```
